# facebookresearch/goliath

Measured on NVIDIA H100. Metric: rendered megapixels/sec (fwd+bwd) RGCA head 300k Gaussians, higher is better.
Workload: dtype f32

## Files before the change

### goliath_b200/_lib.py

```python
import ctypes
import os

import torch

_HERE = os.path.dirname(os.path.abspath(__file__))
LIB_PATH = os.path.join(_HERE, "libgoliath_b200.so")
_lib = None

_vp, _i, _f, _i64, _sz = ctypes.c_void_p, ctypes.c_int, ctypes.c_float, ctypes.c_int64, ctypes.c_size_t

SIGNATURES = {
    "gb_version": (_i, []),
    "gb_launch_count": (ctypes.c_ulonglong, []),
    "gb_launch_count_reset": (None, []),
    "gb_sg_evaluate_fwd": (_i, [_vp] * 7 + [_i] * 4 + [_vp]),
    "gb_sg_evaluate_bwd": (_i, [_vp] * 10 + [_i] * 4 + [_vp]),
    "gb_project_gaussians_fwd": (_i, [_i, _vp, _vp, _f, _vp, _vp, _f, _f, _f, _f, _i, _i, _i, _f] + [_vp] * 7 + [_vp]),
    "gb_project_gaussians_bwd": (_i, [_i, _vp, _vp, _f, _vp, _vp, _f, _f] + [_vp] * 13 + [_vp]),
    "gb_cumsum_workspace_bytes": (_sz, [_i]),
    "gb_cumsum_i32": (_i, [_i, _vp, _vp, _vp, _vp]),
    "gb_map_gaussian_to_intersects": (_i, [_i, _vp, _vp, _vp, _vp, _i, _i, _i, _vp, _vp, _vp]),
    "gb_sort_workspace_bytes": (_sz, [_i64]),
    "gb_sort_intersects": (_i, [_i64, _vp, _vp, _vp, _vp, _i, _vp, _vp]),
    "gb_get_tile_bin_edges": (_i, [_i64, _vp, _vp, _vp]),
    "gb_rasterize_fwd": (_i, [_i, _i, _i, _i] + [_vp] * 10 + [_vp]),
    "gb_rasterize_bwd": (_i, [_i, _i, _i, _i] + [_vp] * 15 + [_vp]),
    "gb_pack_records": (_i, [_i64, _i] + [_vp] * 6 + [_vp]),
    "gb_tile_order": (_i, [_i, _vp, _vp, _vp]),
    "gb_pack_records_fused": (_i, [_i64] + [_vp] * 8 + [_vp]),
    "gb_pack_records_fused_dn": (_i, [_i64] + [_vp] * 9 + [_vp]),
    "gb_map_gaussian_to_intersects_dn": (_i, [_i, _vp, _vp, _vp, _vp, _i, _i, _i, _i64, _vp, _vp, _vp]),
    "gb_sort_intersects_dn": (_i, [_i64, _vp, _vp, _vp, _vp, _vp, _i, _vp, _vp]),
    "gb_get_tile_bin_edges_dn": (_i, [_i64, _vp, _vp, _vp, _vp, _vp]),
    "gb_get_tile_sort_mode": (_i, []),
    "gb_set_tile_sort_mode": (None, [_i]),
    "gb_get_rank_sort_mode": (_i, []),
    "gb_set_rank_sort_mode": (None, [_i]),
    "gb_bin_tiles_supported": (_i, [_i]),
    "gb_bin_tiles_workspace_bytes": (_sz, [_i, _i, _i64]),
    "gb_bin_tiles_pack": (_i, [_i] + [_vp] * 7 + [_i, _i, _i, _i64] + [_vp, _vp, _i] + [_vp] * 5 + [_vp]),
    "gb_bin_tiles_pack_ev": (_i, [_i] + [_vp] * 7 + [_i, _i, _i, _i64] + [_vp, _vp, _i] + [_vp] * 5 + [_vp, _vp]),
    "gb_tile_schedule_ints": (_i, [_i]),
    "gb_tile_schedule": (_i, [_i, _vp, _vp, _vp]),
    "gb_rasterize_sched_fwd": (_i, [_i, _i, _i] + [_vp] * 7 + [_vp]),
    "gb_rasterize_sched_bwd": (_i, [_i, _i, _i] + [_vp] * 13 + [_vp]),
    "gb_records_widen": (_i, [_i64, _vp, _vp, _vp, _vp]),
    "gb_records_set_colors4": (_i, [_i64, _vp, _vp, _vp, _i, _i64, _vp, _vp]),
    "gb_rasterize_multi_fwd": (_i, [_i, _i, _vp, _vp, _i, _vp, _vp, _vp, _vp]),
    "gb_rasterize_multi_bwd": (_i, [_i, _i, _vp, _vp, _vp, _i] + [_vp] * 9 + [_vp]),
    "gb_colors12_unpack": (_i, [_i64, _i, _vp, _vp, _vp]),
    "gb_records_set_colors": (_i, [_i64] + [_vp] * 5 + [_vp]),
    "gb_splat_grad_unpack": (_i, [_i] + [_vp] * 8 + [_vp]),
    "gb_get_blend_mode": (_i, []),
    "gb_set_blend_mode": (None, [_i]),
    "gb_rasterize_packed_fwd": (_i, [_i, _i, _i] + [_vp] * 7 + [_vp]),
    "gb_rasterize_packed_bwd": (_i, [_i, _i, _i] + [_vp] * 13 + [_vp]),
    "gb_rasterize_ranked_fwd": (_i, [_i, _i, _i] + [_vp] * 8 + [_vp]),
    "gb_rasterize_ranked_bwd": (_i, [_i, _i, _i] + [_vp] * 14 + [_vp]),
    "gb_rasterize_ranked_fwd_lists": (_i, [_i, _i, _i] + [_vp] * 10 + [_vp]),
    "gb_rasterize_ranked_bwd_lists": (_i, [_i, _i, _i] + [_vp] * 14 + [_vp]),
    "gb_bin_tiles_ranked": (_i, [_i] + [_vp] * 7 + [_i, _i, _i, _i64] + [_vp, _vp, _i] + [_vp] * 6 + [_vp, _vp]),
    "gb_compute_raydirs_fwd": (_i, [_i, _i, _i] + [_vp] * 5 + [_f] + [_vp] * 3 + [_vp]),
    "gb_compute_raydirs_bwd": (_i, []),
    "gb_mvp_aabb_workspace_bytes": (_sz, [_i, _i]),
    "gb_mvp_compute_aabb": (_i, [_i, _i] + [_vp] * 8 + [_vp]),
    "gb_get_raymarch_mode": (_i, []),
    "gb_set_raymarch_mode": (None, [_i]),
    "gb_mvp_raymarch_fwd": (_i, [_i] * 4 + [_vp, _vp, _f] + [_vp] * 5 + [_i] * 3 + [_vp] + [_i] * 3 + [_vp] * 4
                            + [_i, _f, _f, _i, _i, _vp]),
    "gb_deconv_tc_weight_bytes": (_sz, [_i, _i]),
    "gb_nchw_to_nhwc_split": (_i, [_i] * 5 + [_vp] * 3 + [_vp]),
    "gb_deconv4x4s2_tc_fwd": (_i, [_i] * 6 + [_vp] * 6 + [_f, _i, _vp, _vp, _i, _vp, _vp]),
    "gb_deconv4x4s2_wnub_fwd": (_i, [_i] * 5 + [_vp] * 4 + [_f, _i, _vp, _vp]),
    "gb_deconv4x4s2_wnub_bwd": (_i, [_i] * 5 + [_vp] * 5 + [_f, _i] + [_vp] * 4 + [_vp]),
    "gb_conv4x4s2_wnub_fwd": (_i, [_i] * 5 + [_vp] * 4 + [_f, _i, _vp, _vp]),
    "gb_conv4x4s2_wnub_bwd": (_i, [_i] * 5 + [_vp] * 5 + [_f, _i] + [_vp] * 4 + [_vp]),
    "gb_conv2d_wnub_fwd": (_i, [_i] * 6 + [_vp] * 4 + [_i, _f, _i, _vp, _vp]),
    "gb_conv2d_wnub_bwd": (_i, [_i] * 6 + [_vp] * 5 + [_f, _i, _i] + [_vp] * 4 + [_vp]),
    "gb_mvp_slab_to_prims_fwd": (_i, [_i] * 6 + [_vp] * 3 + [_f, _f, _i, _vp, _vp]),
    "gb_mvp_slab_to_prims_bwd": (_i, [_i] * 6 + [_vp] * 3 + [_f, _f, _i] + [_vp] * 3 + [_vp]),
    "gb_mvp_prim_transform_fwd": (_i, [_i, _i] + [_vp] * 3 + [_f, _i] + [_vp] * 3 + [_vp]),
    "gb_mvp_prim_transform_bwd": (_i, [_i, _i] + [_vp] * 3 + [_f, _i] + [_vp] * 4 + [_vp]),
    "gb_mvp_prim_frames_fwd": (_i, [_i] * 4 + [_vp] * 10 + [_vp]),
    "gb_lbs_max_joints": (_i, []),
    "gb_lbs_skeleton_fwd": (_i, [_i] * 4 + [_vp, _vp, _i] + [_vp] * 7 + [_i] + [_vp] * 3 + [_vp]),
    "gb_lbs_skin_fwd": (_i, [_i] * 4 + [_vp] * 7 + [_vp]),
    "gb_lbs_skin_bwd": (_i, [_i] * 4 + [_vp] * 6 + [_vp]),
    "gb_lbs_unskin_fwd": (_i, [_i] * 4 + [_vp] * 7 + [_vp]),
    "gb_sg_shade_compose_fwd":(_i, [_vp] * 10 + [_i] * 4 + [_vp]),
    "gb_sg_shade_compose_bwd": (_i, [_vp] * 16 + [_i] * 4 + [_vp]),
    "gb_render_finish_fwd": (_i, [_i, _i] + [_vp] * 5 + [_vp]),
    "gb_render_finish_bwd": (_i, [_i, _i] + [_vp] * 4 + [_vp]),
    "gb_rgca_heads_fwd": (_i, [_i, _i] + [_vp] * 7 + [_f, _f] + [_vp] * 15 + [_vp]),
    "gb_rgca_heads_bwd": (_i, [_i, _i] + [_vp] * 7 + [_f, _f] + [_vp] * 20 + [_vp]),
    "gb_vert_normals_fwd": (_i, [_i, _i, _i, _vp, _vp, _f, _vp, _vp, _vp]),
    "gb_vert_normals_bwd": (_i, [_i, _i, _i, _vp, _vp, _f, _vp, _vp, _vp, _vp, _vp]),
    "gb_values_to_uv_fwd": (_i, [_i, _i, _i, _i64, _vp, _vp, _vp, _vp, _vp]),
    "gb_values_to_uv_bwd": (_i, [_i, _i, _i, _i64, _vp, _vp, _vp, _vp, _vp]),
    "gb_optim_chunk_elems": (_i, []),
    "gb_optim_row_bytes": (_i, []),
    "gb_grad_sanitize_sqnorm": (_i, [_vp, _vp, _i, _vp, _vp]),
    "gb_adam_step": (_i, [_vp, _vp, _i, _vp, _f, _f, _f, _f, _i, _i, _i, _vp]),
    "gb_post_render_fwd": (_i, [_i, _i, _i] + [_vp] * 8 + [_vp]),
    "gb_post_render_bwd": (_i, [_i, _i, _i] + [_vp] * 12 + [_vp]),
    "gb_ssim_l1_fwd": (_i, [_i, _i, _i] + [_vp] * 7 + [_vp]),
    "gb_ssim_l1_bwd": (_i, [_i, _i, _i] + [_vp] * 8 + [_f, _f, _vp, _vp]),
    "gb_envmap_spec_fwd": (_i, [_i, _i, _i] + [_vp] * 6 + [_f, _vp, _vp]),
    "gb_envmap_spec_bwd": (_i, [_i, _i, _i] + [_vp] * 6 + [_f, _vp, _vp, _vp, _vp]),
    "gb_envmap_rotate": (_i, [_i, _i, _i, _vp, _vp, _vp, _vp]),
    "gb_envmap_compose_fwd": (_i, [_i] * 5 + [_vp] * 5 + [_i, _i, _vp, _vp, _vp]),
    "gb_envmap_compose_bwd": (_i, [_i, _i, _i, _vp, _vp, _vp]),
    "gb_envmap_prefilter_sg": (_i, [_i, _i] + [_vp] * 5 + [_i, ctypes.c_ulonglong, _vp, _vp]),
    "gb_envmap_spin_table": (_i, [_i, _i, _i, _vp, _vp, _f, _f] + [_vp] * 6 + [_vp]),
    "gb_mvp_shadow_march": (_i, [_i] * 5 + [_vp, _vp, _f] + [_vp] * 5 + [_i] * 4 + [_vp] * 3 + [_f, _f, _i, _i, _vp]),
    "gb_olat_features": (_i, [_i] * 7 + [_f] + [_vp] * 9 + [_i, _vp, _vp]),
    "gb_olat_compose_fwd": (_i, [_i] * 4 + [_vp] * 4 + [_i, _vp, _vp]),
    "gb_olat_compose_bwd": (_i, [_i] * 4 + [_vp] * 6 + [_vp]),
    "gb_mvp_raymarch_bwd":(_i, [_i] * 4 + [_vp, _vp, _f] + [_vp] * 5 + [_i] * 3 + [_vp] + [_i] * 3 + [_vp] * 8
                            + [_i, _f, _f, _i, _i, _vp]),
    "gb_upconv_block_fwd": (_i, [_i] * 6 + [_vp] * 10 + [_f] + [_vp] * 3 + [_vp]),
    "gb_upconv_block_bwd": (_i, [_i] * 6 + [_vp] * 10 + [_f] + [_vp] * 10 + [_vp]),
    "gb_sparse_rows_apply": (_i, [_i] * 3 + [_vp] * 4 + [_i64] * 3 + [_vp] + [_i64] * 3 + [_vp]),
    "gb_conv3x3_ub_slice_fwd": (_i, [_i] * 5 + [_vp, _i64] + [_vp] * 4 + [_vp]),
    "gb_conv3x3_ub_slice_bwd": (_i, [_i] * 5 + [_vp, _i64] + [_vp] * 6 + [_vp]),
    "gb_body_tex_compose_workspace_bytes": (_sz, [_i, _i]),
    "gb_body_tex_compose_fwd": (_i, [_i] * 3 + [_vp] * 5 + [_f] + [_vp] * 3 + [_vp]),
    "gb_body_tex_compose_bwd": (_i, [_i] * 3 + [_vp] * 5 + [_f] + [_vp] * 9 + [_vp]),
    "gb_mesh_raster_workspace_bytes": (_sz, [_i] * 4),
    "gb_mesh_raster": (_i, [_i] * 5 + [_vp] * 4 + [_vp]),
    "gb_mesh_render_fwd": (_i, [_i] * 8 + [_vp] * 11 + [_vp]),
    "gb_mesh_render_bwd_workspace_bytes": (_sz, [_i] * 6),
    "gb_mesh_render_bwd": (_i, [_i] * 8 + [_vp] * 9 + [_i] + [_vp] * 5 + [_vp]),
    "gb_downconv_block_fwd": (_i, [_i] * 6 + [_vp, _i64, _i64, _i, _i, _i, _vp, _f] + [_vp] * 9 + [_f] + [_vp] * 3 + [_vp]),
    "gb_downconv_block_bwd_workspace_bytes": (_sz, [_i] * 6),
    "gb_downconv_block_bwd": (_i, [_i] * 6 + [_vp, _i64, _i64, _i, _i, _i, _vp, _f] + [_vp] * 9 + [_f] + [_vp] * 10
                              + [_vp]),
    "gb_depth_disc_mask": (_i, [_i] * 3 + [_vp, _f, _vp, _vp]),
    "gb_pixel_bias_fwd": (_i, [_i] * 7 + [_vp] * 4 + [_vp]),
    "gb_pixel_bias_bwd": (_i, [_i] * 7 + [_vp] * 3 + [_vp]),
    "gb_face_tex_tail_fwd": (_i, [_i] * 5 + [_vp] * 7 + [_vp]),
    "gb_face_tex_cond_fwd": (_i, [_i] * 6 + [_vp] * 3 + [_vp]),
    "gb_pose_shadow_fwd": (_i, [_i] * 5 + [_vp, _f, _vp, _vp]),
    "gb_pose_shadow_bwd": (_i, [_i] * 5 + [_vp, _f, _vp, _vp, _vp]),
}


class GoliathB200Error(RuntimeError):
    pass


def lib():
    global _lib
    if _lib is None:
        if not os.path.exists(LIB_PATH):
            raise GoliathB200Error(
                "libgoliath_b200.so is not built (%s). Run `python -m goliath_b200.build`; there is no CPU "
                "fallback." % LIB_PATH
            )
        l = ctypes.CDLL(LIB_PATH)
        for name, (res, args) in SIGNATURES.items():
            fn = getattr(l, name)
            fn.restype = res
            fn.argtypes = args
        _lib = l
    return _lib


def check(err, what):
    if err != 0:
        raise GoliathB200Error("%s failed: CUDA error %d" % (what, err))


def ptr(t):
    return None if t is None else t.data_ptr()


def stream_ptr(device=None):
    return torch.cuda.current_stream(device).cuda_stream


def check_input(t, name, dtype=torch.float32):
    if not t.is_cuda:
        raise RuntimeError("%s must be a CUDA tensor" % name)
    if not t.is_contiguous():
        raise RuntimeError("%s must be contiguous" % name)
    if dtype is not None and t.dtype != dtype:
        raise RuntimeError("%s must have dtype %s (got %s)" % (name, dtype, t.dtype))
```

### goliath_b200/csrc/splat_bin_tiles.cu

```cuda

#include "common.cuh"
#include "splat_record.cuh"

#include <algorithm>

extern "C" int gb_tile_order(int num_tiles, const int32_t* tile_bins, int32_t* order, void* stream);
extern "C" int gb_tile_schedule(int num_tiles, const int32_t* tile_bins, int32_t* sched, void* stream);
GB_API int gb_bin_tiles_pack_ev(int G, const float* xys, const float* depths, const int32_t* radii, const float* conics,
                                const float* colors3, const float* opacity, const float* compensation, int img_h,
                                int img_w, int block_width, int64_t cap, int32_t* tile_bins, int32_t* tile_order,
                                int tile_sched, int32_t* gids_sorted, float* records, int32_t* n_out, int32_t* overflow,
                                void* workspace, void* colors_ready, void* stream);

namespace {

constexpr int kGaussBlock = 1024;
constexpr int kScatItems = 3;
constexpr int kMaxSmemTiles = 20 * 1024;
constexpr int kMaxGaussians = 3 << 19;

constexpr int kSortThreads = 512;
constexpr int kSortWarps = kSortThreads / 32;
constexpr int kSortItems = 10;
constexpr int kSortCap = kSortThreads * kSortItems;
constexpr int kDigitBits = 9;
constexpr int kDigits = 1 << kDigitBits;
static_assert(kDigits == kSortThreads, "one digit per thread");
constexpr int kTieRun = 16;

inline int count_items(int G) { return G <= 2048 * 192 ? 2 : 4; }

__device__ __forceinline__ int block_exclusive_scan(int v, int* s_warp, int& total) {
  const int lane = threadIdx.x & 31, warp = threadIdx.x >> 5;
  int inc = v;
#pragma unroll
  for (int o = 1; o < 32; o <<= 1) {
    int t = __shfl_up_sync(0xffffffffu, inc, o);
    if (lane >= o) inc += t;
  }
  if (lane == 31) s_warp[warp] = inc;
  __syncthreads();
  if (warp == 0) {
    int w = (lane < (int)(blockDim.x >> 5)) ? s_warp[lane] : 0;
    int winc = w;
#pragma unroll
    for (int o = 1; o < 32; o <<= 1) {
      int t = __shfl_up_sync(0xffffffffu, winc, o);
      if (lane >= o) winc += t;
    }
    s_warp[lane] = winc - w;
    if (lane == 31) s_warp[32] = winc;
  }
  __syncthreads();
  total = s_warp[32];
  const int r = s_warp[warp] + inc - v;
  __syncthreads();
  return r;
}

__device__ __forceinline__ void tile_bbox(float cx, float cy, float radius, int tbx, int tby, int bw, int& x0,
                                          int& y0, int& x1, int& y1) {
  const float fb = (float)bw;
  const float tcx = __fdiv_rn(cx, fb), tcy = __fdiv_rn(cy, fb), tr = __fdiv_rn(radius, fb);
  x0 = min(max(0, __float2int_rz(__fsub_rn(tcx, tr))), tbx);
  x1 = min(max(0, __float2int_rz(__fadd_rn(__fadd_rn(tcx, tr), 1.f))), tbx);
  y0 = min(max(0, __float2int_rz(__fsub_rn(tcy, tr))), tby);
  y1 = min(max(0, __float2int_rz(__fadd_rn(__fadd_rn(tcy, tr), 1.f))), tby);
}

template <int kItems>
__global__ void __launch_bounds__(kGaussBlock) tile_count_kernel(int G, const float2* __restrict__ xys,
                                                                 const int* __restrict__ radii, int tbx, int tby,
                                                                 int block_width, int smem_tiles,
                                                                 int* __restrict__ tile_counts, int4* __restrict__ rects,
                                                                 int* __restrict__ identity) {
  extern __shared__ int s_cnt[];
  for (int t = threadIdx.x; t < smem_tiles; t += kGaussBlock) s_cnt[t] = 0;
  const int base = blockIdx.x * (kGaussBlock * kItems);
  int r[kItems];
  float2 c[kItems];
#pragma unroll
  for (int j = 0; j < kItems; ++j) {
    const int i = base + j * kGaussBlock + threadIdx.x;
    const bool in = i < G;
    r[j] = in ? radii[i] : 0;
    c[j] = in ? xys[i] : make_float2(0.f, 0.f);
    if (in && identity) identity[i] = i;
  }
  __syncthreads();
#pragma unroll
  for (int j = 0; j < kItems; ++j) {
    const int i = base + j * kGaussBlock + threadIdx.x;
    if (i >= G) continue;
    if (r[j] <= 0) {
      rects[i] = make_int4(-1, 0, 0, 0);
      continue;
    }
    int x0, y0, x1, y1;
    tile_bbox(c[j].x, c[j].y, (float)r[j], tbx, tby, block_width, x0, y0, x1, y1);
    rects[i] = make_int4(x0, y0, x1, y1);
    for (int ty = y0; ty < y1; ++ty)
      for (int tx = x0; tx < x1; ++tx) {
        if (smem_tiles) atomicAdd(&s_cnt[ty * tbx + tx], 1);
        else atomicAdd(&tile_counts[ty * tbx + tx], 1);
      }
  }
  __syncthreads();
  for (int t = threadIdx.x; t < smem_tiles; t += kGaussBlock) {
    const int cnt = s_cnt[t];
    if (cnt) atomicAdd(&tile_counts[t], cnt);
  }
}

__global__ void __launch_bounds__(1024) tile_scan_kernel(int T, long long cap, const int* __restrict__ counts,
                                                         int2* __restrict__ tile_bins, int* __restrict__ cursor,
                                                         int* __restrict__ n_out, int* __restrict__ overflow) {
  __shared__ int s_warp[33];
  int carry = 0;
  for (int base = 0; base < T; base += blockDim.x) {
    const int i = base + threadIdx.x;
    const int v = (i < T) ? counts[i] : 0;
    int total;
    const int ex = block_exclusive_scan(v, s_warp, total);
    if (i < T) {
      const int s = carry + ex;
      cursor[i] = s;
      const int cs = (int)min((long long)s, cap), ce = (int)min((long long)s + v, cap);
      tile_bins[i] = (ce > cs) ? make_int2(cs, ce) : make_int2(0, 0);
    }
    carry += total;
  }
  if (threadIdx.x == 0) {
    if (n_out) *n_out = carry;
    if (overflow && (long long)carry > cap) *overflow = 1;
  }
}

constexpr int kStageCap = 12 * 1024;
constexpr int kStageMaxTiles = 10 * 1024;
constexpr size_t kStageEntryBytes = 4 + 4 + 2;
static_assert(kStageCap * 8 >= (kGaussBlock / 32) * 96 * 16, "the record spans fit in s_id | s_key");

inline int scatter_per_cta(int G, int num_sms) {
  const int per_sm = gb::cdiv(G, num_sms > 0 ? num_sms : 1);
  return std::min(kScatItems * kGaussBlock, std::max(kGaussBlock, (per_sm + 31) & ~31));
}

inline int scatter_stage_cap(int smem_tiles) { return (smem_tiles > 0 && smem_tiles <= kStageMaxTiles) ? kStageCap : 0; }
inline size_t scatter_smem_bytes(int smem_tiles) {
  return (size_t)((smem_tiles + 3) & ~3) * 8 + (size_t)scatter_stage_cap(smem_tiles) * kStageEntryBytes;
}

__global__ void __launch_bounds__(kGaussBlock, 1) tile_scatter_kernel(
    int G, const int4* __restrict__ rects, const float2* __restrict__ xys, const float* __restrict__ conics,
    const float* __restrict__ colors3, const float* __restrict__ depths, const float* __restrict__ opacity,
    const float* __restrict__ comp, int tbx, long long cap, int per_cta, int smem_tiles, int stage_cap,
    int* __restrict__ cursor, int* __restrict__ tile_ids, unsigned* __restrict__ keys, float4* __restrict__ rec_by_id) {
  extern __shared__ int s_cnt[];
  __shared__ int s_warp[33];
  const int tpad = (smem_tiles + 3) & ~3;
  int* s_off = s_cnt + tpad;
  int* s_id = s_off + tpad;
  unsigned* s_key = reinterpret_cast<unsigned*>(s_id + stage_cap);
  unsigned short* s_tile = reinterpret_cast<unsigned short*>(s_key + stage_cap);
  const int lane = threadIdx.x & 31, warp = threadIdx.x >> 5;
  for (int t = threadIdx.x; t < smem_tiles; t += kGaussBlock) s_cnt[t] = 0;
  const int base = blockIdx.x * per_cta, end = min(G, base + per_cta);
  int4 rc[kScatItems];
  unsigned dk[kScatItems];
#pragma unroll
  for (int j = 0; j < kScatItems; ++j) {
    const int i = base + j * kGaussBlock + threadIdx.x;
    rc[j] = (i < end) ? rects[i] : make_int4(-1, 0, 0, 0);
    dk[j] = (i < end) ? __float_as_uint(depths[i]) : 0u;
  }
  __syncthreads();
  unsigned bx[kScatItems], by[kScatItems];
#pragma unroll
  for (int j = 0; j < kScatItems; ++j) {
    const int i = base + j * kGaussBlock + threadIdx.x;
    const bool vis = rc[j].x >= 0;
    bx[j] = vis ? (unsigned)rc[j].x | ((unsigned)rc[j].z << 16) : 0u;
    by[j] = vis ? (unsigned)rc[j].y | ((unsigned)rc[j].w << 16) : 0u;
    if (stage_cap && j * kGaussBlock < per_cta) {
      float4* span = reinterpret_cast<float4*>(s_id) + warp * 96;
      if (vis) gb::pack_record_fused(i, xys, conics, colors3, depths, opacity, comp, span + 3 * lane);
      const unsigned vmask = __ballot_sync(0xffffffffu, vis);
      __syncwarp();
      float4* dst = rec_by_id + 3 * (size_t)(i - lane);
#pragma unroll
      for (int f = lane; f < 96; f += 32) {
        const int r = f / 3, part = f - 3 * r;
        if (((vmask >> r) & 1u) && (part < 2 || colors3)) dst[f] = span[f];
      }
      __syncwarp();
    } else if (vis) {
      gb::pack_record_fused(i, xys, conics, colors3, depths, opacity, comp, rec_by_id + 3 * (size_t)i);
    }
  }
  if (!smem_tiles) {
#pragma unroll
    for (int j = 0; j < kScatItems; ++j) {
      const int i = base + j * kGaussBlock + threadIdx.x;
      const int x0 = bx[j] & 0xffffu, x1 = bx[j] >> 16, y0 = by[j] & 0xffffu, y1 = by[j] >> 16;
      for (int ty = y0; ty < y1; ++ty)
        for (int tx = x0; tx < x1; ++tx) {
          const int pos = atomicAdd(&cursor[ty * tbx + tx], 1);
          if ((long long)pos < cap) {
            tile_ids[pos] = i;
            keys[pos] = dk[j];
          }
        }
    }
    return;
  }
#pragma unroll
  for (int j = 0; j < kScatItems; ++j) {
    const int x0 = bx[j] & 0xffffu, x1 = bx[j] >> 16, y0 = by[j] & 0xffffu, y1 = by[j] >> 16;
    for (int ty = y0; ty < y1; ++ty)
      for (int tx = x0; tx < x1; ++tx) atomicAdd(&s_cnt[ty * tbx + tx], 1);
  }
  __syncthreads();
#pragma unroll 4
  for (int t = threadIdx.x; t < smem_tiles; t += kGaussBlock) {
    const int cnt = s_cnt[t];
    s_off[t] = cnt ? atomicAdd(&cursor[t], cnt) : 0;
  }
  int n_local = 0;
  for (int t0 = 0; t0 < smem_tiles; t0 += kGaussBlock) {
    const int t = t0 + threadIdx.x;
    const int cnt = (t < smem_tiles) ? s_cnt[t] : 0;
    int total;
    const int loc = n_local + block_exclusive_scan(cnt, s_warp, total);
    if (t < smem_tiles) {
      s_off[t] -= loc;
      s_cnt[t] = loc;
    }
    n_local += total;
  }
  __syncthreads();
  const bool staged = n_local <= stage_cap;
#pragma unroll
  for (int j = 0; j < kScatItems; ++j) {
    const int i = base + j * kGaussBlock + threadIdx.x;
    const int x0 = bx[j] & 0xffffu, x1 = bx[j] >> 16, y0 = by[j] & 0xffffu, y1 = by[j] >> 16;
    for (int ty = y0; ty < y1; ++ty)
      for (int tx = x0; tx < x1; ++tx) {
        const int t = ty * tbx + tx;
        const int e = atomicAdd(&s_cnt[t], 1);
        if (staged) {
          s_id[e] = i;
          s_key[e] = dk[j];
          s_tile[e] = (unsigned short)t;
        } else {
          const int pos = s_off[t] + e;
          if ((long long)pos < cap) {
            tile_ids[pos] = i;
            keys[pos] = dk[j];
          }
        }
      }
  }
  if (!staged) return;
  __syncthreads();
  for (int e = threadIdx.x; e < n_local; e += kGaussBlock) {
    const int pos = s_off[s_tile[e]] + e;
    if ((long long)pos < cap) {
      tile_ids[pos] = s_id[e];
      keys[pos] = s_key[e];
    }
  }
}

struct SortSmem {
  unsigned short whist[kSortWarps][kDigits];
  int base[kDigits];
  int run[kDigits];
  int warp[33];
  unsigned red[4];
};

__device__ __forceinline__ int entry_of(int j, int ipt) {
  return (threadIdx.x >> 5) * (32 * ipt) + j * 32 + (threadIdx.x & 31);
}

__device__ __forceinline__ bool holds(int j, int ipt, int m) { return j < ipt && entry_of(j, ipt) < m; }

__device__ __forceinline__ void radix_positions(const unsigned long long (&k)[kSortItems], int m, int ipt, int shift,
                                                bool whole, SortSmem& s, int (&dst)[kSortItems]) {
  const int lane = threadIdx.x & 31, warp = threadIdx.x >> 5;
  const int wbase = warp * (32 * ipt);
  const int ours = min(ipt, max(0, (m - wbase + 31) >> 5)), mine = min(ipt, max(0, (m - wbase - lane + 31) >> 5));
  for (int d = lane; d < kDigits; d += 32) s.whist[warp][d] = 0;
  __syncwarp();
#pragma unroll
  for (int j = 0; j < kSortItems; ++j) {
    dst[j] = 0;
    if (j >= ours) continue;
    const bool valid = j < mine;
    const unsigned dgt = (unsigned)(k[j] >> shift) & (kDigits - 1);
    unsigned peers = __ballot_sync(0xffffffffu, valid);
#pragma unroll
    for (int b = 0; b < kDigitBits; ++b) {
      const unsigned bal = __ballot_sync(0xffffffffu, (dgt >> b) & 1u);
      peers &= ((dgt >> b) & 1u) ? bal : ~bal;
    }
    const unsigned lower = peers & ((1u << lane) - 1u);
    unsigned prev = 0;
    if (valid) prev = s.whist[warp][dgt];
    __syncwarp();
    dst[j] = (int)(prev + __popc(lower));
    if (valid && lower == 0u) s.whist[warp][dgt] = (unsigned short)(prev + __popc(peers));
    __syncwarp();
  }
  __syncthreads();
  {
    const int d = threadIdx.x;
    int run = 0;
#pragma unroll
    for (int w = 0; w < kSortWarps; ++w) {
      const int c = s.whist[w][d];
      s.whist[w][d] = (unsigned short)run;
      run += c;
    }
    int total;
    if (whole) {
      s.base[d] = block_exclusive_scan(run, s.warp, total);
    } else {
      const int b = s.run[d];
      s.base[d] = b;
      s.run[d] = b + run;
    }
  }
  __syncthreads();
#pragma unroll
  for (int j = 0; j < kSortItems; ++j) {
    const unsigned dgt = (unsigned)(k[j] >> shift) & (kDigits - 1);
    dst[j] = (j < mine) ? s.base[dgt] + s.whist[warp][dgt] + dst[j] : -1;
  }
}

__device__ __forceinline__ void smem_pass(unsigned long long (&k)[kSortItems], int n, int ipt, int shift, SortSmem& s,
                                          unsigned long long* s_key) {
  int dst[kSortItems];
  radix_positions(k, n, ipt, shift, true, s, dst);
#pragma unroll
  for (int j = 0; j < kSortItems; ++j)
    if (dst[j] >= 0) s_key[dst[j]] = k[j];
  __syncthreads();
#pragma unroll
  for (int j = 0; j < kSortItems; ++j)
    if (holds(j, ipt, n)) k[j] = s_key[entry_of(j, ipt)];
}

__device__ __forceinline__ void minmax_to_smem(unsigned kmin, unsigned kmax, unsigned imin, unsigned imax, SortSmem& s) {
  kmin = __reduce_min_sync(0xffffffffu, kmin);
  kmax = __reduce_max_sync(0xffffffffu, kmax);
  imin = __reduce_min_sync(0xffffffffu, imin);
  imax = __reduce_max_sync(0xffffffffu, imax);
  if ((threadIdx.x & 31) == 0) {
    atomicMin(&s.red[0], kmin);
    atomicMax(&s.red[1], kmax);
    atomicMin(&s.red[2], imin);
    atomicMax(&s.red[3], imax);
  }
}

__device__ __forceinline__ int bits_of(unsigned span) { return span ? 32 - __clz((int)span) : 0; }

__global__ void __launch_bounds__(kSortThreads, 2) tile_sort_kernel(const int* __restrict__ order,
                                                                    const int2* __restrict__ tile_bins,
                                                                    const unsigned* __restrict__ depth_keys,
                                                                    int* bucket, int* out) {
  extern __shared__ unsigned long long s_key[];
  __shared__ SortSmem s;
  const int tile = order ? order[blockIdx.x] : (int)blockIdx.x;
  const int2 range = tile_bins[tile];
  const int n = range.y - range.x;
  if (n <= 0) return;
  if (threadIdx.x == 0) {
    s.red[0] = s.red[2] = 0xffffffffu;
    s.red[1] = s.red[3] = 0u;
  }
  __syncthreads();

  if (n <= kSortCap) {
    const int ipt = (n + kSortThreads - 1) / kSortThreads;
    int id[kSortItems];
    unsigned dk[kSortItems];
#pragma unroll
    for (int j = 0; j < kSortItems; ++j) {
      const bool h = holds(j, ipt, n);
      id[j] = h ? bucket[range.x + entry_of(j, ipt)] : -1;
      dk[j] = h ? (unsigned)out[range.x + entry_of(j, ipt)] : 0u;
    }
    unsigned kmin = 0xffffffffu, kmax = 0u, imin = 0xffffffffu, imax = 0u;
#pragma unroll
    for (int j = 0; j < kSortItems; ++j) {
      if (id[j] < 0) continue;
      kmin = min(kmin, dk[j]); kmax = max(kmax, dk[j]);
      imin = min(imin, (unsigned)id[j]); imax = max(imax, (unsigned)id[j]);
    }
    minmax_to_smem(kmin, kmax, imin, imax, s);
    __syncthreads();
    kmin = s.red[0];
    imin = s.red[2];
    const int bi = bits_of(s.red[3] - imin), bits = bits_of(s.red[1] - kmin) + bi;
    unsigned long long k[kSortItems];
#pragma unroll
    for (int j = 0; j < kSortItems; ++j)
      k[j] = ((unsigned long long)(dk[j] - kmin) << bi) | (unsigned long long)((unsigned)id[j] - imin);
    for (int shift = bi; shift < bits; shift += kDigitBits) smem_pass(k, n, ipt, shift, s, s_key);
    if (bits == bi) {
#pragma unroll
      for (int j = 0; j < kSortItems; ++j)
        if (holds(j, ipt, n)) s_key[entry_of(j, ipt)] = k[j];
      __syncthreads();
    }
    static_assert(kTieRun < 32 && kSortItems * 5 <= 64, "run lengths are packed 5 bits per item");
    unsigned long long runs = 0ull;
    bool too_long = false;
#pragma unroll
    for (int j = 0; j < kSortItems; ++j) {
      const int e = j * kSortThreads + threadIdx.x;
      if (j >= ipt || e >= n) continue;
      const unsigned long long d = s_key[e] >> bi;
      if (e > 0 && (s_key[e - 1] >> bi) == d) continue;
      int len = 1;
      while (len <= kTieRun && e + len < n && (s_key[e + len] >> bi) == d) ++len;
      if (len > kTieRun) too_long = true;
      else runs |= (unsigned long long)len << (5 * j);
    }
    if (__syncthreads_or(too_long)) {
#pragma unroll
      for (int j = 0; j < kSortItems; ++j) k[j] = holds(j, ipt, n) ? s_key[entry_of(j, ipt)] : 0ull;
      for (int shift = 0; shift < bits; shift += kDigitBits) smem_pass(k, n, ipt, shift, s, s_key);
    } else {
#pragma unroll
      for (int j = 0; j < kSortItems; ++j) {
        const int e = j * kSortThreads + threadIdx.x, len = (int)(runs >> (5 * j)) & 31;
        for (int a = e + 1; a < e + len; ++a) {
          const unsigned long long v = s_key[a];
          int b = a;
          for (; b > e && s_key[b - 1] > v; --b) s_key[b] = s_key[b - 1];
          s_key[b] = v;
        }
      }
      __syncthreads();
    }
    const unsigned long long imask = (1ull << bi) - 1ull;
    for (int e = threadIdx.x; e < n; e += kSortThreads) out[range.x + e] = (int)(imin + (unsigned)(s_key[e] & imask));
    return;
  }

  {
    unsigned kmin = 0xffffffffu, kmax = 0u, imin = 0xffffffffu, imax = 0u;
    for (int i = threadIdx.x; i < n; i += kSortThreads) {
      const int g = bucket[range.x + i];
      const unsigned d = depth_keys[g];
      kmin = min(kmin, d); kmax = max(kmax, d);
      imin = min(imin, (unsigned)g); imax = max(imax, (unsigned)g);
    }
    minmax_to_smem(kmin, kmax, imin, imax, s);
  }
  __syncthreads();
  const unsigned kmin = s.red[0], imin = s.red[2];
  const int bi = bits_of(s.red[3] - imin), bits = bits_of(s.red[1] - kmin) + bi;
  const unsigned long long imask = (1ull << bi) - 1ull;
  auto key_of = [&](int g) {
    return ((unsigned long long)(depth_keys[g] - kmin) << bi) | (unsigned long long)((unsigned)g - imin);
  };
  int* src = bucket + range.x;
  int* dstp = out + range.x;
  for (int shift = 0; shift < bits; shift += kDigitBits) {
    unsigned* s_cnt = reinterpret_cast<unsigned*>(s_key);
    s_cnt[threadIdx.x] = 0u;
    __syncthreads();
    for (int i = threadIdx.x; i < n; i += kSortThreads)
      atomicAdd(&s_cnt[(unsigned)(key_of(src[i]) >> shift) & (kDigits - 1)], 1u);
    __syncthreads();
    int total;
    s.run[threadIdx.x] = block_exclusive_scan((int)s_cnt[threadIdx.x], s.warp, total);
    __syncthreads();
    for (int c0 = 0; c0 < n; c0 += kSortCap) {
      const int m = min(kSortCap, n - c0);
      unsigned long long k[kSortItems];
#pragma unroll
      for (int j = 0; j < kSortItems; ++j)
        k[j] = holds(j, kSortItems, m) ? key_of(src[c0 + entry_of(j, kSortItems)]) : 0ull;
      int dst[kSortItems];
      radix_positions(k, m, kSortItems, shift, false, s, dst);
#pragma unroll
      for (int j = 0; j < kSortItems; ++j)
        if (dst[j] >= 0) dstp[dst[j]] = (int)(imin + (unsigned)(k[j] & imask));
      __syncthreads();
    }
    int* t = src; src = dstp; dstp = t;
  }
  if (src != out + range.x) {
    for (int i = threadIdx.x; i < n; i += kSortThreads) out[range.x + i] = src[i];
  }
}

__global__ void __launch_bounds__(256) rec_colors_kernel(int G, const int* __restrict__ radii,
                                                         const float* __restrict__ colors3,
                                                         const float* __restrict__ depths, float4* __restrict__ rec_by_id) {
  const int g = blockIdx.x * blockDim.x + threadIdx.x;
  if (g >= G || radii[g] <= 0) return;
  rec_by_id[3 * (size_t)g + 2] = make_float4(colors3[3 * (size_t)g], colors3[3 * (size_t)g + 1],
                                             colors3[3 * (size_t)g + 2], depths[g]);
}

__global__ void __launch_bounds__(256) gather_records_kernel(long long cap, const int* __restrict__ n_dev,
                                                             const int* __restrict__ gids_sorted,
                                                             const float4* __restrict__ rec_by_id,
                                                             float4* __restrict__ rec) {
  const long long n = min((long long)*n_dev, cap);
  const long long j = (long long)blockIdx.x * blockDim.x + threadIdx.x;
  if (j >= 3 * n) return;
  const long long i = j / 3;
  const int part = (int)(j - 3 * i);
  rec[j] = gb::ld_nc_f4(rec_by_id + 3 * (size_t)gids_sorted[i] + part);
}

struct Layout {
  size_t counts, sync, zero_bytes, cursor, rects, rec_by_id, bucket, total;
};
inline size_t align256(size_t b) { return (b + 255) & ~(size_t)255; }
inline Layout make_layout(int G, int T, int64_t cap) {
  const int g1 = G > 0 ? G : 1;
  Layout l;
  size_t o = 0;
  l.counts = o; o += align256((size_t)T * 4);
  l.sync = o;   o += 256;
  l.zero_bytes = o;
  l.cursor = o; o += align256((size_t)T * 4);
  l.rects = o;  o += align256((size_t)g1 * 16);
  l.rec_by_id = o; o += align256((size_t)g1 * 48);
  l.bucket = o; o += align256((size_t)(cap > 0 ? cap : 1) * 4);
  l.total = o;
  return l;
}

int num_sms() {
  static int s_sms[64] = {};
  int dev = 0;
  if (cudaGetDevice(&dev) != cudaSuccess) return 0;
  if (dev < 0 || dev >= 64) return 0;
  if (!s_sms[dev] && cudaDeviceGetAttribute(&s_sms[dev], cudaDevAttrMultiProcessorCount, dev) != cudaSuccess) return 0;
  return s_sms[dev];
}

template <typename K>
int opt_in_smem(K kernel, size_t bytes, bool* done) {
  int dev = 0;
  GB_CUDA(cudaGetDevice(&dev));
  if (dev < 0 || dev >= 64 || !done[dev]) {
    GB_CUDA(cudaFuncSetAttribute(kernel, cudaFuncAttributeMaxDynamicSharedMemorySize, (int)bytes));
    if (dev >= 0 && dev < 64) done[dev] = true;
  }
  return 0;
}

}

GB_API int gb_get_tile_sort_mode(void) { return 0; }
GB_API void gb_set_tile_sort_mode(int mode) { (void)mode; }
GB_API int gb_get_rank_sort_mode(void) { return 0; }
GB_API void gb_set_rank_sort_mode(int mode) { (void)mode; }

GB_API int gb_bin_tiles_supported(int G) { return G >= 1 && G <= kMaxGaussians; }

GB_API size_t gb_bin_tiles_workspace_bytes(int G, int num_tiles, int64_t cap) {
  return make_layout(G, num_tiles, cap).total;
}

GB_API int gb_bin_tiles_pack(int G, const float* xys, const float* depths, const int32_t* radii, const float* conics,
                             const float* colors3, const float* opacity, const float* compensation, int img_h,
                             int img_w, int block_width, int64_t cap, int32_t* tile_bins, int32_t* tile_order,
                             int tile_sched, int32_t* gids_sorted, float* records, int32_t* n_out, int32_t* overflow,
                             void* workspace, void* stream) {
  return gb_bin_tiles_pack_ev(G, xys, depths, radii, conics, colors3, opacity, compensation, img_h, img_w, block_width, cap,
                              tile_bins, tile_order, tile_sched, gids_sorted, records, n_out, overflow, workspace, nullptr,
                              stream);
}

static int bin_tiles_impl(int G, const float* xys, const float* depths, const int32_t* radii, const float* conics,
                          const float* colors3, const float* opacity, const float* compensation, int img_h, int img_w,
                          int block_width, int64_t cap, int32_t* tile_bins, int32_t* tile_order, int tile_sched,
                          int32_t* gids_sorted, float* records, int32_t* n_out, int32_t* overflow, void* workspace,
                          void* colors_ready, void* stream, int32_t* ext_ids, float* ext_rec, int32_t* ext_identity);

GB_API int gb_bin_tiles_pack_ev(int G, const float* xys, const float* depths, const int32_t* radii, const float* conics,
                                const float* colors3, const float* opacity, const float* compensation, int img_h,
                                int img_w, int block_width, int64_t cap, int32_t* tile_bins, int32_t* tile_order,
                                int tile_sched, int32_t* gids_sorted, float* records, int32_t* n_out, int32_t* overflow,
                                void* workspace, void* colors_ready, void* stream) {
  return bin_tiles_impl(G, xys, depths, radii, conics, colors3, opacity, compensation, img_h, img_w, block_width, cap,
                        tile_bins, tile_order, tile_sched, gids_sorted, records, n_out, overflow, workspace, colors_ready,
                        stream, nullptr, nullptr, nullptr);
}

GB_API int gb_bin_tiles_ranked(int G, const float* xys, const float* depths, const int32_t* radii, const float* conics,
                               const float* colors3, const float* opacity, const float* compensation, int img_h,
                               int img_w, int block_width, int64_t cap, int32_t* tile_bins, int32_t* tile_order,
                               int tile_sched, int32_t* ranks_sorted, float* rec_by_rank, int32_t* rank_to_gid,
                               int32_t* n_out, int32_t* overflow, void* workspace, void* colors_ready, void* stream) {
  if (!ranks_sorted || !rec_by_rank || !rank_to_gid) return (int)cudaErrorInvalidValue;
  return bin_tiles_impl(G, xys, depths, radii, conics, colors3, opacity, compensation, img_h, img_w, block_width, cap,
                        tile_bins, tile_order, tile_sched, nullptr, nullptr, n_out, overflow, workspace, colors_ready, stream,
                        ranks_sorted, rec_by_rank, rank_to_gid);
}

static int bin_tiles_impl(int G, const float* xys, const float* depths, const int32_t* radii, const float* conics,
                          const float* colors3, const float* opacity, const float* compensation, int img_h, int img_w,
                          int block_width, int64_t cap, int32_t* tile_bins, int32_t* tile_order, int tile_sched,
                          int32_t* gids_sorted, float* records, int32_t* n_out, int32_t* overflow, void* workspace,
                          void* colors_ready, void* stream, int32_t* ext_ids, float* ext_rec, int32_t* ext_identity) {
  if (!gb_bin_tiles_supported(G) || block_width < 1 || cap < 0) return (int)cudaErrorInvalidValue;
  cudaStream_t s = (cudaStream_t)stream;
  const int tbx = gb::cdiv(img_w, block_width), tby = gb::cdiv(img_h, block_width);
  const int T = tbx * tby;
  if (T < 1 || tbx > 65535 || tby > 65535) return (int)cudaErrorInvalidValue;
  const Layout l = make_layout(G, T, cap);
  char* ws = (char*)workspace;
  int* counts = (int*)(ws + l.counts);
  int* cursor = (int*)(ws + l.cursor);
  int* bucket = (int*)(ws + l.bucket);
  int4* rects = (int4*)(ws + l.rects);
  const bool ranked = ext_ids != nullptr;
  float4* rec_by_id = ranked ? (float4*)ext_rec : (float4*)(ws + l.rec_by_id);
  int* ids_sorted = ranked ? ext_ids : gids_sorted;
  const int items = count_items(G);
  const int smem_tiles = (T <= kMaxSmemTiles) ? T : 0;
  const int stage_cap = scatter_stage_cap(smem_tiles);
  const size_t scat_smem = scatter_smem_bytes(smem_tiles);
  static bool s_opt_c2[64] = {}, s_opt_c4[64] = {}, s_opt_scat[64] = {}, s_opt_sort[64] = {};
  if ((size_t)smem_tiles * 4 > 40 * 1024) {
    constexpr size_t kCountSmem = (size_t)kMaxSmemTiles * 4;
    const int e = (items == 2) ? opt_in_smem(tile_count_kernel<2>, kCountSmem, s_opt_c2)
                               : opt_in_smem(tile_count_kernel<4>, kCountSmem, s_opt_c4);
    if (e) return e;
  }
  {
    const size_t a = scatter_smem_bytes(kMaxSmemTiles), b = scatter_smem_bytes(kStageMaxTiles);
    const int e = opt_in_smem(tile_scatter_kernel, a > b ? a : b, s_opt_scat);
    if (e) return e;
  }
  const size_t sort_smem = (size_t)kSortCap * 8;
  {
    const int e = opt_in_smem(tile_sort_kernel, sort_smem, s_opt_sort);
    if (e) return e;
  }

  GB_CUDA(cudaMemsetAsync(ws, 0, l.zero_bytes, s));
  const int ctas = gb::cdiv(G, kGaussBlock * items);
  if (items == 2)
    tile_count_kernel<2><<<ctas, kGaussBlock, (size_t)smem_tiles * 4, s>>>(G, (const float2*)xys, radii, tbx, tby,
                                                                          block_width, smem_tiles, counts, rects, ext_identity);
  else
    tile_count_kernel<4><<<ctas, kGaussBlock, (size_t)smem_tiles * 4, s>>>(G, (const float2*)xys, radii, tbx, tby,
                                                                          block_width, smem_tiles, counts, rects, ext_identity);
  int* n_total = n_out ? n_out : (int*)(ws + l.sync);
  tile_scan_kernel<<<1, 1024, 0, s>>>(T, (long long)cap, counts, (int2*)tile_bins, cursor, n_total, overflow);
  gb::count_launches(2);
  GB_CHECK_LAUNCH();
  const int e = tile_sched ? gb_tile_schedule(T, tile_bins, tile_order, stream)
                           : gb_tile_order(T, tile_bins, tile_order, stream);
  if (e) return e;
  const bool late = colors_ready != nullptr;
  const int per_cta = scatter_per_cta(G, num_sms());
  tile_scatter_kernel<<<gb::cdiv(G, per_cta), kGaussBlock, scat_smem, s>>>(
      G, rects, (const float2*)xys, conics, late ? nullptr : colors3, depths, opacity, compensation, tbx, (long long)cap,
      per_cta, smem_tiles, stage_cap, cursor, bucket, (unsigned*)ids_sorted, rec_by_id);
  tile_sort_kernel<<<T, kSortThreads, sort_smem, s>>>(tile_order, (const int2*)tile_bins, (const unsigned*)depths, bucket,
                                                      ids_sorted);
  gb::count_launches(2);
  if (late) {
    GB_CUDA(cudaStreamWaitEvent(s, (cudaEvent_t)colors_ready, 0));
    rec_colors_kernel<<<gb::cdiv(G, 256), 256, 0, s>>>(G, radii, colors3, depths, rec_by_id);
    gb::count_launches(1);
  }
  if (cap > 0 && !ranked) {
    gather_records_kernel<<<(unsigned)gb::cdiv64(3 * cap, 256), 256, 0, s>>>((long long)cap, n_total, gids_sorted,
                                                                           rec_by_id, (float4*)records);
    gb::count_launches(1);
  }
  GB_CHECK_LAUNCH();
  return 0;
}
```

### goliath_b200/csrc/splat_blend_mom.cu

```cuda
#include <cstdlib>
#include <cstring>

#include "common.cuh"
#include "splat_blend_common.cuh"

namespace {

using namespace gbblend;

constexpr int kPixelWarps = 8;
constexpr int kStageRecs = 128;
constexpr int kFwdStages = 4;
constexpr int kFwdThreads = (kPixelWarps + 1) * 32;
constexpr int kBwdStages = 3;
constexpr int kBwdThreads = kPixelWarps * 32;
constexpr int kChunk = 16;
constexpr int kEntryCap = 48;
constexpr int kMStride = 33;
constexpr float kCullMargin = 2e-3f;

__device__ __forceinline__ float rcp_approx(float x) {
  float r;
  asm("rcp.approx.ftz.f32 %0, %1;" : "=f"(r) : "f"(x));
  return r;
}

__device__ __forceinline__ float exp_neg(float s) {
  float r;
  asm("ex2.approx.ftz.f32 %0, %1;" : "=f"(r) : "f"(s * -1.4426950408889634f));
  return r;
}

__device__ __forceinline__ void cp_async16(void* dst, const void* src) {
  asm volatile("cp.async.cg.shared.global [%0], [%1], 16;" ::"r"(smem_u32(dst)), "l"(src) : "memory");
}
__device__ __forceinline__ void cp_async_arrive(unsigned long long* bar) {
  asm volatile("cp.async.mbarrier.arrive.noinc.shared::cta.b64 [%0];" ::"r"(smem_u32(bar)) : "memory");
}
__device__ __forceinline__ void cp_async_wait_all() { asm volatile("cp.async.wait_all;" ::: "memory"); }
__device__ __forceinline__ void cp_async4(void* dst, const void* src) {
  asm volatile("cp.async.ca.shared.global [%0], [%1], 4;" ::"r"(smem_u32(dst)), "l"(src) : "memory");
}
__device__ __forceinline__ bool footprint_hit(const float4 q0, const float4* __restrict__ q1p, float fx0, float fx1,
                                              float fy0, float fy1) {
  if (!((q0.x + q0.z >= fx0) && (q0.x - q0.z <= fx1) && (q0.y + q0.w >= fy0) && (q0.y - q0.w <= fy1))) return false;
  if (q0.z > 1e30f) return true;
  const float4 q1 = *q1p;
  const float dxlo = q0.x - fx1, dxhi = q0.x - fx0, dylo = q0.y - fy1, dyhi = q0.y - fy0;
  const float ex0 = fminf(fmaxf(0.f, dxlo), dxhi), ey0 = fminf(fmaxf(0.f, dylo), dyhi);
  const float dy1 = fminf(fmaxf(-q1.y * ex0 * rcp_approx(q1.z), dylo), dyhi);
  const float dx2 = fminf(fmaxf(-q1.y * ey0 * rcp_approx(q1.x), dxlo), dxhi);
  const float f1 = 0.5f * (q1.x * ex0 * ex0 + q1.z * dy1 * dy1) + q1.y * ex0 * dy1;
  const float f2 = 0.5f * (q1.x * dx2 * dx2 + q1.z * ey0 * ey0) + q1.y * dx2 * ey0;
  const float s = __logf(255.f * q1.w);
  return fminf(f1, f2) <= s + kCullMargin + 1e-4f * fabsf(s);
}

struct Tile {
  int tile_id, tx, ty;
};
__device__ __forceinline__ Tile make_tile(int tile_id, int tbx) {
  Tile t;
  t.tile_id = tile_id;
  t.ty = tile_id / tbx;
  t.tx = tile_id - t.ty * tbx;
  return t;
}

template <int C, bool LIST, bool RANKED, bool HITS = false>
__global__ void __launch_bounds__(kFwdThreads) blend_fwd_ilp_kernel(
    int img_w, int img_h, int tbx, const int* order, int sched, const int2* __restrict__ tile_bins,
    const float4* __restrict__ rec , const int* __restrict__ ranks ,
    const float* __restrict__ background, float* __restrict__ final_Ts, int* __restrict__ final_idx,
    float* __restrict__ out_img, int* __restrict__ hit_list = nullptr, int* __restrict__ hit_count = nullptr) {
  static_assert(!HITS || LIST, "hit lists are the LIST variant's per-stage lists");
  __shared__ __align__(128) float4 s_rec[kFwdStages][kStageRecs * 3];
  __shared__ __align__(8) unsigned long long s_full[kFwdStages];
  __shared__ __align__(8) unsigned long long s_empty[kFwdStages];
  __shared__ int s_ndone;
  __shared__ int s_tile;
  __shared__ __align__(16) int s_hits[LIST ? kPixelWarps : 1][LIST ? kStageRecs + 4 : 4];

  const int tr = threadIdx.x, lane = tr & 31, warp = tr >> 5;
  if (tr == 0) {
    s_tile = draw_tile(order, sched, tbx * ((img_h + 15) >> 4));
#pragma unroll
    for (int s = 0; s < kFwdStages; ++s) {
      mbar_init(&s_full[s], RANKED ? 32 : 1);
      mbar_init(&s_empty[s], kPixelWarps);
    }
    s_ndone = 0;
    fence_mbar_init();
  }
  __syncthreads();
  if (s_tile < 0) return;
  const Tile tl = make_tile(s_tile, tbx);
  const int2 range = tile_bins[tl.tile_id];
  const int num_batches = (range.y - range.x + kStageRecs - 1) / kStageRecs;

  if (RANKED && warp == kPixelWarps) {
    volatile int* ndone = &s_ndone;
    int r[4];
    auto load_ranks = [&](int b) {
      const int start = range.x + b * kStageRecs;
      const int count = min(kStageRecs, range.y - start);
#pragma unroll
      for (int k = 0; k < 4; ++k) r[k] = (b < num_batches && lane + 32 * k < count) ? ranks[start + lane + 32 * k] : -1;
    };
    load_ranks(0);
    for (int b = 0; b < num_batches; ++b) {
      const int s = b % kFwdStages;
      if (b >= kFwdStages) {
        int go = 1;
        if (lane == 0) {
          const unsigned par = (unsigned)(((b / kFwdStages) - 1) & 1);
          while (!mbar_try(&s_empty[s], par) && *ndone < kPixelWarps) {
        }
          go = *ndone < kPixelWarps;
        }
        go = __shfl_sync(0xffffffffu, go, 0);
        if (!go) break;
      }
#pragma unroll
      for (int k = 0; k < 4; ++k)
        if (r[k] >= 0) {
          const float4* src = rec + 3 * (size_t)r[k];
          float4* dst = &s_rec[s][3 * (lane + 32 * k)];
          cp_async16(dst, src);
          cp_async16(dst + 1, src + 1);
          cp_async16(dst + 2, src + 2);
        }
      cp_async_arrive(&s_full[s]);
      load_ranks(b + 1);
    }
    cp_async_wait_all();
    return;
  }
  if (warp == kPixelWarps) {
    if (lane != 0) return;
    volatile int* ndone = &s_ndone;
    int issued = 0;
    for (int b = 0; b < num_batches; ++b) {
      const int s = b % kFwdStages;
      if (b >= kFwdStages) {
        const unsigned par = (unsigned)(((b / kFwdStages) - 1) & 1);
        while (!mbar_try(&s_empty[s], par) && *ndone < kPixelWarps) {
        }
        if (*ndone >= kPixelWarps) break;
      }
      const int start = range.x + b * kStageRecs;
      const unsigned bytes = (unsigned)min(kStageRecs, range.y - start) * kRecBytes;
      mbar_expect_tx(&s_full[s], bytes);
      bulk_g2s(&s_rec[s][0], rec + (size_t)start * 3, bytes, &s_full[s]);
      issued = b + 1;
    }
    for (int b = max(0, issued - kFwdStages); b < issued; ++b)
      mbar_wait(&s_full[b % kFwdStages], (unsigned)((b / kFwdStages) & 1));
    return;
  }

  const int wx0 = tl.tx * 16 + ((warp & 1) << 3), wy0 = tl.ty * 16 + ((warp >> 1) << 2);
  const int pxi = wx0 + (lane & 7), pyi = wy0 + (lane >> 3);
  const bool inside = (pxi < img_w) && (pyi < img_h);
  const float px = (float)pxi + 0.5f, py = (float)pyi + 0.5f;
  const float fx0 = (float)wx0 + 0.5f, fx1 = (float)wx0 + 7.5f, fy0 = (float)wy0 + 0.5f, fy1 = (float)wy0 + 3.5f;

  bool done = !inside;
  float T = 1.f;
  int cur_idx = 0;
  float acc[4] = {0.f, 0.f, 0.f, 0.f};
  int* const seg = HITS ? hit_list + 8 * (size_t)range.x + (size_t)warp * (range.y - range.x) : nullptr;
  int written = 0, last_pos = -1;

  bool counted = false;
  for (int b = 0; b < num_batches; ++b) {
    const bool all_done = __all_sync(0xffffffffu, done);
    if (all_done && !counted) {
      counted = true;
      if (lane == 0) atomicAdd(&s_ndone, 1);
    }
    const int s = b % kFwdStages;
    const unsigned par = (unsigned)((b / kFwdStages) & 1);
    int st = 0;
    if (lane == 0) {
      volatile int* ndone = &s_ndone;
      for (;;) {
        if (mbar_try(&s_full[s], par)) { st = 1; break; }
        if (all_done && *ndone >= kPixelWarps) { st = 2; break; }
      }
    }
    st = __shfl_sync(0xffffffffu, st, 0);
    if (st == 2) break;
    if (all_done) {
      if (lane == 0) mbar_arrive(&s_empty[s]);
      continue;
    }
    mbar_wait(&s_full[s], par);
    const float4* sr = s_rec[s];
    const int batch_start = range.x + b * kStageRecs;
    const int batch_size = min(kStageRecs, range.y - batch_start);
    if (LIST) {
      int* hl = s_hits[LIST ? warp : 0];
      const unsigned lt = (1u << lane) - 1u;
      int cnt = 0;
#pragma unroll 4
      for (int c0 = 0; c0 < batch_size; c0 += 32) {
        const int ti = c0 + lane;
        bool hit = false;
        if (ti < batch_size) hit = footprint_hit(sr[ti * 3], &sr[ti * 3 + 1], fx0, fx1, fy0, fy1);
        const unsigned mask = __ballot_sync(0xffffffffu, hit);
        if (hit) hl[cnt + __popc(mask & lt)] = ti;
        cnt += __popc(mask);
      }
      __syncwarp();
      if (HITS) {
        for (int i = lane; i < cnt; i += 32) seg[written + i] = batch_start + hl[i];
        if (b == 0 && range.x == 0 && cnt > 0 && hl[0] == 0 && inside) last_pos = 0;
      }
      for (int i0 = 0; i0 < cnt; i0 += 16) {
        const int i1 = min(i0 + 16, cnt);
        for (int i = i0; i < i1; i += 4) {
          const int4 e = *reinterpret_cast<const int4*>(hl + i);
          bool live[4];
          int t[4];
          live[0] = true; live[1] = i + 1 < cnt; live[2] = i + 2 < cnt; live[3] = i + 3 < cnt;
          t[0] = e.x; t[1] = live[1] ? e.y : e.x; t[2] = live[2] ? e.z : e.x; t[3] = live[3] ? e.w : e.x;
          float alpha[4], sig[4];
          float4 col[4];
#pragma unroll
          for (int u = 0; u < 4; ++u) {
            const float4 q0 = sr[t[u] * 3], q1 = sr[t[u] * 3 + 1];
            col[u] = sr[t[u] * 3 + 2];
            const float dx = q0.x - px, dy = q0.y - py;
            sig[u] = 0.5f * (q1.x * dx * dx + q1.z * dy * dy) + q1.y * dx * dy;
            alpha[u] = fminf(kAlphaMaxFwd, q1.w * exp_neg(sig[u]));
          }
#pragma unroll
          for (int u = 0; u < 4; ++u) {
            const bool ok = live[u] && !done && !(sig[u] < 0.f) && !(alpha[u] < kAlphaMin);
            const float next_T = T * (1.f - alpha[u]);
            const bool stop = ok && (next_T <= kTEps);
            const bool take = ok && !stop;
            done = done || stop;
            if (take) {
              const float vis = alpha[u] * T;
              acc[0] += col[u].x * vis;
              acc[1] += col[u].y * vis;
              acc[2] += col[u].z * vis;
              if (C == 4) acc[3] += col[u].w * vis;
              T = next_T;
              cur_idx = batch_start + t[u];
              if (HITS) last_pos = written + i + u;
            }
          }
        }
        if (__all_sync(0xffffffffu, done)) break;
      }
      written += cnt;
    } else {
    for (int c0 = 0; c0 < batch_size; c0 += 32) {
        const int ti = c0 + lane;
        bool hit = false;
        if (ti < batch_size) hit = footprint_hit(sr[ti * 3], &sr[ti * 3 + 1], fx0, fx1, fy0, fy1);
        unsigned mask = __ballot_sync(0xffffffffu, hit);
        while (mask) {
          int t[4];
          bool live[4];
  #pragma unroll
          for (int u = 0; u < 4; ++u) {
            live[u] = mask != 0;
            t[u] = live[u] ? c0 + __ffs(mask) - 1 : t[0];
            mask &= mask - 1;
          }
          float alpha[4], sig[4];
          float4 col[4];
  #pragma unroll
          for (int u = 0; u < 4; ++u) {
            const float4 q0 = sr[t[u] * 3], q1 = sr[t[u] * 3 + 1];
            col[u] = sr[t[u] * 3 + 2];
            const float dx = q0.x - px, dy = q0.y - py;
            sig[u] = 0.5f * (q1.x * dx * dx + q1.z * dy * dy) + q1.y * dx * dy;
            alpha[u] = fminf(kAlphaMaxFwd, q1.w * __expf(-sig[u]));
          }
  #pragma unroll
          for (int u = 0; u < 4; ++u) {
            const bool ok = live[u] && !done && !(sig[u] < 0.f) && !(alpha[u] < kAlphaMin);
            const float next_T = T * (1.f - alpha[u]);
            const bool stop = ok && (next_T <= kTEps);
            const bool take = ok && !stop;
            done = done || stop;
            if (take) {
              const float vis = alpha[u] * T;
              acc[0] += col[u].x * vis;
              acc[1] += col[u].y * vis;
              acc[2] += col[u].z * vis;
              if (C == 4) acc[3] += col[u].w * vis;
              T = next_T;
              cur_idx = batch_start + t[u];
            }
          }
        }
        if (__all_sync(0xffffffffu, done)) break;
      }
  }
    __syncwarp();
    if (lane == 0) mbar_arrive(&s_empty[s]);
  }
  if (HITS) {
#pragma unroll
    for (int o = 16; o > 0; o >>= 1) last_pos = max(last_pos, __shfl_xor_sync(0xffffffffu, last_pos, o));
    if (lane == 0) hit_count[8 * tl.tile_id + warp] = last_pos + 1;
    if (blockIdx.x == 0 && tr == 0) hit_count[8 * tbx * ((img_h + 15) >> 4)] = 0;
  }
  if (inside) {
    const size_t pix = (size_t)pyi * img_w + pxi;
    final_Ts[pix] = T;
    final_idx[pix] = cur_idx;
    if (C == 4) {
      reinterpret_cast<float4*>(out_img)[pix] =
          make_float4(acc[0] + T * background[0], acc[1] + T * background[1], acc[2] + T * background[2],
                      acc[3] + T * background[3]);
    } else {
      out_img[pix * 3 + 0] = acc[0] + T * background[0];
      out_img[pix * 3 + 1] = acc[1] + T * background[1];
      out_img[pix * 3 + 2] = acc[2] + T * background[2];
    }
  }
}

constexpr int kSmRec = kBwdStages * kStageRecs * kRecBytes;
constexpr int kSmEntries = kPixelWarps * kEntryCap * 48;
constexpr int kSmM = kPixelWarps * kChunk * kMStride * 8;
constexpr int kSmVo = kPixelWarps * 32 * 16;
constexpr int kBwdSmem = kSmRec + kSmEntries + kSmM + kSmVo;

template <int C, bool RANKED>
__global__ void __launch_bounds__(kBwdThreads, 3) blend_bwd_mom_kernel(
    int img_w, int img_h, int tbx, const int* order, int sched,
    const int* __restrict__ gids_sorted , const int* __restrict__ ranks ,
    const int2* __restrict__ tile_bins, const float4* __restrict__ rec, const float* __restrict__ background,
    const float* __restrict__ final_Ts, const int* __restrict__ final_idx, const float* __restrict__ v_output,
    const float* __restrict__ v_output_alpha, float* __restrict__ v_xy, float* __restrict__ v_conic,
    float* __restrict__ v_colors, float* __restrict__ v_opacity) {
  extern __shared__ __align__(128) unsigned char smem[];
  float4* s_rec = reinterpret_cast<float4*>(smem);
  __shared__ __align__(8) unsigned long long s_full[kBwdStages];
  __shared__ int s_ticket[kBwdStages];
  __shared__ int s_cta_final;
  __shared__ int s_tile;
  __shared__ int s_rk[RANKED ? kBwdStages : 1][RANKED ? kStageRecs : 1];

  const int tr = threadIdx.x, lane = tr & 31, warp = tr >> 5;
  if (tr == 0) s_tile = draw_tile(order, sched, tbx * ((img_h + 15) >> 4));
  __syncthreads();
  if (s_tile < 0) return;
  float4* E = reinterpret_cast<float4*>(smem + kSmRec) + warp * kEntryCap * 3;
  float2* M = reinterpret_cast<float2*>(smem + kSmRec + kSmEntries) + warp * kChunk * kMStride;
  float4* VO = reinterpret_cast<float4*>(smem + kSmRec + kSmEntries + kSmM) + warp * 32;

  const Tile tl = make_tile(s_tile, tbx);
  const int2 range = tile_bins[tl.tile_id];
  if (range.y <= range.x) return;
  const int wx0 = tl.tx * 16 + ((warp & 1) << 3), wy0 = tl.ty * 16 + ((warp >> 1) << 2);
  const int pxi = wx0 + (lane & 7), pyi = wy0 + (lane >> 3);
  const bool inside = (pxi < img_w) && (pyi < img_h);
  const float px = (float)pxi + 0.5f, py = (float)pyi + 0.5f;
  const float fx0 = (float)wx0 + 0.5f, fx1 = (float)wx0 + 7.5f, fy0 = (float)wy0 + 0.5f, fy1 = (float)wy0 + 3.5f;
  const size_t pix = inside ? ((size_t)pyi * img_w + pxi) : 0;

  const float T_final = inside ? final_Ts[pix] : 1.f;
  float T = T_final;
  float bufv = 0.f;
  const int bin_final = inside ? final_idx[pix] : -1;
  float vo[4] = {0.f, 0.f, 0.f, 0.f};
  float voa = 0.f;
  if (inside) {
#pragma unroll
    for (int c = 0; c < C; ++c) vo[c] = v_output[pix * C + c];
    voa = v_output_alpha ? v_output_alpha[pix] : 0.f;
  }
  VO[lane] = make_float4(vo[0], vo[1], vo[2], vo[3]);
  float bgdot = 0.f;
#pragma unroll
  for (int c = 0; c < C; ++c) bgdot += background[c] * vo[c];
  const float tfc = T_final * (voa - bgdot);

  int warp_bin_final = bin_final;
#pragma unroll
  for (int o = 16; o > 0; o >>= 1) warp_bin_final = max(warp_bin_final, __shfl_xor_sync(0xffffffffu, warp_bin_final, o));
  if (tr == 0) {
    s_cta_final = -1;
#pragma unroll
    for (int s = 0; s < kBwdStages; ++s) {
      mbar_init(&s_full[s], RANKED ? 32 : 1);
      s_ticket[s] = 0;
    }
    fence_mbar_init();
  }
  __syncthreads();
  if (lane == 0) atomicMax(&s_cta_final, warp_bin_final);
  __syncthreads();
  const int last = min(s_cta_final, range.y - 1);
  if (last < range.x) return;
  const int num_batches = (last - range.x + kStageRecs) / kStageRecs;
  auto issue = [&](int k) {
    const int s = k % kBwdStages;
    const int hi = last - k * kStageRecs;
    const int lo = max(range.x, hi - kStageRecs + 1);
    const unsigned bytes = (unsigned)(hi - lo + 1) * kRecBytes;
    mbar_expect_tx(&s_full[s], bytes);
    bulk_g2s(s_rec + s * kStageRecs * 3, rec + (size_t)lo * 3, bytes, &s_full[s]);
  };
  auto issue_ranked = [&](int k) {
    const int s = k % kBwdStages;
    const int hi = last - k * kStageRecs;
    const int lo = max(range.x, hi - kStageRecs + 1);
    const int count = hi - lo + 1;
    int r[4];
#pragma unroll
    for (int i = 0; i < 4; ++i) {
      const int j = lane + 32 * i;
      r[i] = (j < count) ? (k >= kBwdStages ? s_rk[s][j] : ranks[lo + j]) : -1;
    }
    float4* stage = s_rec + s * kStageRecs * 3;
#pragma unroll
    for (int i = 0; i < 4; ++i)
      if (r[i] >= 0) {
        const float4* src = rec + 3 * (size_t)r[i];
        float4* dst = stage + 3 * (lane + 32 * i);
        cp_async16(dst, src);
        cp_async16(dst + 1, src + 1);
        cp_async16(dst + 2, src + 2);
      }
    const int k2 = k + kBwdStages;
    if (k2 < num_batches) {
      const int hi2 = last - k2 * kStageRecs;
      const int lo2 = max(range.x, hi2 - kStageRecs + 1);
#pragma unroll
      for (int i = 0; i < 4; ++i) {
        const int j = lane + 32 * i;
        if (j < hi2 - lo2 + 1) cp_async4(&s_rk[s][j], ranks + lo2 + j);
      }
    }
    cp_async_arrive(&s_full[s]);
  };
  if (RANKED) {
    if (warp == 0)
      for (int k = 0; k < min(kBwdStages, num_batches); ++k) issue_ranked(k);
  } else if (tr == 0) {
    for (int k = 0; k < min(kBwdStages, num_batches); ++k) issue(k);
  }

  auto chunk = [&](int base, int n) {
#pragma unroll 1
    for (int h0 = 0; h0 < n; h0 += 4) {
      float al[4], ov[4], ra[4];
      float4 col[4];
#pragma unroll
      for (int u = 0; u < 4; ++u) {
        const int h = h0 + u;
        const float4 a0 = E[(base + h) * 3], a1 = E[(base + h) * 3 + 1];
        col[u] = E[(base + h) * 3 + 2];
        const float dx = a0.x - px, dy = a0.y - py;
        const float sigma = 0.5f * (a0.z * dx * dx + a1.x * dy * dy) + a0.w * dx * dy;
        const float vis = exp_neg(sigma);
        const float alpha = fminf(kAlphaMaxBwd, a1.y * vis);
        const bool valid = (__float_as_int(a1.z) <= bin_final) && !(sigma < 0.f) && !(alpha < kAlphaMin);
        al[u] = valid ? alpha : 0.f;
        ov[u] = valid ? a1.y * vis : 0.f;
        ra[u] = rcp_approx(1.f - al[u]);
      }
#pragma unroll
      for (int u = 0; u < 4; ++u) {
        const float cc[4] = {col[u].x, col[u].y, col[u].z, col[u].w};
        float cv = 0.f;
#pragma unroll
        for (int c = 0; c < C; ++c) cv += cc[c] * vo[c];
        const float v_alpha = ((cv * T - bufv) + tfc) * ra[u];
        T *= ra[u];
        const float fac = al[u] * T;
        bufv += cv * fac;
        M[(h0 + u) * kMStride + lane] = make_float2(fac, -ov[u] * v_alpha);
      }
    }
    if (RANKED) cp_async_wait_all();
    __syncwarp();
    {
      const int hh = lane & 15, half = lane >> 4;
      const int he = min(hh, n - 1);
      const float4 a0 = E[(base + he) * 3], a1 = E[(base + he) * 3 + 1];
      const int e_idx = __float_as_int(a1.z);
      const int e_safe = e_idx == 0x7fffffff ? range.x : e_idx;
      const int g_id = RANKED ? __float_as_int(a1.w) : gids_sorted[e_safe];
      const float2* Mrow = M + hh * kMStride + half * 16;
      const float4* V = VO + half * 16;
      float g[4] = {0.f, 0.f, 0.f, 0.f};
      float r00 = 0.f, r01 = 0.f, r10 = 0.f, r11 = 0.f, sii = 0.f;
      float facmax = 0.f;
#pragma unroll
      for (int q = 0; q < 16; ++q) {
        const float2 m = Mrow[q];
        const float4 v = V[q];
        const float fi = (float)(q & 7);
        facmax = fmaxf(facmax, m.x);
        g[0] += m.x * v.x;
        g[1] += m.x * v.y;
        g[2] += m.x * v.z;
        if (C == 4) g[3] += m.x * v.w;
        if (q < 8) {
          r00 += m.y;
          r10 += m.y * fi;
        } else {
          r01 += m.y;
          r11 += m.y * fi;
        }
        sii += m.y * (fi * fi);
      }
      const float u_ = a0.x - fx0, v_ = a0.y - (fy0 + (float)(2 * half));
      const float S0 = r00 + r01, Sj = r01, Si = r10 + r11, Sij = r11;
      const float sx = u_ * S0 - Si, sy = v_ * S0 - Sj;
      const float sxx = u_ * (u_ * S0 - 2.f * Si) + sii;
      const float sxy = u_ * (v_ * S0 - Sj) - v_ * Si + Sij;
      const float syy = v_ * (v_ * S0 - 2.f * Sj) + Sj;
      float o[10];
      o[0] = g[0]; o[1] = g[1]; o[2] = g[2]; o[3] = g[3];
      o[4] = 0.5f * sxx; o[5] = sxy; o[6] = 0.5f * syy;
      o[7] = a0.z * sx + a0.w * sy;
      o[8] = a0.w * sx + a1.x * sy;
      o[9] = S0;
#pragma unroll
      for (int i = 0; i < 10; ++i) o[i] += __shfl_xor_sync(0xffffffffu, o[i], 16);
      facmax = fmaxf(facmax, __shfl_xor_sync(0xffffffffu, facmax, 16));
      if (half == 0 && hh < n && facmax > 0.f) {
        if (C == 4) {
          gb::red_add_v4(v_colors + 4 * (size_t)g_id, o[0], o[1], o[2], o[3]);
        } else {
          gb::red_add(v_colors + 3 * (size_t)g_id + 0, o[0]);
          gb::red_add(v_colors + 3 * (size_t)g_id + 1, o[1]);
          gb::red_add(v_colors + 3 * (size_t)g_id + 2, o[2]);
        }
        gb::red_add(v_conic + 3 * (size_t)g_id + 0, o[4]);
        gb::red_add(v_conic + 3 * (size_t)g_id + 1, o[5]);
        gb::red_add(v_conic + 3 * (size_t)g_id + 2, o[6]);
        gb::red_add_v2(v_xy + 2 * (size_t)g_id, o[7], o[8]);
        gb::red_add(v_opacity + g_id, -o[9] * rcp_approx(a1.y));
      }
    }
    __syncwarp();
  };

  auto pad4 = [&](int cnt_) {
    const int padded = (cnt_ + 3) & ~3;
    if (lane < padded - cnt_) {
      E[(cnt_ + lane) * 3 + 0] = make_float4(0.f, 0.f, 1.f, 0.f);
      E[(cnt_ + lane) * 3 + 1] = make_float4(1.f, 0.f, __int_as_float(0x7fffffff), 0.f);
      E[(cnt_ + lane) * 3 + 2] = make_float4(0.f, 0.f, 0.f, 0.f);
    }
    __syncwarp();
    return padded;
  };
  int cnt = 0;
  for (int k = 0; k < num_batches; ++k) {
    const int s = k % kBwdStages;
    const int hi = last - k * kStageRecs;
    const int lo = max(range.x, hi - kStageRecs + 1);
    const int batch_size = hi - lo + 1;
    while (!mbar_try(&s_full[s], (unsigned)((k / kBwdStages) & 1))) __nanosleep(64);
    const float4* sr = s_rec + s * kStageRecs * 3;
    const int j_top = min(batch_size - 1, warp_bin_final - lo);
    for (int c1 = (j_top & ~31); c1 >= 0 && j_top >= 0; c1 -= 32) {
      const int tj = c1 + lane;
      bool hit = false;
      if (tj <= j_top) hit = footprint_hit(sr[tj * 3], &sr[tj * 3 + 1], fx0, fx1, fy0, fy1);
      const unsigned mask = __ballot_sync(0xffffffffu, hit);
      if (mask == 0) continue;
      if (hit) {
        const int pos = cnt + __popc(mask & ~((2u << lane) - 1u));
        const float4 q0 = sr[tj * 3], q1 = sr[tj * 3 + 1], q2 = sr[tj * 3 + 2];
        E[pos * 3 + 0] = make_float4(q0.x, q0.y, q1.x, q1.y);
        if constexpr (RANKED) {
          float* e1 = reinterpret_cast<float*>(&E[pos * 3 + 1]);
          *reinterpret_cast<float2*>(e1) = make_float2(q1.z, q1.w);
          e1[2] = __int_as_float(lo + tj);
          cp_async4(e1 + 3, ranks + lo + tj);
        } else {
          E[pos * 3 + 1] = make_float4(q1.z, q1.w, __int_as_float(lo + tj), 0.f);
        }
        E[pos * 3 + 2] = q2;
      }
      cnt += __popc(mask);
      __syncwarp();
      if (cnt >= kChunk) {
        int base = 0;
        while (cnt - base >= kChunk) {
          chunk(base, kChunk);
          base += kChunk;
        }
        const int left = cnt - base;
        if (lane < left) {
          const float4 e0 = E[(base + lane) * 3], e1 = E[(base + lane) * 3 + 1], e2 = E[(base + lane) * 3 + 2];
          E[lane * 3 + 0] = e0;
          E[lane * 3 + 1] = e1;
          E[lane * 3 + 2] = e2;
        }
        cnt = left;
        __syncwarp();
      }
    }
    __syncwarp();
    int refill = 0;
    if (lane == 0) {
      __threadfence_block();
      const int ticket = atomicAdd(&s_ticket[s], 1);
      if (ticket == kPixelWarps - 1) {
        __threadfence_block();
        s_ticket[s] = 0;
        if (k + kBwdStages < num_batches) {
          if (RANKED) refill = 1;
          else issue(k + kBwdStages);
        }
      }
    }
    if (RANKED) {
      refill = __shfl_sync(0xffffffffu, refill, 0);
      if (refill) issue_ranked(k + kBwdStages);
    }
  }
  if (cnt > 0) chunk(0, pad4(cnt));
  if (RANKED) cp_async_wait_all();
}

constexpr int kListWarps = 4;
constexpr int kListThreads = kListWarps * 32;
constexpr int kOrderBuckets = 64;

__device__ __forceinline__ void cp_async_commit() { asm volatile("cp.async.commit_group;" ::: "memory"); }

__global__ void __launch_bounds__(1024) order_items_kernel(int n_items, int* __restrict__ hit_count) {
  __shared__ int s_off[kOrderBuckets];
  const int tr = threadIdx.x, lane = tr & 31;
  auto bucket = [](int n) { return kOrderBuckets - 1 - min((n + kChunk - 1) / kChunk, kOrderBuckets - 1); };
  if (tr < kOrderBuckets) s_off[tr] = 0;
  __syncthreads();
  for (int i = tr; i < n_items; i += blockDim.x) {
    const int n = hit_count[i];
    if (n > 0) atomicAdd(&s_off[bucket(n)], 1);
  }
  __syncthreads();
  if (tr < 32) {
    const int a = s_off[2 * lane], b = s_off[2 * lane + 1];
    int incl = a + b;
#pragma unroll
    for (int o = 1; o < 32; o <<= 1) {
      const int t = __shfl_up_sync(0xffffffffu, incl, o);
      if (lane >= o) incl += t;
    }
    const int excl = incl - a - b;
    s_off[2 * lane] = excl;
    s_off[2 * lane + 1] = excl + a;
    if (lane == 31) hit_count[n_items + 1] = incl;
  }
  __syncthreads();
  int* items = hit_count + n_items + 2;
  for (int i = tr; i < n_items; i += blockDim.x) {
    const int n = hit_count[i];
    if (n > 0) items[atomicAdd(&s_off[bucket(n)], 1)] = i;
  }
}

template <int C>
__global__ void __launch_bounds__(kListThreads, 6) blend_bwd_lists_kernel(
    int img_w, int img_h, int tbx, int n_items, const int2* __restrict__ tile_bins, const int* __restrict__ hit_list,
    const int* __restrict__ hit_count, int* draw ,
    const int* __restrict__ ranks, const float4* __restrict__ rec, const float* __restrict__ background,
    const float* __restrict__ final_Ts, const int* __restrict__ final_idx, const float* __restrict__ v_output,
    const float* __restrict__ v_output_alpha, float* __restrict__ v_xy, float* __restrict__ v_conic,
    float* __restrict__ v_colors, float* __restrict__ v_opacity) {
  __shared__ __align__(16) float4 s_e[kListWarps][2][kChunk * 3];
  __shared__ __align__(8) int2 s_ig[kListWarps][2][kChunk];
  __shared__ float2 s_m[kListWarps][kChunk * kMStride];
  __shared__ float4 s_vo[kListWarps][32];

  const int lane = threadIdx.x & 31, wib = threadIdx.x >> 5;
  float2* M = s_m[wib];
  float4* VO = s_vo[wib];
  const int n_work = hit_count[n_items + 1];
  const int* items = hit_count + n_items + 2;
  const int n_draws = n_work + (int)gridDim.x * kListWarps;
  for (;;) {
    int k = 0;
    if (lane == 0) {
      k = atomicAdd(draw, 1);
      if (k == n_draws - 1) *draw = 0;
    }
    k = __shfl_sync(0xffffffffu, k, 0);
    if (k >= n_work) break;
    const int item = items[k], tile = item >> 3, warp = item & 7;
    const int n = hit_count[item];
    const int2 range = tile_bins[tile];
    const int* list = hit_list + 8 * (size_t)range.x + (size_t)warp * (range.y - range.x);
    const Tile tl = make_tile(tile, tbx);
    const int wx0 = tl.tx * 16 + ((warp & 1) << 3), wy0 = tl.ty * 16 + ((warp >> 1) << 2);
    const int pxi = wx0 + (lane & 7), pyi = wy0 + (lane >> 3);
    const bool inside = (pxi < img_w) && (pyi < img_h);
    const float px = (float)pxi + 0.5f, py = (float)pyi + 0.5f;
    const float fx0 = (float)wx0 + 0.5f, fy0 = (float)wy0 + 0.5f;
    const size_t pix = inside ? ((size_t)pyi * img_w + pxi) : 0;

    const int nchunks = (n + kChunk - 1) / kChunk;
    int g_idx = 0, g_id = 0;
    auto load_next = [&](int j) {
      const int top = n - kChunk * j;
      if (lane < min(kChunk, top)) {
        g_idx = list[top - 1 - lane];
        g_id = ranks[g_idx];
      }
    };
    auto gather = [&](int j) {
      const int cnt = min(kChunk, n - kChunk * j);
      float4* E = s_e[wib][j & 1];
      if (lane < cnt) {
        const float4* src = rec + 3 * (size_t)g_id;
        cp_async16(&E[lane * 3 + 0], src);
        cp_async16(&E[lane * 3 + 1], src + 1);
        cp_async16(&E[lane * 3 + 2], src + 2);
        s_ig[wib][j & 1][lane] = make_int2(g_idx, g_id);
      } else if (lane < ((cnt + 3) & ~3)) {
        E[lane * 3 + 0] = make_float4(0.f, 0.f, 0.f, 0.f);
        E[lane * 3 + 1] = make_float4(1.f, 0.f, 1.f, 0.f);
        E[lane * 3 + 2] = make_float4(0.f, 0.f, 0.f, 0.f);
        s_ig[wib][j & 1][lane] = make_int2(0x7fffffff, 0);
      }
      cp_async_commit();
    };
    load_next(0);
    gather(0);

    const float T_final = inside ? final_Ts[pix] : 1.f;
    float T = T_final;
    float bufv = 0.f;
    const int bin_final = inside ? final_idx[pix] : -1;
    float vo[4] = {0.f, 0.f, 0.f, 0.f};
    float voa = 0.f;
    if (inside) {
#pragma unroll
      for (int c = 0; c < C; ++c) vo[c] = v_output[pix * C + c];
      voa = v_output_alpha ? v_output_alpha[pix] : 0.f;
    }
    VO[lane] = make_float4(vo[0], vo[1], vo[2], vo[3]);
    float bgdot = 0.f;
#pragma unroll
    for (int c = 0; c < C; ++c) bgdot += background[c] * vo[c];
    const float tfc = T_final * (voa - bgdot);
    if (nchunks > 1) load_next(1);

    for (int j = 0; j < nchunks; ++j) {
      const int cnt = min(kChunk, n - kChunk * j);
      const int nn = j + 1 < nchunks ? kChunk : ((cnt + 3) & ~3);
      const float4* E = s_e[wib][j & 1];
      const int2* IG = s_ig[wib][j & 1];
      cp_async_wait_all();
      __syncwarp();
#pragma unroll 1
      for (int h0 = 0; h0 < nn; h0 += 4) {
        float al[4], ov[4], ra[4];
        float4 col[4];
#pragma unroll
        for (int u = 0; u < 4; ++u) {
          const int h = h0 + u;
          const float4 q0 = E[h * 3], q1 = E[h * 3 + 1];
          col[u] = E[h * 3 + 2];
          const float dx = q0.x - px, dy = q0.y - py;
          const float sigma = 0.5f * (q1.x * dx * dx + q1.z * dy * dy) + q1.y * dx * dy;
          const float vis = exp_neg(sigma);
          const float alpha = fminf(kAlphaMaxBwd, q1.w * vis);
          const bool valid = (IG[h].x <= bin_final) && !(sigma < 0.f) && !(alpha < kAlphaMin);
          al[u] = valid ? alpha : 0.f;
          ov[u] = valid ? q1.w * vis : 0.f;
          ra[u] = rcp_approx(1.f - al[u]);
        }
#pragma unroll
        for (int u = 0; u < 4; ++u) {
          const float cc[4] = {col[u].x, col[u].y, col[u].z, col[u].w};
          float cv = 0.f;
#pragma unroll
          for (int c = 0; c < C; ++c) cv += cc[c] * vo[c];
          const float v_alpha = ((cv * T - bufv) + tfc) * ra[u];
          T *= ra[u];
          const float fac = al[u] * T;
          bufv += cv * fac;
          M[(h0 + u) * kMStride + lane] = make_float2(fac, -ov[u] * v_alpha);
        }
      }
      if (j + 1 < nchunks) {
        gather(j + 1);
        if (j + 2 < nchunks) load_next(j + 2);
      }
      __syncwarp();
      {
        const int hh = lane & 15, half = lane >> 4;
        const int he = min(hh, nn - 1);
        const float4 q0 = E[he * 3], q1 = E[he * 3 + 1];
        const int e_id = IG[he].y;
        const float2* Mrow = M + hh * kMStride + half * 16;
        const float4* V = VO + half * 16;
        float g[4] = {0.f, 0.f, 0.f, 0.f};
        float r00 = 0.f, r01 = 0.f, r10 = 0.f, r11 = 0.f, sii = 0.f;
        float facmax = 0.f;
#pragma unroll
        for (int q = 0; q < 16; ++q) {
          const float2 m = Mrow[q];
          const float4 v = V[q];
          const float fi = (float)(q & 7);
          facmax = fmaxf(facmax, m.x);
          g[0] += m.x * v.x;
          g[1] += m.x * v.y;
          g[2] += m.x * v.z;
          if (C == 4) g[3] += m.x * v.w;
          if (q < 8) {
            r00 += m.y;
            r10 += m.y * fi;
          } else {
            r01 += m.y;
            r11 += m.y * fi;
          }
          sii += m.y * (fi * fi);
        }
        const float u_ = q0.x - fx0, v_ = q0.y - (fy0 + (float)(2 * half));
        const float S0 = r00 + r01, Sj = r01, Si = r10 + r11, Sij = r11;
        const float sx = u_ * S0 - Si, sy = v_ * S0 - Sj;
        const float sxx = u_ * (u_ * S0 - 2.f * Si) + sii;
        const float sxy = u_ * (v_ * S0 - Sj) - v_ * Si + Sij;
        const float syy = v_ * (v_ * S0 - 2.f * Sj) + Sj;
        float o[10];
        o[0] = g[0]; o[1] = g[1]; o[2] = g[2]; o[3] = g[3];
        o[4] = 0.5f * sxx; o[5] = sxy; o[6] = 0.5f * syy;
        o[7] = q1.x * sx + q1.y * sy;
        o[8] = q1.y * sx + q1.z * sy;
        o[9] = S0;
#pragma unroll
        for (int i = 0; i < 10; ++i) o[i] += __shfl_xor_sync(0xffffffffu, o[i], 16);
        facmax = fmaxf(facmax, __shfl_xor_sync(0xffffffffu, facmax, 16));
        if (half == 0 && hh < nn && facmax > 0.f) {
          if (C == 4) {
            gb::red_add_v4(v_colors + 4 * (size_t)e_id, o[0], o[1], o[2], o[3]);
          } else {
            gb::red_add(v_colors + 3 * (size_t)e_id + 0, o[0]);
            gb::red_add(v_colors + 3 * (size_t)e_id + 1, o[1]);
            gb::red_add(v_colors + 3 * (size_t)e_id + 2, o[2]);
          }
          gb::red_add(v_conic + 3 * (size_t)e_id + 0, o[4]);
          gb::red_add(v_conic + 3 * (size_t)e_id + 1, o[5]);
          gb::red_add(v_conic + 3 * (size_t)e_id + 2, o[6]);
          gb::red_add_v2(v_xy + 2 * (size_t)e_id, o[7], o[8]);
          gb::red_add(v_opacity + e_id, -o[9] * rcp_approx(q1.w));
        }
      }
      __syncwarp();
    }
  }
}

constexpr int kMK = 4;
constexpr int kMC = 3 * kMK;
constexpr int kMRQ = 5;
constexpr int kMRecBytes = kMRQ * 16;

__global__ void __launch_bounds__(kFwdThreads) blend_fwd_multi_kernel(
    int img_w, int img_h, int tbx, const int* order, int sched, const int2* __restrict__ tile_bins,
    const float4* __restrict__ rec, const float* __restrict__ background, float* __restrict__ out_planes ) {
  __shared__ __align__(128) float4 s_rec[kFwdStages][kStageRecs * kMRQ];
  __shared__ __align__(8) unsigned long long s_full[kFwdStages];
  __shared__ __align__(8) unsigned long long s_empty[kFwdStages];
  __shared__ int s_ndone;
  __shared__ __align__(16) int s_hits[kPixelWarps][kStageRecs + 4];
  __shared__ int s_tile;

  const int tr = threadIdx.x, lane = tr & 31, warp = tr >> 5;
  if (tr == 0) {
    s_tile = draw_tile(order, sched, tbx * ((img_h + 15) >> 4));
#pragma unroll
    for (int s = 0; s < kFwdStages; ++s) {
      mbar_init(&s_full[s], 1);
      mbar_init(&s_empty[s], kPixelWarps);
    }
    s_ndone = 0;
    fence_mbar_init();
  }
  __syncthreads();
  if (s_tile < 0) return;
  const Tile tl = make_tile(s_tile, tbx);
  const int2 range = tile_bins[tl.tile_id];
  const int num_batches = (range.y - range.x + kStageRecs - 1) / kStageRecs;

  if (warp == kPixelWarps) {
    if (lane != 0) return;
    volatile int* ndone = &s_ndone;
    int issued = 0;
    for (int b = 0; b < num_batches; ++b) {
      const int s = b % kFwdStages;
      if (b >= kFwdStages) {
        const unsigned par = (unsigned)(((b / kFwdStages) - 1) & 1);
        while (!mbar_try(&s_empty[s], par) && *ndone < kPixelWarps) {
        }
        if (*ndone >= kPixelWarps) break;
      }
      const int start = range.x + b * kStageRecs;
      const unsigned bytes = (unsigned)min(kStageRecs, range.y - start) * kMRecBytes;
      mbar_expect_tx(&s_full[s], bytes);
      bulk_g2s(&s_rec[s][0], rec + (size_t)start * kMRQ, bytes, &s_full[s]);
      issued = b + 1;
    }
    for (int b = max(0, issued - kFwdStages); b < issued; ++b)
      mbar_wait(&s_full[b % kFwdStages], (unsigned)((b / kFwdStages) & 1));
    return;
  }

  const int wx0 = tl.tx * 16 + ((warp & 1) << 3), wy0 = tl.ty * 16 + ((warp >> 1) << 2);
  const int pxi = wx0 + (lane & 7), pyi = wy0 + (lane >> 3);
  const bool inside = (pxi < img_w) && (pyi < img_h);
  const float px = (float)pxi + 0.5f, py = (float)pyi + 0.5f;
  const float fx0 = (float)wx0 + 0.5f, fx1 = (float)wx0 + 7.5f, fy0 = (float)wy0 + 0.5f, fy1 = (float)wy0 + 3.5f;

  bool done = !inside;
  float T = 1.f;
  float acc[kMC];
#pragma unroll
  for (int c = 0; c < kMC; ++c) acc[c] = 0.f;

  bool counted = false;
  for (int b = 0; b < num_batches; ++b) {
    const bool all_done = __all_sync(0xffffffffu, done);
    if (all_done && !counted) {
      counted = true;
      if (lane == 0) atomicAdd(&s_ndone, 1);
    }
    const int s = b % kFwdStages;
    const unsigned par = (unsigned)((b / kFwdStages) & 1);
    int st = 0;
    if (lane == 0) {
      volatile int* ndone = &s_ndone;
      for (;;) {
        if (mbar_try(&s_full[s], par)) { st = 1; break; }
        if (all_done && *ndone >= kPixelWarps) { st = 2; break; }
      }
    }
    st = __shfl_sync(0xffffffffu, st, 0);
    if (st == 2) break;
    if (all_done) {
      if (lane == 0) mbar_arrive(&s_empty[s]);
      continue;
    }
    mbar_wait(&s_full[s], par);
    const float4* sr = s_rec[s];
    const int batch_start = range.x + b * kStageRecs;
    const int batch_size = min(kStageRecs, range.y - batch_start);
    {
      int* hl = s_hits[warp];
      const unsigned lt = (1u << lane) - 1u;
      int cnt = 0;
#pragma unroll 4
      for (int c0 = 0; c0 < batch_size; c0 += 32) {
        const int ti = c0 + lane;
        bool hit = false;
        if (ti < batch_size) hit = footprint_hit(sr[ti * kMRQ], &sr[ti * kMRQ + 1], fx0, fx1, fy0, fy1);
        const unsigned mask = __ballot_sync(0xffffffffu, hit);
        if (hit) hl[cnt + __popc(mask & lt)] = ti;
        cnt += __popc(mask);
      }
      __syncwarp();
      for (int i0 = 0; i0 < cnt; i0 += 16) {
        const int i1 = min(i0 + 16, cnt);
        for (int i = i0; i < i1; i += 2) {
          const int2 e = *reinterpret_cast<const int2*>(hl + i);
          bool live[2];
          int t[2];
          live[0] = true; live[1] = i + 1 < cnt;
          t[0] = e.x; t[1] = live[1] ? e.y : e.x;
          float alpha[2], sig[2];
          float4 col[2][3];
#pragma unroll
          for (int u = 0; u < 2; ++u) {
            const float4 q0 = sr[t[u] * kMRQ], q1 = sr[t[u] * kMRQ + 1];
            col[u][0] = sr[t[u] * kMRQ + 2]; col[u][1] = sr[t[u] * kMRQ + 3]; col[u][2] = sr[t[u] * kMRQ + 4];
            const float dx = q0.x - px, dy = q0.y - py;
            sig[u] = 0.5f * (q1.x * dx * dx + q1.z * dy * dy) + q1.y * dx * dy;
            alpha[u] = fminf(kAlphaMaxFwd, q1.w * exp_neg(sig[u]));
          }
#pragma unroll
          for (int u = 0; u < 2; ++u) {
            const bool ok = live[u] && !done && !(sig[u] < 0.f) && !(alpha[u] < kAlphaMin);
            const float next_T = T * (1.f - alpha[u]);
            const bool stop = ok && (next_T <= kTEps);
            const bool take = ok && !stop;
            done = done || stop;
            if (take) {
              const float vis = alpha[u] * T;
              const float cc[kMC] = {col[u][0].x, col[u][0].y, col[u][0].z, col[u][0].w, col[u][1].x, col[u][1].y,
                                     col[u][1].z, col[u][1].w, col[u][2].x, col[u][2].y, col[u][2].z, col[u][2].w};
#pragma unroll
              for (int c = 0; c < kMC; ++c) acc[c] += cc[c] * vis;
              T = next_T;
            }
          }
        }
        if (__all_sync(0xffffffffu, done)) break;
      }
    }
    __syncwarp();
    if (lane == 0) mbar_arrive(&s_empty[s]);
  }
  if (inside) {
    const size_t pix = (size_t)pyi * img_w + pxi, plane = (size_t)img_h * img_w * 3;
#pragma unroll
    for (int k = 0; k < kMK; ++k) {
      float* o = out_planes + k * plane + pix * 3;
      o[0] = acc[3 * k + 0] + T * background[0];
      o[1] = acc[3 * k + 1] + T * background[1];
      o[2] = acc[3 * k + 2] + T * background[2];
    }
  }
}

constexpr int kMSmRec = kBwdStages * kStageRecs * kMRecBytes;
constexpr int kMSmEntries = kPixelWarps * kEntryCap * kMRecBytes;
constexpr int kMSmM = kPixelWarps * kChunk * kMStride * 8;
constexpr int kMSmVo = kPixelWarps * 32 * 48;
constexpr int kMBwdSmem = kMSmRec + kMSmEntries + kMSmM + kMSmVo;

__global__ void __launch_bounds__(kBwdThreads, 2) blend_bwd_multi_kernel(
    int img_w, int img_h, int tbx, const int* order, int sched, const int* __restrict__ gids_sorted,
    const int2* __restrict__ tile_bins, const float4* __restrict__ rec, const float* __restrict__ background,
    const float* __restrict__ final_Ts, const int* __restrict__ final_idx,
    const float* __restrict__ v_planes , float* __restrict__ v_xy, float* __restrict__ v_conic,
    float* __restrict__ v_colors12 , float* __restrict__ v_opacity) {
  extern __shared__ __align__(128) unsigned char smem[];
  float4* s_rec = reinterpret_cast<float4*>(smem);
  __shared__ __align__(8) unsigned long long s_full[kBwdStages];
  __shared__ int s_ticket[kBwdStages];
  __shared__ int s_cta_final;
  __shared__ int s_tile;

  const int tr = threadIdx.x, lane = tr & 31, warp = tr >> 5;
  if (tr == 0) s_tile = draw_tile(order, sched, tbx * ((img_h + 15) >> 4));
  __syncthreads();
  if (s_tile < 0) return;
  float4* E = reinterpret_cast<float4*>(smem + kMSmRec) + warp * kEntryCap * kMRQ;
  float2* M = reinterpret_cast<float2*>(smem + kMSmRec + kMSmEntries) + warp * kChunk * kMStride;
  float4* VO = reinterpret_cast<float4*>(smem + kMSmRec + kMSmEntries + kMSmM) + warp * 32 * 3;

  const Tile tl = make_tile(s_tile, tbx);
  const int2 range = tile_bins[tl.tile_id];
  if (range.y <= range.x) return;
  const int wx0 = tl.tx * 16 + ((warp & 1) << 3), wy0 = tl.ty * 16 + ((warp >> 1) << 2);
  const int pxi = wx0 + (lane & 7), pyi = wy0 + (lane >> 3);
  const bool inside = (pxi < img_w) && (pyi < img_h);
  const float px = (float)pxi + 0.5f, py = (float)pyi + 0.5f;
  const float fx0 = (float)wx0 + 0.5f, fx1 = (float)wx0 + 7.5f, fy0 = (float)wy0 + 0.5f, fy1 = (float)wy0 + 3.5f;
  const size_t pix = inside ? ((size_t)pyi * img_w + pxi) : 0, plane = (size_t)img_h * img_w * 3;

  const float T_final = inside ? final_Ts[pix] : 1.f;
  float T = T_final;
  const int bin_final = inside ? final_idx[pix] : -1;
  float vo[kMC];
  float bufv = 0.f;
  float bgdot = 0.f;
#pragma unroll
  for (int k = 0; k < kMK; ++k) {
#pragma unroll
    for (int c = 0; c < 3; ++c) {
      vo[3 * k + c] = inside ? v_planes[k * plane + pix * 3 + c] : 0.f;
      bgdot += background[c] * vo[3 * k + c];
    }
  }
  VO[lane * 3 + 0] = make_float4(vo[0], vo[1], vo[2], vo[3]);
  VO[lane * 3 + 1] = make_float4(vo[4], vo[5], vo[6], vo[7]);
  VO[lane * 3 + 2] = make_float4(vo[8], vo[9], vo[10], vo[11]);
  const float tfc = -T_final * bgdot;

  int warp_bin_final = bin_final;
#pragma unroll
  for (int o = 16; o > 0; o >>= 1) warp_bin_final = max(warp_bin_final, __shfl_xor_sync(0xffffffffu, warp_bin_final, o));
  if (tr == 0) {
    s_cta_final = -1;
#pragma unroll
    for (int s = 0; s < kBwdStages; ++s) {
      mbar_init(&s_full[s], 1);
      s_ticket[s] = 0;
    }
    fence_mbar_init();
  }
  __syncthreads();
  if (lane == 0) atomicMax(&s_cta_final, warp_bin_final);
  __syncthreads();
  const int last = min(s_cta_final, range.y - 1);
  if (last < range.x) return;
  const int num_batches = (last - range.x + kStageRecs) / kStageRecs;
  auto issue = [&](int k) {
    const int s = k % kBwdStages;
    const int hi = last - k * kStageRecs;
    const int lo = max(range.x, hi - kStageRecs + 1);
    const unsigned bytes = (unsigned)(hi - lo + 1) * kMRecBytes;
    mbar_expect_tx(&s_full[s], bytes);
    bulk_g2s(s_rec + s * kStageRecs * kMRQ, rec + (size_t)lo * kMRQ, bytes, &s_full[s]);
  };
  if (tr == 0)
    for (int k = 0; k < min(kBwdStages, num_batches); ++k) issue(k);

  auto chunk = [&](int base, int n) {
#pragma unroll 1
    for (int h0 = 0; h0 < n; h0 += 2) {
      float al[2], ov[2], ra[2];
#pragma unroll
      for (int u = 0; u < 2; ++u) {
        const int h = h0 + u;
        const float4 a0 = E[(base + h) * kMRQ], a1 = E[(base + h) * kMRQ + 1];
        const float dx = a0.x - px, dy = a0.y - py;
        const float sigma = 0.5f * (a0.z * dx * dx + a1.x * dy * dy) + a0.w * dx * dy;
        const float vis = exp_neg(sigma);
        const float alpha = fminf(kAlphaMaxBwd, a1.y * vis);
        const bool valid = (__float_as_int(a1.z) <= bin_final) && !(sigma < 0.f) && !(alpha < kAlphaMin);
        al[u] = valid ? alpha : 0.f;
        ov[u] = valid ? a1.y * vis : 0.f;
        ra[u] = rcp_approx(1.f - al[u]);
      }
#pragma unroll
      for (int u = 0; u < 2; ++u) {
        const float4 c0 = E[(base + h0 + u) * kMRQ + 2], c1 = E[(base + h0 + u) * kMRQ + 3], c2 = E[(base + h0 + u) * kMRQ + 4];
        const float cc[kMC] = {c0.x, c0.y, c0.z, c0.w, c1.x, c1.y, c1.z, c1.w, c2.x, c2.y, c2.z, c2.w};
        float cv = 0.f;
#pragma unroll
        for (int c = 0; c < kMC; ++c) cv += cc[c] * vo[c];
        const float v_alpha = ((cv * T - bufv) + tfc) * ra[u];
        T *= ra[u];
        const float fac = al[u] * T;
        bufv += cv * fac;
        M[(h0 + u) * kMStride + lane] = make_float2(fac, -ov[u] * v_alpha);
      }
    }
    __syncwarp();
    {
      const int hh = lane & 15, half = lane >> 4;
      const int he = min(hh, n - 1);
      const float4 a0 = E[(base + he) * kMRQ], a1 = E[(base + he) * kMRQ + 1];
      const int e_idx = __float_as_int(a1.z);
      const int g_id = gids_sorted[e_idx == 0x7fffffff ? 0 : e_idx];
      const float2* Mrow = M + hh * kMStride + half * 16;
      const float4* V = VO + half * 16 * 3;
      float g[kMC];
#pragma unroll
      for (int c = 0; c < kMC; ++c) g[c] = 0.f;
      float r00 = 0.f, r01 = 0.f, r10 = 0.f, r11 = 0.f, sii = 0.f, facmax = 0.f;
#pragma unroll
      for (int q = 0; q < 16; ++q) {
        const float2 m = Mrow[q];
        const float4 v0 = V[q * 3], v1 = V[q * 3 + 1], v2 = V[q * 3 + 2];
        const float fi = (float)(q & 7);
        facmax = fmaxf(facmax, m.x);
        g[0] += m.x * v0.x; g[1] += m.x * v0.y; g[2] += m.x * v0.z; g[3] += m.x * v0.w;
        g[4] += m.x * v1.x; g[5] += m.x * v1.y; g[6] += m.x * v1.z; g[7] += m.x * v1.w;
        g[8] += m.x * v2.x; g[9] += m.x * v2.y; g[10] += m.x * v2.z; g[11] += m.x * v2.w;
        if (q < 8) {
          r00 += m.y;
          r10 += m.y * fi;
        } else {
          r01 += m.y;
          r11 += m.y * fi;
        }
        sii += m.y * (fi * fi);
      }
      const float u_ = a0.x - fx0, v_ = a0.y - (fy0 + (float)(2 * half));
      const float S0 = r00 + r01, Sj = r01, Si = r10 + r11, Sij = r11;
      const float sx = u_ * S0 - Si, sy = v_ * S0 - Sj;
      const float sxx = u_ * (u_ * S0 - 2.f * Si) + sii;
      const float sxy = u_ * (v_ * S0 - Sj) - v_ * Si + Sij;
      const float syy = v_ * (v_ * S0 - 2.f * Sj) + Sj;
      float o[kMC + 6];
#pragma unroll
      for (int c = 0; c < kMC; ++c) o[c] = g[c];
      o[kMC + 0] = 0.5f * sxx; o[kMC + 1] = sxy; o[kMC + 2] = 0.5f * syy;
      o[kMC + 3] = a0.z * sx + a0.w * sy;
      o[kMC + 4] = a0.w * sx + a1.x * sy;
      o[kMC + 5] = S0;
#pragma unroll
      for (int i = 0; i < kMC + 6; ++i) o[i] += __shfl_xor_sync(0xffffffffu, o[i], 16);
      facmax = fmaxf(facmax, __shfl_xor_sync(0xffffffffu, facmax, 16));
      if (half == 0 && hh < n && facmax > 0.f) {
        float* vc = v_colors12 + (size_t)kMC * g_id;
        gb::red_add_v4(vc, o[0], o[1], o[2], o[3]);
        gb::red_add_v4(vc + 4, o[4], o[5], o[6], o[7]);
        gb::red_add_v4(vc + 8, o[8], o[9], o[10], o[11]);
        gb::red_add(v_conic + 3 * (size_t)g_id + 0, o[kMC + 0]);
        gb::red_add(v_conic + 3 * (size_t)g_id + 1, o[kMC + 1]);
        gb::red_add(v_conic + 3 * (size_t)g_id + 2, o[kMC + 2]);
        gb::red_add_v2(v_xy + 2 * (size_t)g_id, o[kMC + 3], o[kMC + 4]);
        gb::red_add(v_opacity + g_id, -o[kMC + 5] * rcp_approx(a1.y));
      }
    }
    __syncwarp();
  };

  auto pad2 = [&](int cnt_) {
    const int padded = (cnt_ + 1) & ~1;
    if (lane < padded - cnt_) {
      E[(cnt_ + lane) * kMRQ + 0] = make_float4(0.f, 0.f, 1.f, 0.f);
      E[(cnt_ + lane) * kMRQ + 1] = make_float4(1.f, 0.f, __int_as_float(0x7fffffff), 0.f);
      E[(cnt_ + lane) * kMRQ + 2] = make_float4(0.f, 0.f, 0.f, 0.f);
      E[(cnt_ + lane) * kMRQ + 3] = make_float4(0.f, 0.f, 0.f, 0.f);
      E[(cnt_ + lane) * kMRQ + 4] = make_float4(0.f, 0.f, 0.f, 0.f);
    }
    __syncwarp();
    return padded;
  };
  int cnt = 0;
  for (int k = 0; k < num_batches; ++k) {
    const int s = k % kBwdStages;
    const int hi = last - k * kStageRecs;
    const int lo = max(range.x, hi - kStageRecs + 1);
    const int batch_size = hi - lo + 1;
    while (!mbar_try(&s_full[s], (unsigned)((k / kBwdStages) & 1))) __nanosleep(64);
    const float4* sr = s_rec + s * kStageRecs * kMRQ;
    const int j_top = min(batch_size - 1, warp_bin_final - lo);
    for (int c1 = (j_top & ~31); c1 >= 0 && j_top >= 0; c1 -= 32) {
      const int tj = c1 + lane;
      bool hit = false;
      if (tj <= j_top) hit = footprint_hit(sr[tj * kMRQ], &sr[tj * kMRQ + 1], fx0, fx1, fy0, fy1);
      const unsigned mask = __ballot_sync(0xffffffffu, hit);
      if (mask == 0) continue;
      if (hit) {
        const int pos = cnt + __popc(mask & ~((2u << lane) - 1u));
        const float4 q0 = sr[tj * kMRQ], q1 = sr[tj * kMRQ + 1];
        E[pos * kMRQ + 0] = make_float4(q0.x, q0.y, q1.x, q1.y);
        E[pos * kMRQ + 1] = make_float4(q1.z, q1.w, __int_as_float(lo + tj), 0.f);
        E[pos * kMRQ + 2] = sr[tj * kMRQ + 2];
        E[pos * kMRQ + 3] = sr[tj * kMRQ + 3];
        E[pos * kMRQ + 4] = sr[tj * kMRQ + 4];
      }
      cnt += __popc(mask);
      __syncwarp();
      if (cnt >= kChunk) {
        int base = 0;
        while (cnt - base >= kChunk) {
          chunk(base, kChunk);
          base += kChunk;
        }
        const int left = cnt - base;
        if (lane < left) {
          float4 e[kMRQ];
#pragma unroll
          for (int q = 0; q < kMRQ; ++q) e[q] = E[(base + lane) * kMRQ + q];
#pragma unroll
          for (int q = 0; q < kMRQ; ++q) E[lane * kMRQ + q] = e[q];
        }
        cnt = left;
        __syncwarp();
      }
    }
    __syncwarp();
    if (lane == 0) {
      __threadfence_block();
      const int ticket = atomicAdd(&s_ticket[s], 1);
      if (ticket == kPixelWarps - 1) {
        __threadfence_block();
        s_ticket[s] = 0;
        if (k + kBwdStages < num_batches) issue(k + kBwdStages);
      }
    }
  }
  if (cnt > 0) chunk(0, pad2(cnt));
}

__global__ void __launch_bounds__(256) records_widen_kernel(long long cap, const int* __restrict__ n_dev,
                                                            const float4* __restrict__ rec12, float4* __restrict__ rec20) {
  const long long n = n_dev ? min((long long)*n_dev, cap) : cap;
  const long long i = (long long)blockIdx.x * blockDim.x + threadIdx.x;
  if (i >= n) return;
  rec20[kMRQ * i + 0] = rec12[3 * i + 0];
  rec20[kMRQ * i + 1] = rec12[3 * i + 1];
}

__global__ void __launch_bounds__(256) records_set_colors4_kernel(long long cap, const int* __restrict__ n_dev,
                                                                  const int* __restrict__ gids_sorted,
                                                                  const float* __restrict__ colors , int nk,
                                                                  long long G, float4* __restrict__ rec20) {
  const long long n = n_dev ? min((long long)*n_dev, cap) : cap;
  const long long i = (long long)blockIdx.x * blockDim.x + threadIdx.x;
  if (i >= n) return;
  const int g = gids_sorted[i];
  float c[kMC];
#pragma unroll
  for (int k = 0; k < kMK; ++k) {
    const float* src = colors + ((size_t)k * G + g) * 3;
    const bool on = k < nk;
    c[3 * k + 0] = on ? src[0] : 0.f; c[3 * k + 1] = on ? src[1] : 0.f; c[3 * k + 2] = on ? src[2] : 0.f;
  }
  rec20[kMRQ * i + 2] = make_float4(c[0], c[1], c[2], c[3]);
  rec20[kMRQ * i + 3] = make_float4(c[4], c[5], c[6], c[7]);
  rec20[kMRQ * i + 4] = make_float4(c[8], c[9], c[10], c[11]);
}

__global__ void __launch_bounds__(256) colors12_unpack_kernel(long long G, int nk, float4* __restrict__ v12,
                                                              float* __restrict__ v_colors ) {
  const long long g = (long long)blockIdx.x * blockDim.x + threadIdx.x;
  if (g >= G) return;
  const float4 a = v12[3 * g], b = v12[3 * g + 1], c = v12[3 * g + 2];
  const float v[kMC] = {a.x, a.y, a.z, a.w, b.x, b.y, b.z, b.w, c.x, c.y, c.z, c.w};
#pragma unroll
  for (int k = 0; k < kMK; ++k)
    if (k < nk) {
      float* dst = v_colors + ((size_t)k * G + g) * 3;
      dst[0] = v[3 * k]; dst[1] = v[3 * k + 1]; dst[2] = v[3 * k + 2];
    }
  const float4 z = make_float4(0.f, 0.f, 0.f, 0.f);
  v12[3 * g] = z; v12[3 * g + 1] = z; v12[3 * g + 2] = z;
}

bool g_multi_attr_set[64] = {};

bool g_attr_set[64] = {};

}

namespace gbblend {

static bool fwd_list_variant() {
  const char* e = getenv("GOLIATH_B200_BLEND_FWD");
  return !(e && !strcmp(e, "rounds"));
}

static int launch_fwd_any(int img_h, int img_w, int channels, const int32_t* tile_bins, const int32_t* tile_order, int sched,
                          const float* records, const int32_t* ranks, const float* background, float* out_img,
                          float* final_Ts, int32_t* final_idx, cudaStream_t s, int32_t* hit_list = nullptr,
                          int32_t* hit_count = nullptr) {
  const int tbx = gb::cdiv(img_w, 16), tby = gb::cdiv(img_h, 16);
  if (sched && !tile_order) return (int)cudaErrorInvalidValue;
  static const bool list = fwd_list_variant();
#define GB_FWD_MOM(CC, LL, RR, ...)                                                                                     \
  blend_fwd_ilp_kernel<CC, LL, RR, ##__VA_ARGS__><<<tbx * tby, kFwdThreads, 0, s>>>(                                   \
      img_w, img_h, tbx, tile_order, sched, (const int2*)tile_bins, (const float4*)records, ranks, background, final_Ts, \
      final_idx, out_img, hit_list, hit_count)
  if (ranks && hit_list) {
    if (channels == 3) GB_FWD_MOM(3, true, true, true); else GB_FWD_MOM(4, true, true, true);
  } else if (ranks) {
    if (channels == 3) GB_FWD_MOM(3, true, true); else GB_FWD_MOM(4, true, true);
  } else if (channels == 3) {
    if (list) GB_FWD_MOM(3, true, false); else GB_FWD_MOM(3, false, false);
  } else {
    if (list) GB_FWD_MOM(4, true, false); else GB_FWD_MOM(4, false, false);
  }
#undef GB_FWD_MOM
  gb::count_launches(1);
  GB_CHECK_LAUNCH();
  return 0;
}

static int launch_bwd_any(int img_h, int img_w, int channels, const int32_t* gids_sorted, const int32_t* ranks,
                          const int32_t* tile_bins, const int32_t* tile_order, int sched, const float* records,
                          const float* background, const float* final_Ts, const int32_t* final_idx, const float* v_output,
                          const float* v_output_alpha, float* v_xy, float* v_conic, float* v_colors, float* v_opacity,
                          cudaStream_t s) {
  const int tbx = gb::cdiv(img_w, 16), tby = gb::cdiv(img_h, 16);
  if (sched && !tile_order) return (int)cudaErrorInvalidValue;
  int dev = 0;
  GB_CUDA(cudaGetDevice(&dev));
  if (dev < 0 || dev >= 64 || !g_attr_set[dev]) {
    GB_CUDA(cudaFuncSetAttribute(blend_bwd_mom_kernel<3, false>, cudaFuncAttributeMaxDynamicSharedMemorySize, kBwdSmem));
    GB_CUDA(cudaFuncSetAttribute(blend_bwd_mom_kernel<4, false>, cudaFuncAttributeMaxDynamicSharedMemorySize, kBwdSmem));
    GB_CUDA(cudaFuncSetAttribute(blend_bwd_mom_kernel<3, true>, cudaFuncAttributeMaxDynamicSharedMemorySize, kBwdSmem));
    GB_CUDA(cudaFuncSetAttribute(blend_bwd_mom_kernel<4, true>, cudaFuncAttributeMaxDynamicSharedMemorySize, kBwdSmem));
    if (dev >= 0 && dev < 64) g_attr_set[dev] = true;
  }
#define GB_BWD_MOM(CC, RR)                                                                                              \
  blend_bwd_mom_kernel<CC, RR><<<tbx * tby, kBwdThreads, kBwdSmem, s>>>(                                                \
      img_w, img_h, tbx, tile_order, sched, gids_sorted, ranks, (const int2*)tile_bins, (const float4*)records, background, \
      final_Ts, final_idx, v_output, v_output_alpha, v_xy, v_conic, v_colors, v_opacity)
  if (ranks) {
    if (channels == 3) GB_BWD_MOM(3, true); else GB_BWD_MOM(4, true);
  } else {
    if (channels == 3) GB_BWD_MOM(3, false); else GB_BWD_MOM(4, false);
  }
#undef GB_BWD_MOM
  gb::count_launches(1);
  GB_CHECK_LAUNCH();
  return 0;
}

static int launch_bwd_lists(int img_h, int img_w, int channels, const int32_t* ranks, const int32_t* tile_bins,
                            const int32_t* hit_list, int32_t* hit_count, const float* records,
                            const float* background, const float* final_Ts, const int32_t* final_idx,
                            const float* v_output, const float* v_output_alpha, float* v_xy, float* v_conic,
                            float* v_colors, float* v_opacity, cudaStream_t s) {
  const int tbx = gb::cdiv(img_w, 16), tby = gb::cdiv(img_h, 16);
  const int n_items = 8 * tbx * tby;
  int dev = 0;
  GB_CUDA(cudaGetDevice(&dev));
  static int resident[64][2] = {};
  int uncached = 0;
  int& per_sm = (dev >= 0 && dev < 64) ? resident[dev][channels == 4] : uncached;
  if (per_sm == 0) {
    int n = 0, sms = 0;
    if (channels == 4)
      GB_CUDA(cudaOccupancyMaxActiveBlocksPerMultiprocessor(&n, blend_bwd_lists_kernel<4>, kListThreads, 0));
    else
      GB_CUDA(cudaOccupancyMaxActiveBlocksPerMultiprocessor(&n, blend_bwd_lists_kernel<3>, kListThreads, 0));
    GB_CUDA(cudaDeviceGetAttribute(&sms, cudaDevAttrMultiProcessorCount, dev));
    per_sm = max(1, n) * sms;
  }
  const int grid = min(per_sm, gb::cdiv(n_items, kListWarps));
  order_items_kernel<<<1, 1024, 0, s>>>(n_items, hit_count);
#define GB_BWD_LISTS(CC)                                                                                                \
  blend_bwd_lists_kernel<CC><<<grid, kListThreads, 0, s>>>(                                                             \
      img_w, img_h, tbx, n_items, (const int2*)tile_bins, hit_list, hit_count, hit_count + n_items, ranks,              \
      (const float4*)records, background, final_Ts, final_idx, v_output, v_output_alpha, v_xy, v_conic, v_colors,       \
      v_opacity)
  if (channels == 3) GB_BWD_LISTS(3); else GB_BWD_LISTS(4);
#undef GB_BWD_LISTS
  gb::count_launches(2);
  GB_CHECK_LAUNCH();
  return 0;
}

int launch_fwd_mom(int img_h, int img_w, int channels, const int32_t* tile_bins, const int32_t* tile_order, int sched,
                   const float* records, const float* background, float* out_img, float* final_Ts, int32_t* final_idx,
                   cudaStream_t s) {
  return launch_fwd_any(img_h, img_w, channels, tile_bins, tile_order, sched, records, nullptr, background, out_img, final_Ts,
                        final_idx, s);
}

int launch_bwd_mom(int img_h, int img_w, int channels, const int32_t* gids_sorted, const int32_t* tile_bins,
                   const int32_t* tile_order, int sched, const float* records, const float* background, const float* final_Ts,
                   const int32_t* final_idx, const float* v_output, const float* v_output_alpha, float* v_xy,
                   float* v_conic, float* v_colors, float* v_opacity, cudaStream_t s) {
  return launch_bwd_any(img_h, img_w, channels, gids_sorted, nullptr, tile_bins, tile_order, sched, records, background,
                        final_Ts, final_idx, v_output, v_output_alpha, v_xy, v_conic, v_colors, v_opacity, s);
}

}

GB_API int gb_rasterize_ranked_fwd(int img_h, int img_w, int channels, const int32_t* tile_bins, const int32_t* tile_order,
                                   const int32_t* ranks_sorted, const float* rec_by_rank, const float* background,
                                   float* out_img, float* final_Ts, int32_t* final_idx, void* stream) {
  if (img_h <= 0 || img_w <= 0) return 0;
  if ((channels != 3 && channels != 4) || !ranks_sorted) return (int)cudaErrorInvalidValue;
  return gbblend::launch_fwd_any(img_h, img_w, channels, tile_bins, tile_order, 0, rec_by_rank, ranks_sorted, background,
                                 out_img, final_Ts, final_idx, (cudaStream_t)stream);
}
GB_API int gb_rasterize_ranked_bwd(int img_h, int img_w, int channels, const int32_t* rank_to_gid,
                                   const int32_t* ranks_sorted, const int32_t* tile_bins, const int32_t* tile_order,
                                   const float* rec_by_rank, const float* background, const float* final_Ts,
                                   const int32_t* final_idx, const float* v_output, const float* v_output_alpha,
                                   float* v_xy, float* v_conic, float* v_colors, float* v_opacity, void* stream) {
  if (img_h <= 0 || img_w <= 0) return 0;
  if ((channels != 3 && channels != 4) || !ranks_sorted) return (int)cudaErrorInvalidValue;
  return gbblend::launch_bwd_any(img_h, img_w, channels, rank_to_gid, ranks_sorted, tile_bins, tile_order, 0, rec_by_rank,
                                 background, final_Ts, final_idx, v_output, v_output_alpha, v_xy, v_conic, v_colors,
                                 v_opacity, (cudaStream_t)stream);
}
GB_API int gb_rasterize_ranked_fwd_lists(int img_h, int img_w, int channels, const int32_t* tile_bins,
                                         const int32_t* tile_order, const int32_t* ranks_sorted, const float* rec_by_rank,
                                         const float* background, float* out_img, float* final_Ts, int32_t* final_idx,
                                         int32_t* hit_list, int32_t* hit_count, void* stream) {
  if (img_h <= 0 || img_w <= 0) return 0;
  if ((channels != 3 && channels != 4) || !ranks_sorted || !hit_list || !hit_count) return (int)cudaErrorInvalidValue;
  return gbblend::launch_fwd_any(img_h, img_w, channels, tile_bins, tile_order, 0, rec_by_rank, ranks_sorted, background,
                                 out_img, final_Ts, final_idx, (cudaStream_t)stream, hit_list, hit_count);
}
GB_API int gb_rasterize_ranked_bwd_lists(int img_h, int img_w, int channels, const int32_t* ranks_sorted,
                                         const int32_t* tile_bins, const int32_t* hit_list, int32_t* hit_count,
                                         const float* rec_by_rank, const float* background, const float* final_Ts,
                                         const int32_t* final_idx, const float* v_output, const float* v_output_alpha,
                                         float* v_xy, float* v_conic, float* v_colors, float* v_opacity, void* stream) {
  if (img_h <= 0 || img_w <= 0) return 0;
  if ((channels != 3 && channels != 4) || !ranks_sorted || !hit_list || !hit_count) return (int)cudaErrorInvalidValue;
  return gbblend::launch_bwd_lists(img_h, img_w, channels, ranks_sorted, tile_bins, hit_list, hit_count,
                                   rec_by_rank, background, final_Ts, final_idx, v_output, v_output_alpha, v_xy, v_conic,
                                   v_colors, v_opacity, (cudaStream_t)stream);
}

GB_API int gb_records_widen(int64_t cap, const int32_t* n_dev, const float* records, float* records_wide, void* stream) {
  if (cap <= 0) return 0;
  records_widen_kernel<<<(unsigned)gb::cdiv64(cap, 256), 256, 0, (cudaStream_t)stream>>>(cap, n_dev, (const float4*)records,
                                                                                         (float4*)records_wide);
  gb::count_launches(1);
  GB_CHECK_LAUNCH();
  return 0;
}
GB_API int gb_records_set_colors4(int64_t cap, const int32_t* n_dev, const int32_t* gids_sorted, const float* colors, int nk,
                                  int64_t G, float* records_wide, void* stream) {
  if (cap <= 0) return 0;
  if (nk < 1 || nk > 4) return (int)cudaErrorInvalidValue;
  records_set_colors4_kernel<<<(unsigned)gb::cdiv64(cap, 256), 256, 0, (cudaStream_t)stream>>>(cap, n_dev, gids_sorted, colors, nk,
                                                                                               G, (float4*)records_wide);
  gb::count_launches(1);
  GB_CHECK_LAUNCH();
  return 0;
}
GB_API int gb_rasterize_multi_fwd(int img_h, int img_w, const int32_t* tile_bins, const int32_t* tile_order, int sched,
                                  const float* records_wide, const float* background, float* out_planes, void* stream) {
  if (img_h <= 0 || img_w <= 0) return 0;
  if (sched && !tile_order) return (int)cudaErrorInvalidValue;
  const int tbx = gb::cdiv(img_w, 16), tby = gb::cdiv(img_h, 16);
  blend_fwd_multi_kernel<<<tbx * tby, kFwdThreads, 0, (cudaStream_t)stream>>>(
      img_w, img_h, tbx, tile_order, sched, (const int2*)tile_bins, (const float4*)records_wide, background, out_planes);
  gb::count_launches(1);
  GB_CHECK_LAUNCH();
  return 0;
}
GB_API int gb_rasterize_multi_bwd(int img_h, int img_w, const int32_t* gids_sorted, const int32_t* tile_bins,
                                  const int32_t* tile_order, int sched, const float* records_wide, const float* background,
                                  const float* final_Ts, const int32_t* final_idx, const float* v_planes, float* v_xy,
                                  float* v_conic, float* v_colors12, float* v_opacity, void* stream) {
  if (img_h <= 0 || img_w <= 0) return 0;
  if (sched && !tile_order) return (int)cudaErrorInvalidValue;
  int dev = 0;
  GB_CUDA(cudaGetDevice(&dev));
  if (dev < 0 || dev >= 64 || !g_multi_attr_set[dev]) {
    GB_CUDA(cudaFuncSetAttribute(blend_bwd_multi_kernel, cudaFuncAttributeMaxDynamicSharedMemorySize, kMBwdSmem));
    if (dev >= 0 && dev < 64) g_multi_attr_set[dev] = true;
  }
  const int tbx = gb::cdiv(img_w, 16), tby = gb::cdiv(img_h, 16);
  blend_bwd_multi_kernel<<<tbx * tby, kBwdThreads, kMBwdSmem, (cudaStream_t)stream>>>(
      img_w, img_h, tbx, tile_order, sched, gids_sorted, (const int2*)tile_bins, (const float4*)records_wide, background, final_Ts,
      final_idx, v_planes, v_xy, v_conic, v_colors12, v_opacity);
  gb::count_launches(1);
  GB_CHECK_LAUNCH();
  return 0;
}
GB_API int gb_colors12_unpack(int64_t G, int nk, float* v_colors12, float* v_colors, void* stream) {
  if (G <= 0) return 0;
  if (nk < 1 || nk > 4) return (int)cudaErrorInvalidValue;
  colors12_unpack_kernel<<<(unsigned)gb::cdiv64(G, 256), 256, 0, (cudaStream_t)stream>>>(G, nk, (float4*)v_colors12, v_colors);
  gb::count_launches(1);
  GB_CHECK_LAUNCH();
  return 0;
}
```

### goliath_b200/gsplat/fused.py

```python
import os
from typing import NamedTuple

import torch
from torch.autograd import Function

from .. import _lib
from .project import _project_bwd, _project_fwd
from .utils import _tile_bounds, _workspace, bin_and_sort_gaussians, compute_cumulative_intersects, key_bits

_OVERFLOW = {}

BINNING = os.environ.get("GOLIATH_B200_BINNING", "buckets")
SPLIT = os.environ.get("GOLIATH_B200_RENDER_SPLIT", "1") != "0"
RANKED = os.environ.get("GOLIATH_B200_RECORDS", "ranked") == "ranked"


def _overflow_flag(dev):
    f = _OVERFLOW.get(dev.index)
    if f is None:
        f = torch.zeros(1, dtype=torch.int32, device=dev)
        _OVERFLOW[dev.index] = f
    return f


def check_overflow(device=None) -> bool:
    dev = torch.device("cuda", torch.cuda.current_device()) if device is None else torch.device(device)
    f = _OVERFLOW.get(dev.index)
    if f is None:
        return False
    hit = bool(f.item())
    if hit:
        f.zero_()
    return hit


class _BlendPlan(NamedTuple):
    sched: int
    order_len: int
    fwd: object
    bwd: object
    ranked: bool


def _blend_plan(T, schedule=True):
    L = _lib.lib()
    mode = L.gb_get_blend_mode()
    sched = 1 if schedule and mode in (2, 4) else 0
    return _BlendPlan(sched, L.gb_tile_schedule_ints(T) if sched else T,
                      L.gb_rasterize_sched_fwd if sched else L.gb_rasterize_packed_fwd,
                      L.gb_rasterize_sched_bwd if sched else L.gb_rasterize_packed_bwd,
                      RANKED and not sched and mode == 3)


def _bin_tiles(xys, depths, radii, conics, colors, opacity, comp, H, W, cap, plan, outs, ranked=False, n_out=None,
               colors_ready=None):
    G = xys.size(0)
    dev = xys.device
    L = _lib.lib()
    tb = _tile_bounds(H, W, 16)
    T = tb[0] * tb[1]
    bins = torch.empty(T, 2, device=dev, dtype=torch.int32)
    order = torch.empty(plan.order_len, device=dev, dtype=torch.int32)
    ws = _workspace(dev, L.gb_bin_tiles_workspace_bytes(G, T, cap))
    with torch.cuda.device(dev):
        _lib.check((L.gb_bin_tiles_ranked if ranked else L.gb_bin_tiles_pack_ev)(
            G, _lib.ptr(xys), _lib.ptr(depths), _lib.ptr(radii), _lib.ptr(conics), _lib.ptr(colors), _lib.ptr(opacity),
            _lib.ptr(comp), H, W, 16, cap, _lib.ptr(bins), _lib.ptr(order), plan.sched, *map(_lib.ptr, outs),
            _lib.ptr(n_out), _lib.ptr(_overflow_flag(dev)), _lib.ptr(ws), colors_ready, _lib.stream_ptr(dev)),
            "bin_tiles_ranked" if ranked else "bin_tiles_pack")
    return bins, order


def _blend_grads(H, W, v_out4, v_alpha, opacity, comp, blend, v_colors=None):
    G = comp.size(0)
    dev = comp.device
    f32 = dict(device=dev, dtype=torch.float32)
    v_out4 = torch.zeros(H, W, 4, **f32) if v_out4 is None else v_out4.contiguous()
    v_alpha = None if v_alpha is None else v_alpha.contiguous()
    acc = torch.zeros(G * 10, **f32)
    v_xy, v_conic = acc[:2 * G].view(G, 2), acc[2 * G:5 * G].view(G, 3)
    v_col4, v_opeff = acc[5 * G:9 * G].view(G, 4), acc[9 * G:]
    v_colors = torch.empty(G, 3, **f32) if v_colors is None else v_colors
    v_opacity, v_comp, v_depth = torch.empty(G, 1, **f32), torch.empty(G, **f32), torch.empty(G, **f32)
    with torch.cuda.device(dev):
        st = _lib.stream_ptr(dev)
        blend(st, v_out4, v_alpha, v_xy, v_conic, v_col4, v_opeff)
        _lib.check(_lib.lib().gb_splat_grad_unpack(G, _lib.ptr(v_col4), _lib.ptr(v_opeff), _lib.ptr(opacity),
                                                   _lib.ptr(comp), _lib.ptr(v_colors), _lib.ptr(v_opacity),
                                                   _lib.ptr(v_comp), _lib.ptr(v_depth), st), "splat_grad_unpack")
    return v_xy, v_conic, v_colors, v_opacity, v_comp, v_depth


class _RenderFused(Function):
    @staticmethod
    def forward(ctx, means3d, scales, quats, opacity, colors, viewmat, background, glob_scale, fx, fy, cx, cy, img_height,
                img_width, clip_thresh, capacity):
        ins = [t.contiguous() for t in (means3d, scales, quats, opacity, colors, viewmat, background)]
        for t, n in zip(ins, ("means3d", "scales", "quats", "opacity", "colors", "viewmat", "background")):
            _lib.check_input(t, n)
        means3d, scales, quats, opacity, colors, viewmat, background = ins
        G = means3d.size(0)
        if G == 0:
            capacity = None
        dev = means3d.device
        L = _lib.lib()
        f32 = dict(device=dev, dtype=torch.float32)
        i32 = dict(device=dev, dtype=torch.int32)
        H, W, BW = int(img_height), int(img_width), 16
        out4 = torch.empty(H, W, 4, **f32)
        final_Ts = torch.empty(H, W, **f32)
        final_idx = torch.empty(H, W, **i32)
        bg4 = torch.cat([background, background[:1]])
        xys, depths, radii, conics, comp, num_tiles_hit, cov3d = _project_fwd(
            means3d, scales, quats, viewmat, glob_scale, fx, fy, cx, cy, H, W, BW, clip_thresh)
        tb = _tile_bounds(H, W, BW)
        T = tb[0] * tb[1]
        plan = _blend_plan(T, schedule=capacity is not None)
        with torch.cuda.device(dev):
            st = _lib.stream_ptr(dev)
            if capacity is not None:
                cap = num_intersects = int(capacity)
                gids = torch.empty(cap, **i32)
                records = torch.empty(cap, 12, **f32)
                if BINNING == "buckets" and L.gb_bin_tiles_supported(G):
                    bins, order = _bin_tiles(xys, depths, radii, conics, colors, opacity, comp, H, W, cap, plan,
                                             (gids, records))
                else:
                    order = torch.empty(plan.order_len, **i32)
                    cum = torch.empty_like(num_tiles_hit)
                    ws = _workspace(dev, max(L.gb_cumsum_workspace_bytes(G), L.gb_sort_workspace_bytes(cap)))
                    _lib.check(L.gb_cumsum_i32(G, _lib.ptr(num_tiles_hit), _lib.ptr(cum), _lib.ptr(ws), st), "cumsum")
                    n_dev = cum.data_ptr() + 4 * (G - 1)
                    isect = torch.empty(cap, device=dev, dtype=torch.int64)
                    gids_u = torch.empty(cap, **i32)
                    isect_s = torch.empty(cap, device=dev, dtype=torch.int64)
                    bins = torch.zeros(T, 2, **i32)
                    _lib.check(L.gb_map_gaussian_to_intersects_dn(G, _lib.ptr(xys), _lib.ptr(depths), _lib.ptr(radii),
                                                                  _lib.ptr(cum), H, W, BW, cap, _lib.ptr(isect),
                                                                  _lib.ptr(gids_u), st), "map_dn")
                    _lib.check(L.gb_sort_intersects_dn(cap, n_dev, _lib.ptr(isect), _lib.ptr(gids_u),
                                                       _lib.ptr(isect_s), _lib.ptr(gids), key_bits(T), _lib.ptr(ws),
                                                       st), "sort_dn")
                    _lib.check(L.gb_get_tile_bin_edges_dn(cap, n_dev, _lib.ptr(isect_s), _lib.ptr(bins),
                                                          _lib.ptr(_overflow_flag(dev)), st), "edges_dn")
                    _lib.check((L.gb_tile_schedule if plan.sched else L.gb_tile_order)(
                        T, _lib.ptr(bins), _lib.ptr(order), st), "tile_order")
                    _lib.check(L.gb_pack_records_fused_dn(cap, n_dev, _lib.ptr(gids), _lib.ptr(xys), _lib.ptr(conics),
                                                          _lib.ptr(colors), _lib.ptr(depths), _lib.ptr(opacity),
                                                          _lib.ptr(comp), _lib.ptr(records), st),
                               "pack_records_fused_dn")
            else:
                num_intersects, cum = compute_cumulative_intersects(num_tiles_hit)
                if num_intersects < 1:
                    out4.copy_(bg4.expand(H, W, 4))
                    final_Ts.zero_()
                    final_idx.zero_()
                    gids = bins = order = records = torch.empty(0, **i32)
                else:
                    _, _, _, gids, bins = bin_and_sort_gaussians(G, num_intersects, xys, depths, radii, cum, tb, BW)
                    order = torch.empty(T, **i32)
                    records = torch.empty(num_intersects, 12, **f32)
                    _lib.check(L.gb_tile_order(T, _lib.ptr(bins), _lib.ptr(order), st), "tile_order")
                    _lib.check(L.gb_pack_records_fused(num_intersects, _lib.ptr(gids), _lib.ptr(xys), _lib.ptr(conics),
                                                       _lib.ptr(colors), _lib.ptr(depths), _lib.ptr(opacity),
                                                       _lib.ptr(comp), _lib.ptr(records), st), "pack_records_fused")
            if capacity is not None or num_intersects >= 1:
                _lib.check(plan.fwd(H, W, 4, _lib.ptr(bins), _lib.ptr(order), _lib.ptr(records), _lib.ptr(bg4),
                                    _lib.ptr(out4), _lib.ptr(final_Ts), _lib.ptr(final_idx), st),
                           "rasterize_packed_forward")
        ctx.save_for_backward(means3d, scales, quats, opacity, viewmat, bg4, cov3d, radii, conics, comp, gids, bins, order,
                              records, final_Ts, final_idx)
        ctx.meta = (H, W, num_intersects, float(glob_scale), float(fx), float(fy), plan)
        ctx.mark_non_differentiable(radii)
        ctx.set_materialize_grads(False)
        return out4, 1 - final_Ts, radii

    @staticmethod
    def backward(ctx, v_out4, v_alpha, _v_radii):
        (means3d, scales, quats, opacity, viewmat, bg4, cov3d, radii, conics, comp, gids, bins, order, records, final_Ts,
         final_idx) = ctx.saved_tensors
        H, W, num_intersects, glob_scale, fx, fy, plan = ctx.meta

        def blend(st, *grads):
            if num_intersects >= 1:
                _lib.check(plan.bwd(H, W, 4, _lib.ptr(gids), _lib.ptr(bins), _lib.ptr(order), _lib.ptr(records),
                                    _lib.ptr(bg4), _lib.ptr(final_Ts), _lib.ptr(final_idx), *map(_lib.ptr, grads), st),
                           "rasterize_packed_backward")

        v_xy, v_conic, v_colors, v_opacity, v_comp, v_depth = _blend_grads(H, W, v_out4, v_alpha, opacity, comp, blend)
        g_mean, g_scale, g_quat = _project_bwd(means3d, scales, quats, viewmat, cov3d, radii, conics, comp, glob_scale,
                                               fx, fy, v_xy, v_depth, v_conic, v_comp)
        return (g_mean, g_scale, g_quat, v_opacity, v_colors) + (None,) * 11


class _ProjectGeom(Function):

    @staticmethod
    def forward(ctx, means3d, scales, quats, viewmat, glob_scale, fx, fy, cx, cy, img_height, img_width, clip_thresh):
        ins = [t.contiguous() for t in (means3d, scales, quats, viewmat)]
        for t, n in zip(ins, ("means3d", "scales", "quats", "viewmat")):
            _lib.check_input(t, n)
        means3d, scales, quats, viewmat = ins
        xys, depths, radii, conics, comp, _, cov3d = _project_fwd(means3d, scales, quats, viewmat, glob_scale, fx, fy,
                                                                  cx, cy, img_height, img_width, 16, clip_thresh)
        ctx.save_for_backward(means3d, scales, quats, viewmat, cov3d, radii, conics, comp)
        ctx.meta = (float(glob_scale), float(fx), float(fy))
        ctx.mark_non_differentiable(radii)
        ctx.set_materialize_grads(False)
        return xys, depths, conics, comp, radii

    @staticmethod
    def backward(ctx, v_xy, v_depth, v_conic, v_comp, _v_radii):
        return _project_bwd(*ctx.saved_tensors, *ctx.meta, v_xy, v_depth, v_conic, v_comp) + (None,) * 9


class _BinBlend(Function):

    @staticmethod
    def forward(ctx, xys, depths, conics, comp, radii, opacity, colors, background, img_height, img_width, capacity,
                colors_event):
        opacity, colors, background = opacity.contiguous(), colors.contiguous(), background.contiguous()
        for t, n in zip((opacity, colors, background), ("opacity", "colors", "background")):
            _lib.check_input(t, n)
        G = xys.size(0)
        dev = xys.device
        L = _lib.lib()
        f32 = dict(device=dev, dtype=torch.float32)
        i32 = dict(device=dev, dtype=torch.int32)
        H, W = int(img_height), int(img_width)
        out4 = torch.empty(H, W, 4, **f32)
        final_Ts = torch.empty(H, W, **f32)
        final_idx = torch.empty(H, W, **i32)
        bg4 = torch.cat([background, background[:1]])
        tb = _tile_bounds(H, W, 16)
        cap = int(capacity)
        plan = _blend_plan(tb[0] * tb[1])
        ev = None
        if colors_event is not None:
            ev = colors_event.cuda_event
            colors.record_stream(torch.cuda.current_stream(dev))
        if plan.ranked:
            gids = torch.empty(G, **i32)
            ranks = torch.empty(cap, **i32)
            records = torch.empty(G, 12, **f32)
            outs = (ranks, records, gids)
        else:
            gids = torch.empty(cap, **i32)
            ranks = gids
            records = torch.empty(cap, 12, **f32)
            outs = (gids, records)
        bins, order = _bin_tiles(xys, depths, radii, conics, colors, opacity, comp, H, W, cap, plan, outs,
                                 ranked=plan.ranked, colors_ready=ev)
        hit_list = hit_count = None
        with torch.cuda.device(dev):
            st = _lib.stream_ptr(dev)
            if plan.ranked:
                hit_list = torch.empty(8 * cap, **i32)
                hit_count = torch.empty(16 * tb[0] * tb[1] + 2, **i32)
                _lib.check(L.gb_rasterize_ranked_fwd_lists(H, W, 4, _lib.ptr(bins), _lib.ptr(order), _lib.ptr(ranks),
                                                           _lib.ptr(records), _lib.ptr(bg4), _lib.ptr(out4),
                                                           _lib.ptr(final_Ts), _lib.ptr(final_idx), _lib.ptr(hit_list),
                                                           _lib.ptr(hit_count), st), "rasterize_ranked_forward")
            else:
                _lib.check(plan.fwd(H, W, 4, _lib.ptr(bins), _lib.ptr(order), _lib.ptr(records), _lib.ptr(bg4),
                                    _lib.ptr(out4), _lib.ptr(final_Ts), _lib.ptr(final_idx), st),
                           "rasterize_packed_forward")
        ctx.save_for_backward(opacity, comp, bg4, gids, bins, order, records, final_Ts, final_idx, ranks, hit_list,
                              hit_count)
        ctx.meta = (H, W, plan)
        ctx.set_materialize_grads(False)
        return out4, 1 - final_Ts

    @staticmethod
    def backward(ctx, v_out4, v_alpha):
        (opacity, comp, bg4, gids, bins, order, records, final_Ts, final_idx, ranks, hit_list,
         hit_count) = ctx.saved_tensors
        H, W, plan = ctx.meta

        def blend(st, *grads):
            if plan.ranked:
                _lib.check(_lib.lib().gb_rasterize_ranked_bwd_lists(
                    H, W, 4, _lib.ptr(ranks), _lib.ptr(bins), _lib.ptr(hit_list),
                    _lib.ptr(hit_count), _lib.ptr(records), _lib.ptr(bg4), _lib.ptr(final_Ts), _lib.ptr(final_idx),
                    *map(_lib.ptr, grads), st), "rasterize_ranked_backward")
            else:
                _lib.check(plan.bwd(H, W, 4, _lib.ptr(gids), _lib.ptr(bins), _lib.ptr(order), _lib.ptr(records),
                                    _lib.ptr(bg4), _lib.ptr(final_Ts), _lib.ptr(final_idx), *map(_lib.ptr, grads), st),
                           "rasterize_packed_backward")

        v_xy, v_conic, v_colors, v_opacity, v_comp, v_depth = _blend_grads(H, W, v_out4, v_alpha, opacity, comp, blend)
        return (v_xy, v_depth, v_conic, v_comp, None, v_opacity, v_colors) + (None,) * 5


def render_fused_split(means3d, scales, glob_scale, quats, viewmat, fx, fy, cx, cy, img_height, img_width, opacity, colors,
                       background, clip_thresh, capacity, colors_event=None):
    xys, depths, conics, comp, radii = _ProjectGeom.apply(means3d, scales, quats, viewmat, glob_scale, fx, fy, cx, cy,
                                                          img_height, img_width, clip_thresh)
    out4, alpha = _BinBlend.apply(xys, depths, conics, comp, radii, opacity, colors, background, img_height, img_width,
                                  capacity, colors_event)
    return out4, alpha, radii


def render_fused(means3d, scales, glob_scale, quats, viewmat, fx, fy, cx, cy, img_height, img_width, opacity, colors,
                 background, clip_thresh=0.01, capacity=None, colors_event=None):
    if (capacity is not None and SPLIT and BINNING == "buckets" and means3d.size(0) > 0
            and _lib.lib().gb_bin_tiles_supported(means3d.size(0))):
        return render_fused_split(means3d, scales, glob_scale, quats, viewmat, fx, fy, cx, cy, img_height, img_width,
                                  opacity, colors, background, clip_thresh, capacity, colors_event)
    if colors_event is not None:
        torch.cuda.current_stream(means3d.device).wait_event(colors_event)
    return _RenderFused.apply(means3d, scales, quats, opacity, colors, viewmat, background, glob_scale, fx, fy, cx, cy,
                              img_height, img_width, clip_thresh, capacity)
```

### include/goliath_b200.h

```cpp
#ifndef GOLIATH_B200_H_
#define GOLIATH_B200_H_

#include <stddef.h>
#include <stdint.h>

#ifdef __cplusplus
extern "C" {
#endif

int gb_version(void);
unsigned long long gb_launch_count(void);
void gb_launch_count_reset(void);


int gb_sg_evaluate_fwd(const float* lobe_dirs, const float* lobe_sigmas, const float* light_values,
                       const float* light_pts, const float* prim_pts, const int32_t* n_lights, float* integral,
                       int N, int D, int L, int w_type, void* stream);

int gb_sg_evaluate_bwd(const float* lobe_dirs, const float* lobe_sigmas, const float* light_values,
                       const float* light_pts, const float* prim_pts, const int32_t* n_lights,
                       const float* grad_integral, float* grad_dirs, float* grad_sigmas, float* grad_light_values,
                       int N, int D, int L, int w_type, void* stream);


int gb_project_gaussians_fwd(int G, const float* means3d, const float* scales, float glob_scale,
                             const float* quats, const float* viewmat, float fx, float fy, float cx, float cy,
                             int img_h, int img_w, int block_width, float clip_thresh, float* cov3d, float* xys,
                             float* depths, int32_t* radii, float* conics, float* compensation,
                             int32_t* num_tiles_hit, void* stream);

int gb_project_gaussians_bwd(int G, const float* means3d, const float* scales, float glob_scale,
                             const float* quats, const float* viewmat, float fx, float fy, const float* cov3d,
                             const int32_t* radii, const float* conics, const float* compensation,
                             const float* v_xy, const float* v_depth, const float* v_conic,
                             const float* v_compensation, float* v_cov2d, float* v_cov3d, float* v_mean3d,
                             float* v_scale, float* v_quat, void* stream);

size_t gb_cumsum_workspace_bytes(int n);
int gb_cumsum_i32(int n, const int32_t* in, int32_t* out, void* workspace, void* stream);

int gb_map_gaussian_to_intersects(int G, const float* xys, const float* depths, const int32_t* radii,
                                  const int32_t* cum_tiles_hit, int img_h, int img_w, int block_width,
                                  int64_t* isect_ids, int32_t* gaussian_ids, void* stream);

size_t gb_sort_workspace_bytes(int64_t n);
int gb_sort_intersects(int64_t n, const int64_t* isect_ids, const int32_t* gaussian_ids, int64_t* isect_sorted,
                       int32_t* gids_sorted, int key_bits, void* workspace, void* stream);

int gb_get_tile_bin_edges(int64_t n, const int64_t* isect_sorted, int32_t* tile_bins, void* stream);

int gb_rasterize_fwd(int img_h, int img_w, int block_width, int channels, const int32_t* gids_sorted,
                     const int32_t* tile_bins, const float* xys, const float* conics, const float* colors,
                     const float* opacities, const float* background, float* out_img, float* final_Ts,
                     int32_t* final_idx, void* stream);

int gb_rasterize_bwd(int img_h, int img_w, int block_width, int channels, const int32_t* gids_sorted,
                     const int32_t* tile_bins, const float* xys, const float* conics, const float* colors,
                     const float* opacities, const float* background, const float* final_Ts,
                     const int32_t* final_idx, const float* v_output, const float* v_output_alpha, float* v_xy,
                     float* v_conic, float* v_colors, float* v_opacity, void* stream);


int gb_pack_records(int64_t n, int channels, const int32_t* gids_sorted, const float* xys, const float* conics,
                    const float* colors, const float* opacities, float* records, void* stream);

int gb_pack_records_fused(int64_t n, const int32_t* gids_sorted, const float* xys, const float* conics,
                          const float* colors3, const float* depths, const float* opacity, const float* compensation,
                          float* records, void* stream);

int gb_records_set_colors(int64_t cap, const int32_t* n_dev, const int32_t* gids_sorted, const float* colors3,
                          const float* depths, float* records, void* stream);

int gb_records_widen(int64_t cap, const int32_t* n_dev, const float* records, float* records_wide, void* stream);
int gb_records_set_colors4(int64_t cap, const int32_t* n_dev, const int32_t* gids_sorted, const float* colors, int nk,
                           int64_t G, float* records_wide, void* stream);
int gb_rasterize_multi_fwd(int img_h, int img_w, const int32_t* tile_bins, const int32_t* tile_order, int sched,
                           const float* records_wide, const float* background, float* out_planes, void* stream);
int gb_rasterize_multi_bwd(int img_h, int img_w, const int32_t* gids_sorted, const int32_t* tile_bins,
                           const int32_t* tile_order, int sched, const float* records_wide, const float* background,
                           const float* final_Ts, const int32_t* final_idx, const float* v_planes, float* v_xy, float* v_conic,
                           float* v_colors12, float* v_opacity, void* stream);
int gb_colors12_unpack(int64_t G, int nk, float* v_colors12, float* v_colors, void* stream);

int gb_splat_grad_unpack(int G, const float* v_colors4, const float* v_opac_eff, const float* opacity,
                         const float* compensation, float* v_colors3, float* v_opacity, float* v_comp, float* v_depth,
                         void* stream);

int gb_map_gaussian_to_intersects_dn(int G, const float* xys, const float* depths, const int32_t* radii,
                                     const int32_t* cum_tiles_hit, int img_h, int img_w, int block_width, int64_t cap,
                                     int64_t* isect_ids, int32_t* gaussian_ids, void* stream);
int gb_sort_intersects_dn(int64_t cap, const int32_t* n_dev, const int64_t* isect_ids, const int32_t* gaussian_ids,
                          int64_t* isect_sorted, int32_t* gids_sorted, int key_bits, void* workspace, void* stream);
int gb_get_tile_bin_edges_dn(int64_t cap, const int32_t* n_dev, const int64_t* isect_sorted, int32_t* tile_bins,
                             int32_t* overflow, void* stream);
int gb_pack_records_fused_dn(int64_t cap, const int32_t* n_dev, const int32_t* gids_sorted, const float* xys,
                             const float* conics, const float* colors3, const float* depths, const float* opacity,
                             const float* compensation, float* records, void* stream);

int gb_get_rank_sort_mode(void);
int gb_get_tile_sort_mode(void);
void gb_set_tile_sort_mode(int mode);
void gb_set_rank_sort_mode(int mode);

int gb_bin_tiles_supported(int G);
size_t gb_bin_tiles_workspace_bytes(int G, int num_tiles, int64_t cap);
int gb_bin_tiles_pack(int G, const float* xys, const float* depths, const int32_t* radii, const float* conics,
                      const float* colors3, const float* opacity, const float* compensation, int img_h, int img_w,
                      int block_width, int64_t cap, int32_t* tile_bins, int32_t* tile_order, int tile_sched,
                      int32_t* gids_sorted, float* records, int32_t* n_out, int32_t* overflow, void* workspace,
                      void* stream);
int gb_bin_tiles_pack_ev(int G, const float* xys, const float* depths, const int32_t* radii, const float* conics,
                         const float* colors3, const float* opacity, const float* compensation, int img_h, int img_w,
                         int block_width, int64_t cap, int32_t* tile_bins, int32_t* tile_order, int tile_sched,
                         int32_t* gids_sorted, float* records, int32_t* n_out, int32_t* overflow, void* workspace,
                         void* colors_ready, void* stream);

int gb_bin_tiles_ranked(int G, const float* xys, const float* depths, const int32_t* radii, const float* conics,
                        const float* colors3, const float* opacity, const float* compensation, int img_h, int img_w,
                        int block_width, int64_t cap, int32_t* tile_bins, int32_t* tile_order, int tile_sched,
                        int32_t* ranks_sorted, float* rec_by_rank, int32_t* rank_to_gid, int32_t* n_out, int32_t* overflow,
                        void* workspace, void* colors_ready, void* stream);
int gb_rasterize_ranked_fwd(int img_h, int img_w, int channels, const int32_t* tile_bins, const int32_t* tile_order,
                            const int32_t* ranks_sorted, const float* rec_by_rank, const float* background,
                            float* out_img, float* final_Ts, int32_t* final_idx, void* stream);
int gb_rasterize_ranked_bwd(int img_h, int img_w, int channels, const int32_t* rank_to_gid, const int32_t* ranks_sorted,
                            const int32_t* tile_bins, const int32_t* tile_order, const float* rec_by_rank,
                            const float* background, const float* final_Ts, const int32_t* final_idx,
                            const float* v_output, const float* v_output_alpha, float* v_xy, float* v_conic,
                            float* v_colors, float* v_opacity, void* stream);
int gb_rasterize_ranked_fwd_lists(int img_h, int img_w, int channels, const int32_t* tile_bins, const int32_t* tile_order,
                                  const int32_t* ranks_sorted, const float* rec_by_rank, const float* background,
                                  float* out_img, float* final_Ts, int32_t* final_idx, int32_t* hit_list,
                                  int32_t* hit_count, void* stream);
int gb_rasterize_ranked_bwd_lists(int img_h, int img_w, int channels, const int32_t* ranks_sorted,
                                  const int32_t* tile_bins, const int32_t* hit_list,
                                  int32_t* hit_count, const float* rec_by_rank, const float* background,
                                  const float* final_Ts, const int32_t* final_idx, const float* v_output,
                                  const float* v_output_alpha, float* v_xy, float* v_conic, float* v_colors,
                                  float* v_opacity, void* stream);

int gb_tile_order(int num_tiles, const int32_t* tile_bins, int32_t* order, void* stream);

int gb_get_blend_mode(void);
void gb_set_blend_mode(int mode);

int gb_tile_schedule_ints(int num_tiles);
int gb_tile_schedule(int num_tiles, const int32_t* tile_bins, int32_t* sched, void* stream);
int gb_rasterize_sched_fwd(int img_h, int img_w, int channels, const int32_t* tile_bins, int32_t* sched,
                           const float* records, const float* background, float* out_img, float* final_Ts,
                           int32_t* final_idx, void* stream);
int gb_rasterize_sched_bwd(int img_h, int img_w, int channels, const int32_t* gids_sorted, const int32_t* tile_bins,
                           int32_t* sched, const float* records, const float* background, const float* final_Ts,
                           const int32_t* final_idx, const float* v_output, const float* v_output_alpha, float* v_xy,
                           float* v_conic, float* v_colors, float* v_opacity, void* stream);

int gb_rasterize_packed_fwd(int img_h, int img_w, int channels, const int32_t* tile_bins, const int32_t* tile_order,
                            const float* records, const float* background, float* out_img, float* final_Ts,
                            int32_t* final_idx, void* stream);

int gb_rasterize_packed_bwd(int img_h, int img_w, int channels, const int32_t* gids_sorted,
                            const int32_t* tile_bins, const int32_t* tile_order, const float* records,
                            const float* background, const float* final_Ts, const int32_t* final_idx,
                            const float* v_output, const float* v_output_alpha, float* v_xy, float* v_conic,
                            float* v_colors, float* v_opacity, void* stream);


int gb_compute_raydirs_fwd(int N, int H, int W, const float* viewpos, const float* viewrot, const float* focal,
                           const float* princpt, const float* pixelcoords, float volradius, float* raypos,
                           float* raydir, float* tminmax, void* stream);
int gb_compute_raydirs_bwd(void);


size_t gb_mvp_aabb_workspace_bytes(int N, int K);
int gb_mvp_compute_aabb(int N, int K, const float* primpos, const float* primrot, const float* primscale,
                        const int32_t* sortedobjid, const int32_t* nodechildren, const int32_t* nodeparent,
                        float* nodeaabb, void* workspace, void* stream);

int gb_get_raymarch_mode(void);
void gb_set_raymarch_mode(int mode);

int gb_mvp_raymarch_fwd(int N, int H, int W, int K, const float* raypos, const float* raydir, float stepsize,
                        const float* tminmax, const float* nodeaabb, const float* primpos, const float* primrot,
                        const float* primscale, int TD, int TH, int TW, const float* tplate, int WD, int WH, int WW,
                        const float* warp, float* rayrgba, float* raysat, float* shadow, int algo, float fadescale,
                        float fadeexp, int blocksizex, int blocksizey, void* stream);

int gb_mvp_raymarch_bwd(int N, int H, int W, int K, const float* raypos, const float* raydir, float stepsize,
                        const float* tminmax, const float* nodeaabb, const float* primpos, const float* primrot,
                        const float* primscale, int TD, int TH, int TW, const float* tplate, int WD, int WH, int WW,
                        const float* warp, const float* raysat, const float* grad_rayrgba, float* grad_primpos,
                        float* grad_primrot, float* grad_primscale, float* grad_tplate, float* grad_warp, int algo,
                        float fadescale, float fadeexp, int blocksizex, int blocksizey, void* stream);


int gb_rgca_heads_fwd(int B, int G, const float* f_vnocond, const float* f_vcond, const float* postex, const float* tn,
                      const float* albedo, const float* light_sh, const float* campos, float scale_lo, float scale_hi,
                      float* primpos, float* primqvec, float* primscale, float* primscale_preclip, float* opacity,
                      float* sigma, float* spec_vis, float* spec_dnml, float* spec_nml, float* diff_color,
                      float* ref_dirs, float* primnmlbase, float* shsum, const float* light_sh2, float* shsum2,
                      void* stream);

int gb_rgca_heads_bwd(int B, int G, const float* f_vnocond, const float* f_vcond, const float* postex, const float* tn,
                      const float* albedo, const float* light_sh, const float* campos, float scale_lo, float scale_hi,
                      const float* shsum, const float* g_primpos, const float* g_primqvec, const float* g_primscale,
                      const float* g_primscale_preclip, const float* g_opacity, const float* g_sigma,
                      const float* g_spec_vis, const float* g_spec_dnml, const float* g_spec_nml,
                      const float* g_diff_color, const float* g_ref_dirs, const float* g_primnmlbase, float* g_f_vnocond,
                      float* g_f_vcond, float* g_postex, float* g_tn, float* g_albedo, const float* light_sh2,
                      const float* g_shsum2, void* stream);


int gb_vert_normals_fwd(int B, int V, int F, const float* v, const int32_t* vi, float eps, float* acc, float* vn, void* stream);
int gb_vert_normals_bwd(int B, int V, int F, const float* v, const int32_t* vi, float eps, const float* acc, const float* g_vn,
                        float* g_acc, float* g_v, void* stream);
int gb_values_to_uv_fwd(int B, int V, int C, int64_t T, const float* values, const int32_t* index, const float* bary, float* out,
                        void* stream);
int gb_values_to_uv_bwd(int B, int V, int C, int64_t T, const int32_t* index, const float* bary, const float* g_out,
                        float* g_values, void* stream);


int gb_optim_chunk_elems(void);
int gb_optim_row_bytes(void);
int gb_grad_sanitize_sqnorm(const void* rows, const int32_t* chunks, int n_chunks, double* sqnorm, void* stream);
int gb_adam_step(const void* rows, const int32_t* chunks, int n_chunks, const double* sqnorm, float max_norm, float beta1,
                 float beta2, float eps, int step, int adamw, int write_grads, void* stream);


int gb_post_render_fwd(int B, int H, int W, const float* rgb, const float* alpha, const float* bg, const float* cal_w,
                       const float* cal_b, const int32_t* grey, const float* blur_w, float* pred, void* stream);
int gb_post_render_bwd(int B, int H, int W, const float* rgb, const float* alpha, const float* bg, const float* cal_w,
                       const float* cal_b, const int32_t* grey, const float* blur_w, const float* g_pred, float* g_rgb,
                       float* g_cal_w, float* g_cal_b, float* g_blur_w, void* stream);
int gb_ssim_l1_fwd(int B, int H, int W, const float* pred, const float* target, const float* mask, float* d_mu, float* d_pp,
                   float* d_tp, double* sums, void* stream);
int gb_ssim_l1_bwd(int B, int H, int W, const float* pred, const float* target, const float* mask, const float* d_mu,
                   const float* d_pp, const float* d_tp, const double* sums, const float* g_loss, float l1_weight,
                   float ssim_weight, float* g_pred, void* stream);

int gb_envmap_spec_fwd(int B, int G, int q, const float* const* levels, const int32_t* level_hw, const float* ref_dirs,
                       const float* sigma, const float* spec_vis, const float* lightrot, float level_scale, float* spec,
                       void* stream);
int gb_envmap_spec_bwd(int B, int G, int q, const float* const* levels, const int32_t* level_hw, const float* ref_dirs,
                       const float* sigma, const float* spec_vis, const float* lightrot, float level_scale,
                       const float* g_spec, float* g_ref_dirs, float* g_spec_vis, void* stream);

int gb_envmap_rotate(int B, int He, int We, const float* image, const float* rot_mat, float* out, void* stream);
int gb_envmap_compose_fwd(int B, int H, int W, int He, int We, const float* render, const float* alpha,
                          const float* envbg, const float* K, const float* Rt, int rt_rows, int rt_cols, float* hblur,
                          float* out, void* stream);
int gb_envmap_compose_bwd(int B, int H, int W, const float* g_out, float* g_render, void* stream);
int gb_envmap_prefilter_sg(int B, int q, const int32_t* level_hw, const float* sigma, const float* const* v,
                           const float* const* env_tex, const float* const* xi, int num_samples, unsigned long long seed,
                           float* const* out, void* stream);
int gb_envmap_spin_table(int B, int He, int We, const float* angles, const float* image, float perc90, float env_scale,
                         float* lightrot, float* envbg, float* hpass, float* envmap, float* light_intensity,
                         float* norm_scale, void* stream);

int gb_render_finish_fwd(int img_h, int img_w, const float* out4, const float* alpha, float* rgb, float* alpha_img,
                         float* depth, void* stream);
int gb_render_finish_bwd(int img_h, int img_w, const float* alpha, const float* g_rgb, const float* g_depth,
                         float* g_out4, void* stream);

int gb_sg_shade_compose_fwd(const float* lobe_dirs, const float* lobe_sigmas, const float* light_values,
                            const float* light_pts, const float* prim_pts, const int32_t* n_lights,
                            const float* diff_color, const float* spec_vis, float* color, float* spec_color, int N,
                            int D, int L, int w_type, void* stream);
int gb_sg_shade_compose_bwd(const float* lobe_dirs, const float* lobe_sigmas, const float* light_values,
                            const float* light_pts, const float* prim_pts, const int32_t* n_lights,
                            const float* diff_color, const float* spec_vis, const float* color, const float* g_color,
                            const float* g_spec_color, float* g_dirs, float* g_sigmas, float* g_diff, float* g_vis,
                            float* g_light_values, int N, int D, int L, int w_type, void* stream);


int gb_deconv4x4s2_wnub_fwd(int B, int Cin, int Cout, int Hi, int Wi, const float* x, const float* v,
                            const float* scale, const float* bias, float slope, int apply_act, float* out,
                            void* stream);

int gb_deconv4x4s2_wnub_bwd(int B, int Cin, int Cout, int Hi, int Wi, const float* x, const float* v,
                            const float* scale, const float* out, const float* gout, float slope, int apply_act,
                            float* gz, float* g_bias, float* gx, float* gw, void* stream);

int gb_conv4x4s2_wnub_fwd(int B, int Cin, int Cout, int Ho, int Wo, const float* x, const float* v,
                          const float* scale, const float* bias, float slope, int apply_act, float* out, void* stream);

int gb_conv4x4s2_wnub_bwd(int B, int Cin, int Cout, int Ho, int Wo, const float* x, const float* v,
                          const float* scale, const float* out, const float* gout, float slope, int apply_act,
                          float* gz, float* g_bias, float* gx, float* gw, void* stream);

size_t gb_deconv_tc_weight_bytes(int Cin_pad, int Cout);
int gb_nchw_to_nhwc_split(int B, int C, int Cpad, int H, int W, const float* x, float* hi, float* lo, void* stream);
int gb_deconv4x4s2_tc_fwd(int B, int Cin, int Cin_pad, int Cout, int Hi, int Wi, const float* x_hi, const float* x_lo,
                          const float* v, float* w_scratch, const float* scale, const float* bias, float slope,
                          int apply_act, float* out_hi, float* out_lo, int ldc, float* out_nchw, void* stream);


int gb_conv2d_wnub_fwd(int B, int Cin, int Cout, int H, int W, int K, const float* x, const float* v, const float* scale,
                       const float* bias, int bias_mode, float slope, int apply_act, float* out, void* stream);

int gb_conv2d_wnub_bwd(int B, int Cin, int Cout, int H, int W, int K, const float* x, const float* v, const float* scale,
                       const float* out, const float* gout, float slope, int apply_act, int bias_mode, float* gz,
                       float* g_bias, float* gx, float* gw, void* stream);

int gb_mvp_slab_to_prims_fwd(int B, int PZ, int U, int PSX, int PSY, int Kout, const float* rgb, const float* alpha,
                             const int* prim_slot, float rgb_mul, float rgb_add, int apply_relu, float* tpl,
                             void* stream);
int gb_mvp_slab_to_prims_bwd(int B, int PZ, int U, int PSX, int PSY, int Kout, const float* rgb, const float* alpha,
                             const int* prim_slot, float rgb_mul, float rgb_add, int apply_relu, const float* g_tpl,
                             float* g_rgb, float* g_alpha, void* stream);

int gb_mvp_prim_transform_fwd(int B, int K, const float* dec, const float* posbase, const float* rotbase,
                              float prim_scale, int zero_delta, float* primpos, float* primrot, float* primscale,
                              void* stream);
int gb_mvp_prim_transform_bwd(int B, int K, const float* dec, const float* posbase, const float* rotbase,
                              float prim_scale, int zero_delta, const float* g_primpos, const float* g_primrot,
                              const float* g_primscale, float* g_dec, void* stream);

int gb_mvp_prim_frames_fwd(int B, int V, int NT, int T, const float* verts, const int32_t* vidx, const int32_t* vtidx,
                           const float* bary, const float* vt, const float* vn, const float* campos, float* posbase,
                           float* rotbase, float* view_cos, void* stream);


int gb_lbs_max_joints(void);

int gb_lbs_skeleton_fwd(int B, int J, int P, int S, const float* motion, const float* scale, int scale_stride,
                        const float* transform, const float* transform_offsets, const float* joint_offset,
                        const float* joint_rotation, const int32_t* parents, const int32_t* level_order,
                        const int32_t* level_start, int n_levels, const float* bind_state, float* mats, float* states,
                        void* stream);

int gb_lbs_skin_fwd(int B, int V, int J, int vb, const float* mats, const float* verts, const float* templ,
                    const int32_t* skin_indices, const float* skin_weights, const float* global_scaling, float* out,
                    void* stream);
int gb_lbs_skin_bwd(int B, int V, int J, int vb, const float* mats, const int32_t* skin_indices,
                    const float* skin_weights, const float* global_scaling, const float* g_out, float* g_verts,
                    void* stream);

int gb_lbs_unskin_fwd(int B, int V, int J, int vb, const float* mats, const float* verts, const float* templ,
                      const int32_t* skin_indices, const float* skin_weights, const float* global_scaling, float* out,
                      void* stream);


int gb_mvp_shadow_march(int N, int L, int H, int W, int K, const float* raypos, const float* raydir, float stepsize,
                        const float* tminmax, const float* nodeaabb, const float* primpos, const float* primrot,
                        const float* primscale, int TD, int TH, int TW, int U, const float* alpha_slab,
                        const float* valid, float* shadow, float fadescale, float fadeexp, int blocksizex,
                        int blocksizey, void* stream);

int gb_olat_features(int B, int L, int K, int TD, int TH, int TW, int U, float volradius, const float* primpos,
                     const float* primrot, const float* primscale, const float* valid, const float* light_pos,
                     const float* campos, const float* shadow, float* feat, float* primshadow, int accumulate,
                     float* shadow_feat, void* stream);

int gb_olat_compose_fwd(int B, int L, int Z, int U, const float* tex, const float* intensity, const float* shadow_feat,
                        float* rgb, int accumulate, float* texolat, void* stream);
int gb_olat_compose_bwd(int B, int L, int Z, int U, const float* tex, const float* intensity, const float* shadow_feat,
                        const float* g_rgb, const float* g_texolat, float* g_tex, void* stream);


int gb_upconv_block_fwd(int B, int Cin, int Cout, int groups, int Hi, int Wi, const float* x, const float* v1,
                        const float* s1, const float* b1, const float* v2, const float* s2, const float* b2,
                        const float* vr, const float* sr, const float* br, float slope, float* h1, float* out,
                        unsigned char* mask, void* stream);
int gb_upconv_block_bwd(int B, int Cin, int Cout, int groups, int Hi, int Wi, const float* x, const float* v1,
                        const float* s1, const float* v2, const float* s2, const float* vr, const float* sr,
                        const float* h1, const unsigned char* mask, const float* gout, float slope, float* gz2,
                        float* gz1, float* gu, float* gb1, float* gb2, float* gbr, float* gw1, float* gw2, float* gwr,
                        float* gx, void* stream);

int gb_sparse_rows_apply(int B, int C, int n_rows, const int* row_ptr, const int* col, const float* coef,
                         const float* in, long long in_bs, long long in_cs, long long in_rs, float* out,
                         long long out_bs, long long out_cs, long long out_rs, void* stream);

int gb_conv3x3_ub_slice_fwd(int B, int Cin, int Cout, int H, int W, const float* x, long long x_bs, const float* v,
                            const float* scale, const float* bias, float* out, void* stream);
int gb_conv3x3_ub_slice_bwd(int B, int Cin, int Cout, int H, int W, const float* x, long long x_bs, const float* v,
                            const float* scale, const float* gout, float* g_bias, float* gx, float* gw, void* stream);

int gb_body_tex_compose_fwd(int B, int H, int W, const float* t1, const float* h, const float* v, const float* scale,
                            const float* bias, float tex_std, const float* tex_mean, const float* s3, float* out,
                            void* stream);
size_t gb_body_tex_compose_workspace_bytes(int H, int W);
int gb_body_tex_compose_bwd(int B, int H, int W, const float* t1, const float* h, const float* v, const float* scale,
                            const float* bias, float tex_std, const float* tex_mean, const float* s3,
                            const float* g_out, float* g_t1, float* g_h, float* g_bias, float* g_w, float* g_s3,
                            float* workspace, void* stream);


size_t gb_mesh_raster_workspace_bytes(int B, int F, int H, int W);
int gb_mesh_raster(int B, int V, int F, int H, int W, const float* v_pix, const int32_t* vi, int32_t* index_img,
                   void* workspace, void* stream);
int gb_mesh_render_fwd(int B, int V, int F, int H, int W, int C, int Ht, int Wt, const float* v_pix, const int32_t* vi,
                       const int32_t* vti, const float* vt, const float* tex, const int32_t* index_img,
                       float* depth_img, float* bary_img, float* vt_img, float* mask, float* render, void* stream);
size_t gb_mesh_render_bwd_workspace_bytes(int B, int F, int H, int W, int Ht, int Wt);
int gb_mesh_render_bwd(int B, int V, int F, int H, int W, int C, int Ht, int Wt, const float* v_pix, const int32_t* vi,
                       const int32_t* vti, const float* vt, const float* tex, const int32_t* index_img,
                       const float* vt_img, const float* render, const float* g_render, int edge_grad,
                       const int32_t* inc_ptr, const int32_t* inc, float* g_v_pix, float* g_tex, void* workspace,
                       void* stream);


int gb_downconv_block_fwd(int B, int Cin, int Cout, int groups, int H, int W, const float* x, long long x_bs,
                          long long x_cs, int x_rs, int Hs, int Ws, const unsigned char* cond_mask, float cond_scale,
                          const float* v1, const float* s1, const float* b1, const float* v2, const float* s2,
                          const float* b2, const float* vr, const float* sr, const float* br, float slope, float* h1,
                          float* out, unsigned char* mask, void* stream);
size_t gb_downconv_block_bwd_workspace_bytes(int B, int Cin, int Cout, int groups, int H, int W);
int gb_downconv_block_bwd(int B, int Cin, int Cout, int groups, int H, int W, const float* x, long long x_bs,
                          long long x_cs, int x_rs, int Hs, int Ws, const unsigned char* cond_mask, float cond_scale,
                          const float* v1, const float* s1, const float* v2, const float* s2, const float* vr,
                          const float* sr, const float* h1, const unsigned char* mask, const float* gout, float slope,
                          float* gz2, float* gz1, float* gb1, float* gb2, float* gbr, float* gw1, float* gw2,
                          float* gwr, float* gx, void* workspace, void* stream);


int gb_depth_disc_mask(int B, int H, int W, const float* depth, float threshold, unsigned char* mask, void* stream);
int gb_pixel_bias_fwd(int B, int C, int H, int W, int n_cams, int Hb, int Wb, const float* rgb, const float* bias,
                      const long long* idx, float* out, void* stream);
int gb_pixel_bias_bwd(int B, int C, int H, int W, int n_cams, int Hb, int Wb, const long long* idx, const float* g_out,
                      float* g_bias, void* stream);


int gb_face_tex_tail_fwd(int B, int Cin, int Cout, int Hi, int Wi, const float* x, const float* weight_v,
                         const float* scale, const float* bias, const float* face_bias, float* tex_raw, float* tex,
                         void* stream);
int gb_face_tex_cond_fwd(int B, int C, int Hs, int Ws, int H, int W, const float* x, const float* mask, float* out,
                         void* stream);
int gb_pose_shadow_fwd(int N, int h, int w, int H, int W, const float* x, float beta, float* out, void* stream);
int gb_pose_shadow_bwd(int N, int h, int w, int H, int W, const float* x, float beta, const float* g_out, float* g_x,
                       void* stream);

#ifdef __cplusplus
}
#endif
#endif
```

Baseline: 1583.

## Fuse per-tile depth sort into ranked rasterize forward kernel

Moves the per-tile radix sort out of the binning pipeline into a shared TileSort template, and adds a ranked rasterize forward entry point that sorts each tile's bucket inside the rasterizer before blending. The ranked path now calls a new bin_tiles_buckets entry that skips the separate tile_sort launch and hands the unsorted bucket to the rasterizer. This removes one kernel launch and a global round-trip of sorted ids. In exchange the rasterize kernel does more work per tile and may need more shared memory, which can lower occupancy.

Result: faster. 1644 (median of 6 runs) (+3.9%).

```diff
diff --git a/goliath_b200/_lib.py b/goliath_b200/_lib.py
--- a/goliath_b200/_lib.py
+++ b/goliath_b200/_lib.py
@@ -59,7 +59,9 @@
     "gb_rasterize_ranked_bwd": (_i, [_i, _i, _i] + [_vp] * 14 + [_vp]),
     "gb_rasterize_ranked_fwd_lists": (_i, [_i, _i, _i] + [_vp] * 10 + [_vp]),
     "gb_rasterize_ranked_bwd_lists": (_i, [_i, _i, _i] + [_vp] * 14 + [_vp]),
+    "gb_rasterize_ranked_fwd_sort_lists": (_i, [_i, _i, _i] + [_vp] * 12 + [_vp]),
     "gb_bin_tiles_ranked": (_i, [_i] + [_vp] * 7 + [_i, _i, _i, _i64] + [_vp, _vp, _i] + [_vp] * 6 + [_vp, _vp]),
+    "gb_bin_tiles_buckets": (_i, [_i] + [_vp] * 7 + [_i, _i, _i, _i64] + [_vp] * 8 + [_vp, _vp, _vp]),
     "gb_compute_raydirs_fwd": (_i, [_i, _i, _i] + [_vp] * 5 + [_f] + [_vp] * 3 + [_vp]),
     "gb_compute_raydirs_bwd": (_i, []),
     "gb_mvp_aabb_workspace_bytes": (_sz, [_i, _i]),
diff --git a/goliath_b200/csrc/splat_bin_tiles.cu b/goliath_b200/csrc/splat_bin_tiles.cu
--- a/goliath_b200/csrc/splat_bin_tiles.cu
+++ b/goliath_b200/csrc/splat_bin_tiles.cu
@@ -1,6 +1,7 @@
 
 #include "common.cuh"
 #include "splat_record.cuh"
+#include "splat_tile_sort.cuh"
 
 #include <algorithm>
 
@@ -20,43 +21,11 @@
 constexpr int kMaxGaussians = 3 << 19;
 
 constexpr int kSortThreads = 512;
-constexpr int kSortWarps = kSortThreads / 32;
-constexpr int kSortItems = 10;
-constexpr int kSortCap = kSortThreads * kSortItems;
-constexpr int kDigitBits = 9;
-constexpr int kDigits = 1 << kDigitBits;
-static_assert(kDigits == kSortThreads, "one digit per thread");
-constexpr int kTieRun = 16;
+using Sort = gbsort::TileSort<kSortThreads, 10>;
+constexpr int kSortCap = Sort::kCap;
+using gbsort::block_exclusive_scan;
 
 inline int count_items(int G) { return G <= 2048 * 192 ? 2 : 4; }
-
-__device__ __forceinline__ int block_exclusive_scan(int v, int* s_warp, int& total) {
-  const int lane = threadIdx.x & 31, warp = threadIdx.x >> 5;
-  int inc = v;
-#pragma unroll
-  for (int o = 1; o < 32; o <<= 1) {
-    int t = __shfl_up_sync(0xffffffffu, inc, o);
-    if (lane >= o) inc += t;
-  }
-  if (lane == 31) s_warp[warp] = inc;
-  __syncthreads();
-  if (warp == 0) {
-    int w = (lane < (int)(blockDim.x >> 5)) ? s_warp[lane] : 0;
-    int winc = w;
-#pragma unroll
-    for (int o = 1; o < 32; o <<= 1) {
-      int t = __shfl_up_sync(0xffffffffu, winc, o);
-      if (lane >= o) winc += t;
-    }
-    s_warp[lane] = winc - w;
-    if (lane == 31) s_warp[32] = winc;
-  }
-  __syncthreads();
-  total = s_warp[32];
-  const int r = s_warp[warp] + inc - v;
-  __syncthreads();
-  return r;
-}
 
 __device__ __forceinline__ void tile_bbox(float cx, float cy, float radius, int tbx, int tby, int bw, int& x0,
                                           int& y0, int& x1, int& y1) {
@@ -272,234 +241,16 @@
   }
 }
 
-struct SortSmem {
-  unsigned short whist[kSortWarps][kDigits];
-  int base[kDigits];
-  int run[kDigits];
-  int warp[33];
-  unsigned red[4];
-};
-
-__device__ __forceinline__ int entry_of(int j, int ipt) {
-  return (threadIdx.x >> 5) * (32 * ipt) + j * 32 + (threadIdx.x & 31);
-}
-
-__device__ __forceinline__ bool holds(int j, int ipt, int m) { return j < ipt && entry_of(j, ipt) < m; }
-
-__device__ __forceinline__ void radix_positions(const unsigned long long (&k)[kSortItems], int m, int ipt, int shift,
-                                                bool whole, SortSmem& s, int (&dst)[kSortItems]) {
-  const int lane = threadIdx.x & 31, warp = threadIdx.x >> 5;
-  const int wbase = warp * (32 * ipt);
-  const int ours = min(ipt, max(0, (m - wbase + 31) >> 5)), mine = min(ipt, max(0, (m - wbase - lane + 31) >> 5));
-  for (int d = lane; d < kDigits; d += 32) s.whist[warp][d] = 0;
-  __syncwarp();
-#pragma unroll
-  for (int j = 0; j < kSortItems; ++j) {
-    dst[j] = 0;
-    if (j >= ours) continue;
-    const bool valid = j < mine;
-    const unsigned dgt = (unsigned)(k[j] >> shift) & (kDigits - 1);
-    unsigned peers = __ballot_sync(0xffffffffu, valid);
-#pragma unroll
-    for (int b = 0; b < kDigitBits; ++b) {
-      const unsigned bal = __ballot_sync(0xffffffffu, (dgt >> b) & 1u);
-      peers &= ((dgt >> b) & 1u) ? bal : ~bal;
-    }
-    const unsigned lower = peers & ((1u << lane) - 1u);
-    unsigned prev = 0;
-    if (valid) prev = s.whist[warp][dgt];
-    __syncwarp();
-    dst[j] = (int)(prev + __popc(lower));
-    if (valid && lower == 0u) s.whist[warp][dgt] = (unsigned short)(prev + __popc(peers));
-    __syncwarp();
-  }
-  __syncthreads();
-  {
-    const int d = threadIdx.x;
-    int run = 0;
-#pragma unroll
-    for (int w = 0; w < kSortWarps; ++w) {
-      const int c = s.whist[w][d];
-      s.whist[w][d] = (unsigned short)run;
-      run += c;
-    }
-    int total;
-    if (whole) {
-      s.base[d] = block_exclusive_scan(run, s.warp, total);
-    } else {
-      const int b = s.run[d];
-      s.base[d] = b;
-      s.run[d] = b + run;
-    }
-  }
-  __syncthreads();
-#pragma unroll
-  for (int j = 0; j < kSortItems; ++j) {
-    const unsigned dgt = (unsigned)(k[j] >> shift) & (kDigits - 1);
-    dst[j] = (j < mine) ? s.base[dgt] + s.whist[warp][dgt] + dst[j] : -1;
-  }
-}
-
-__device__ __forceinline__ void smem_pass(unsigned long long (&k)[kSortItems], int n, int ipt, int shift, SortSmem& s,
-                                          unsigned long long* s_key) {
-  int dst[kSortItems];
-  radix_positions(k, n, ipt, shift, true, s, dst);
-#pragma unroll
-  for (int j = 0; j < kSortItems; ++j)
-    if (dst[j] >= 0) s_key[dst[j]] = k[j];
-  __syncthreads();
-#pragma unroll
-  for (int j = 0; j < kSortItems; ++j)
-    if (holds(j, ipt, n)) k[j] = s_key[entry_of(j, ipt)];
-}
-
-__device__ __forceinline__ void minmax_to_smem(unsigned kmin, unsigned kmax, unsigned imin, unsigned imax, SortSmem& s) {
-  kmin = __reduce_min_sync(0xffffffffu, kmin);
-  kmax = __reduce_max_sync(0xffffffffu, kmax);
-  imin = __reduce_min_sync(0xffffffffu, imin);
-  imax = __reduce_max_sync(0xffffffffu, imax);
-  if ((threadIdx.x & 31) == 0) {
-    atomicMin(&s.red[0], kmin);
-    atomicMax(&s.red[1], kmax);
-    atomicMin(&s.red[2], imin);
-    atomicMax(&s.red[3], imax);
-  }
-}
-
-__device__ __forceinline__ int bits_of(unsigned span) { return span ? 32 - __clz((int)span) : 0; }
-
 __global__ void __launch_bounds__(kSortThreads, 2) tile_sort_kernel(const int* __restrict__ order,
                                                                     const int2* __restrict__ tile_bins,
                                                                     const unsigned* __restrict__ depth_keys,
                                                                     int* bucket, int* out) {
   extern __shared__ unsigned long long s_key[];
-  __shared__ SortSmem s;
+  __shared__ Sort::Smem s;
   const int tile = order ? order[blockIdx.x] : (int)blockIdx.x;
   const int2 range = tile_bins[tile];
-  const int n = range.y - range.x;
-  if (n <= 0) return;
-  if (threadIdx.x == 0) {
-    s.red[0] = s.red[2] = 0xffffffffu;
-    s.red[1] = s.red[3] = 0u;
-  }
-  __syncthreads();
-
-  if (n <= kSortCap) {
-    const int ipt = (n + kSortThreads - 1) / kSortThreads;
-    int id[kSortItems];
-    unsigned dk[kSortItems];
-#pragma unroll
-    for (int j = 0; j < kSortItems; ++j) {
-      const bool h = holds(j, ipt, n);
-      id[j] = h ? bucket[range.x + entry_of(j, ipt)] : -1;
-      dk[j] = h ? (unsigned)out[range.x + entry_of(j, ipt)] : 0u;
-    }
-    unsigned kmin = 0xffffffffu, kmax = 0u, imin = 0xffffffffu, imax = 0u;
-#pragma unroll
-    for (int j = 0; j < kSortItems; ++j) {
-      if (id[j] < 0) continue;
-      kmin = min(kmin, dk[j]); kmax = max(kmax, dk[j]);
-      imin = min(imin, (unsigned)id[j]); imax = max(imax, (unsigned)id[j]);
-    }
-    minmax_to_smem(kmin, kmax, imin, imax, s);
-    __syncthreads();
-    kmin = s.red[0];
-    imin = s.red[2];
-    const int bi = bits_of(s.red[3] - imin), bits = bits_of(s.red[1] - kmin) + bi;
-    unsigned long long k[kSortItems];
-#pragma unroll
-    for (int j = 0; j < kSortItems; ++j)
-      k[j] = ((unsigned long long)(dk[j] - kmin) << bi) | (unsigned long long)((unsigned)id[j] - imin);
-    for (int shift = bi; shift < bits; shift += kDigitBits) smem_pass(k, n, ipt, shift, s, s_key);
-    if (bits == bi) {
-#pragma unroll
-      for (int j = 0; j < kSortItems; ++j)
-        if (holds(j, ipt, n)) s_key[entry_of(j, ipt)] = k[j];
-      __syncthreads();
-    }
-    static_assert(kTieRun < 32 && kSortItems * 5 <= 64, "run lengths are packed 5 bits per item");
-    unsigned long long runs = 0ull;
-    bool too_long = false;
-#pragma unroll
-    for (int j = 0; j < kSortItems; ++j) {
-      const int e = j * kSortThreads + threadIdx.x;
-      if (j >= ipt || e >= n) continue;
-      const unsigned long long d = s_key[e] >> bi;
-      if (e > 0 && (s_key[e - 1] >> bi) == d) continue;
-      int len = 1;
-      while (len <= kTieRun && e + len < n && (s_key[e + len] >> bi) == d) ++len;
-      if (len > kTieRun) too_long = true;
-      else runs |= (unsigned long long)len << (5 * j);
-    }
-    if (__syncthreads_or(too_long)) {
-#pragma unroll
-      for (int j = 0; j < kSortItems; ++j) k[j] = holds(j, ipt, n) ? s_key[entry_of(j, ipt)] : 0ull;
-      for (int shift = 0; shift < bits; shift += kDigitBits) smem_pass(k, n, ipt, shift, s, s_key);
-    } else {
-#pragma unroll
-      for (int j = 0; j < kSortItems; ++j) {
-        const int e = j * kSortThreads + threadIdx.x, len = (int)(runs >> (5 * j)) & 31;
-        for (int a = e + 1; a < e + len; ++a) {
-          const unsigned long long v = s_key[a];
-          int b = a;
-          for (; b > e && s_key[b - 1] > v; --b) s_key[b] = s_key[b - 1];
-          s_key[b] = v;
-        }
-      }
-      __syncthreads();
-    }
-    const unsigned long long imask = (1ull << bi) - 1ull;
-    for (int e = threadIdx.x; e < n; e += kSortThreads) out[range.x + e] = (int)(imin + (unsigned)(s_key[e] & imask));
-    return;
-  }
-
-  {
-    unsigned kmin = 0xffffffffu, kmax = 0u, imin = 0xffffffffu, imax = 0u;
-    for (int i = threadIdx.x; i < n; i += kSortThreads) {
-      const int g = bucket[range.x + i];
-      const unsigned d = depth_keys[g];
-      kmin = min(kmin, d); kmax = max(kmax, d);
-      imin = min(imin, (unsigned)g); imax = max(imax, (unsigned)g);
-    }
-    minmax_to_smem(kmin, kmax, imin, imax, s);
-  }
-  __syncthreads();
-  const unsigned kmin = s.red[0], imin = s.red[2];
-  const int bi = bits_of(s.red[3] - imin), bits = bits_of(s.red[1] - kmin) + bi;
-  const unsigned long long imask = (1ull << bi) - 1ull;
-  auto key_of = [&](int g) {
-    return ((unsigned long long)(depth_keys[g] - kmin) << bi) | (unsigned long long)((unsigned)g - imin);
-  };
-  int* src = bucket + range.x;
-  int* dstp = out + range.x;
-  for (int shift = 0; shift < bits; shift += kDigitBits) {
-    unsigned* s_cnt = reinterpret_cast<unsigned*>(s_key);
-    s_cnt[threadIdx.x] = 0u;
-    __syncthreads();
-    for (int i = threadIdx.x; i < n; i += kSortThreads)
-      atomicAdd(&s_cnt[(unsigned)(key_of(src[i]) >> shift) & (kDigits - 1)], 1u);
-    __syncthreads();
-    int total;
-    s.run[threadIdx.x] = block_exclusive_scan((int)s_cnt[threadIdx.x], s.warp, total);
-    __syncthreads();
-    for (int c0 = 0; c0 < n; c0 += kSortCap) {
-      const int m = min(kSortCap, n - c0);
-      unsigned long long k[kSortItems];
-#pragma unroll
-      for (int j = 0; j < kSortItems; ++j)
-        k[j] = holds(j, kSortItems, m) ? key_of(src[c0 + entry_of(j, kSortItems)]) : 0ull;
-      int dst[kSortItems];
-      radix_positions(k, m, kSortItems, shift, false, s, dst);
-#pragma unroll
-      for (int j = 0; j < kSortItems; ++j)
-        if (dst[j] >= 0) dstp[dst[j]] = (int)(imin + (unsigned)(k[j] & imask));
-      __syncthreads();
-    }
-    int* t = src; src = dstp; dstp = t;
-  }
-  if (src != out + range.x) {
-    for (int i = threadIdx.x; i < n; i += kSortThreads) out[range.x + i] = src[i];
-  }
+  if (range.y <= range.x) return;
+  Sort::sort_tile(range, depth_keys, bucket, out, s_key, s);
 }
 
 __global__ void __launch_bounds__(256) rec_colors_kernel(int G, const int* __restrict__ radii,
@@ -589,7 +340,8 @@
                           const float* colors3, const float* opacity, const float* compensation, int img_h, int img_w,
                           int block_width, int64_t cap, int32_t* tile_bins, int32_t* tile_order, int tile_sched,
                           int32_t* gids_sorted, float* records, int32_t* n_out, int32_t* overflow, void* workspace,
-                          void* colors_ready, void* stream, int32_t* ext_ids, float* ext_rec, int32_t* ext_identity);
+                          void* colors_ready, void* stream, int32_t* ext_ids, float* ext_rec, int32_t* ext_identity,
+                          int32_t* ext_bucket);
 
 GB_API int gb_bin_tiles_pack_ev(int G, const float* xys, const float* depths, const int32_t* radii, const float* conics,
                                 const float* colors3, const float* opacity, const float* compensation, int img_h,
@@ -598,7 +350,7 @@
                                 void* workspace, void* colors_ready, void* stream) {
   return bin_tiles_impl(G, xys, depths, radii, conics, colors3, opacity, compensation, img_h, img_w, block_width, cap,
                         tile_bins, tile_order, tile_sched, gids_sorted, records, n_out, overflow, workspace, colors_ready,
-                        stream, nullptr, nullptr, nullptr);
+                        stream, nullptr, nullptr, nullptr, nullptr);
 }
 
 GB_API int gb_bin_tiles_ranked(int G, const float* xys, const float* depths, const int32_t* radii, const float* conics,
@@ -609,14 +361,26 @@
   if (!ranks_sorted || !rec_by_rank || !rank_to_gid) return (int)cudaErrorInvalidValue;
   return bin_tiles_impl(G, xys, depths, radii, conics, colors3, opacity, compensation, img_h, img_w, block_width, cap,
                         tile_bins, tile_order, tile_sched, nullptr, nullptr, n_out, overflow, workspace, colors_ready, stream,
-                        ranks_sorted, rec_by_rank, rank_to_gid);
+                        ranks_sorted, rec_by_rank, rank_to_gid, nullptr);
+}
+
+GB_API int gb_bin_tiles_buckets(int G, const float* xys, const float* depths, const int32_t* radii, const float* conics,
+                                const float* colors3, const float* opacity, const float* compensation, int img_h,
+                                int img_w, int block_width, int64_t cap, int32_t* tile_bins, int32_t* tile_order,
+                                int32_t* ranks_keys, int32_t* bucket, float* rec_by_rank, int32_t* rank_to_gid,
+                                int32_t* n_out, int32_t* overflow, void* workspace, void* colors_ready, void* stream) {
+  if (!ranks_keys || !bucket || !rec_by_rank || !rank_to_gid) return (int)cudaErrorInvalidValue;
+  return bin_tiles_impl(G, xys, depths, radii, conics, colors3, opacity, compensation, img_h, img_w, block_width, cap,
+                        tile_bins, tile_order, 0, nullptr, nullptr, n_out, overflow, workspace, colors_ready, stream,
+                        ranks_keys, rec_by_rank, rank_to_gid, bucket);
 }
 
 static int bin_tiles_impl(int G, const float* xys, const float* depths, const int32_t* radii, const float* conics,
                           const float* colors3, const float* opacity, const float* compensation, int img_h, int img_w,
                           int block_width, int64_t cap, int32_t* tile_bins, int32_t* tile_order, int tile_sched,
                           int32_t* gids_sorted, float* records, int32_t* n_out, int32_t* overflow, void* workspace,
-                          void* colors_ready, void* stream, int32_t* ext_ids, float* ext_rec, int32_t* ext_identity) {
+                          void* colors_ready, void* stream, int32_t* ext_ids, float* ext_rec, int32_t* ext_identity,
+                          int32_t* ext_bucket) {
   if (!gb_bin_tiles_supported(G) || block_width < 1 || cap < 0) return (int)cudaErrorInvalidValue;
   cudaStream_t s = (cudaStream_t)stream;
   const int tbx = gb::cdiv(img_w, block_width), tby = gb::cdiv(img_h, block_width);
@@ -626,7 +390,7 @@
   char* ws = (char*)workspace;
   int* counts = (int*)(ws + l.counts);
   int* cursor = (int*)(ws + l.cursor);
-  int* bucket = (int*)(ws + l.bucket);
+  int* bucket = ext_bucket ? ext_bucket : (int*)(ws + l.bucket);
   int4* rects = (int4*)(ws + l.rects);
   const bool ranked = ext_ids != nullptr;
   float4* rec_by_id = ranked ? (float4*)ext_rec : (float4*)(ws + l.rec_by_id);
@@ -673,9 +437,12 @@
   tile_scatter_kernel<<<gb::cdiv(G, per_cta), kGaussBlock, scat_smem, s>>>(
       G, rects, (const float2*)xys, conics, late ? nullptr : colors3, depths, opacity, compensation, tbx, (long long)cap,
       per_cta, smem_tiles, stage_cap, cursor, bucket, (unsigned*)ids_sorted, rec_by_id);
-  tile_sort_kernel<<<T, kSortThreads, sort_smem, s>>>(tile_order, (const int2*)tile_bins, (const unsigned*)depths, bucket,
-                                                      ids_sorted);
-  gb::count_launches(2);
+  gb::count_launches(1);
+  if (!ext_bucket) {
+    tile_sort_kernel<<<T, kSortThreads, sort_smem, s>>>(tile_order, (const int2*)tile_bins, (const unsigned*)depths, bucket,
+                                                        ids_sorted);
+    gb::count_launches(1);
+  }
   if (late) {
     GB_CUDA(cudaStreamWaitEvent(s, (cudaEvent_t)colors_ready, 0));
     rec_colors_kernel<<<gb::cdiv(G, 256), 256, 0, s>>>(G, radii, colors3, depths, rec_by_id);
diff --git a/goliath_b200/csrc/splat_blend_mom.cu b/goliath_b200/csrc/splat_blend_mom.cu
--- a/goliath_b200/csrc/splat_blend_mom.cu
+++ b/goliath_b200/csrc/splat_blend_mom.cu
@@ -3,6 +3,7 @@
 
 #include "common.cuh"
 #include "splat_blend_common.cuh"
+#include "splat_tile_sort.cuh"
 
 namespace {
 
@@ -67,19 +68,46 @@
   return t;
 }
 
-template <int C, bool LIST, bool RANKED, bool HITS = false>
-__global__ void __launch_bounds__(kFwdThreads) blend_fwd_ilp_kernel(
+using FwdSort = gbsort::TileSort<kFwdThreads, 15>;
+
+template <bool LIST>
+struct FwdRing {
+  float4 rec[kFwdStages][kStageRecs * 3];
+  int hits[LIST ? kPixelWarps : 1][LIST ? kStageRecs + 4 : 4];
+};
+template <bool LIST, bool SORT>
+struct FwdSmem {
+  FwdRing<LIST> f;
+};
+template <bool LIST>
+struct FwdSmem<LIST, true> {
+  union {
+    FwdRing<LIST> f;
+    struct {
+      unsigned long long key[FwdSort::kCap];
+      FwdSort::Smem s;
+    } sort;
+  };
+};
+
+template <int C, bool LIST, bool RANKED, bool HITS, bool SORT>
+__device__ __forceinline__ void blend_fwd_body(
     int img_w, int img_h, int tbx, const int* order, int sched, const int2* __restrict__ tile_bins,
     const float4* __restrict__ rec , const int* __restrict__ ranks ,
     const float* __restrict__ background, float* __restrict__ final_Ts, int* __restrict__ final_idx,
-    float* __restrict__ out_img, int* __restrict__ hit_list = nullptr, int* __restrict__ hit_count = nullptr) {
+    float* __restrict__ out_img, int* __restrict__ hit_list, int* __restrict__ hit_count,
+    const unsigned* __restrict__ depth_keys , int* bucket ,
+    int* sorted ) {
   static_assert(!HITS || LIST, "hit lists are the LIST variant's per-stage lists");
-  __shared__ __align__(128) float4 s_rec[kFwdStages][kStageRecs * 3];
+  static_assert(!SORT || (LIST && RANKED && HITS), "the sorting forward is the ranked hit-list forward");
+  __shared__ __align__(128) FwdSmem<LIST, SORT> sm;
+  float4 (&s_rec)[kFwdStages][kStageRecs * 3] = sm.f.rec;
+  auto& s_hits = sm.f.hits;
   __shared__ __align__(8) unsigned long long s_full[kFwdStages];
   __shared__ __align__(8) unsigned long long s_empty[kFwdStages];
   __shared__ int s_ndone;
   __shared__ int s_tile;
-  __shared__ __align__(16) int s_hits[LIST ? kPixelWarps : 1][LIST ? kStageRecs + 4 : 4];
+  const int* rk = SORT ? sorted : ranks;
 
   const int tr = threadIdx.x, lane = tr & 31, warp = tr >> 5;
   if (tr == 0) {
@@ -96,6 +124,9 @@
   if (s_tile < 0) return;
   const Tile tl = make_tile(s_tile, tbx);
   const int2 range = tile_bins[tl.tile_id];
+  if constexpr (SORT) {
+    if (range.y > range.x) FwdSort::sort_tile(range, depth_keys, bucket, sorted, sm.sort.key, sm.sort.s);
+  }
   const int num_batches = (range.y - range.x + kStageRecs - 1) / kStageRecs;
 
   if (RANKED && warp == kPixelWarps) {
@@ -105,7 +136,7 @@
       const int start = range.x + b * kStageRecs;
       const int count = min(kStageRecs, range.y - start);
 #pragma unroll
-      for (int k = 0; k < 4; ++k) r[k] = (b < num_batches && lane + 32 * k < count) ? ranks[start + lane + 32 * k] : -1;
+      for (int k = 0; k < 4; ++k) r[k] = (b < num_batches && lane + 32 * k < count) ? rk[start + lane + 32 * k] : -1;
     };
     load_ranks(0);
     for (int b = 0; b < num_batches; ++b) {
@@ -328,6 +359,27 @@
   }
 }
 
+template <int C, bool LIST, bool RANKED, bool HITS = false>
+__global__ void __launch_bounds__(kFwdThreads) blend_fwd_ilp_kernel(
+    int img_w, int img_h, int tbx, const int* order, int sched, const int2* __restrict__ tile_bins,
+    const float4* __restrict__ rec, const int* __restrict__ ranks, const float* __restrict__ background,
+    float* __restrict__ final_Ts, int* __restrict__ final_idx, float* __restrict__ out_img,
+    int* __restrict__ hit_list = nullptr, int* __restrict__ hit_count = nullptr) {
+  blend_fwd_body<C, LIST, RANKED, HITS, false>(img_w, img_h, tbx, order, sched, tile_bins, rec, ranks, background,
+                                               final_Ts, final_idx, out_img, hit_list, hit_count, nullptr, nullptr,
+                                               nullptr);
+}
+
+template <int C>
+__global__ void __launch_bounds__(kFwdThreads, 3) blend_fwd_sort_kernel(
+    int img_w, int img_h, int tbx, const int* order, const int2* __restrict__ tile_bins, const float4* __restrict__ rec,
+    const float* __restrict__ background, float* __restrict__ final_Ts, int* __restrict__ final_idx,
+    float* __restrict__ out_img, int* __restrict__ hit_list, int* __restrict__ hit_count,
+    const unsigned* __restrict__ depth_keys, int* bucket, int* sorted) {
+  blend_fwd_body<C, true, true, true, true>(img_w, img_h, tbx, order, 0, tile_bins, rec, nullptr, background, final_Ts,
+                                            final_idx, out_img, hit_list, hit_count, depth_keys, bucket, sorted);
+}
+
 constexpr int kSmRec = kBwdStages * kStageRecs * kRecBytes;
 constexpr int kSmEntries = kPixelWarps * kEntryCap * 48;
 constexpr int kSmM = kPixelWarps * kChunk * kMStride * 8;
@@ -1354,6 +1406,23 @@
   return 0;
 }
 
+static int launch_fwd_sort(int img_h, int img_w, int channels, const int32_t* tile_bins, const int32_t* tile_order,
+                           const float* depths, int32_t* bucket, int32_t* ranks, const float* records,
+                           const float* background, float* out_img, float* final_Ts, int32_t* final_idx,
+                           int32_t* hit_list, int32_t* hit_count, cudaStream_t s) {
+  const int tbx = gb::cdiv(img_w, 16), tby = gb::cdiv(img_h, 16);
+#define GB_FWD_SORT(CC)                                                                                                 \
+  blend_fwd_sort_kernel<CC><<<tbx * tby, kFwdThreads, 0, s>>>(img_w, img_h, tbx, tile_order, (const int2*)tile_bins,     \
+                                                            (const float4*)records, background, final_Ts, final_idx,    \
+                                                            out_img, hit_list, hit_count, (const unsigned*)depths,      \
+                                                            bucket, ranks)
+  if (channels == 3) GB_FWD_SORT(3); else GB_FWD_SORT(4);
+#undef GB_FWD_SORT
+  gb::count_launches(1);
+  GB_CHECK_LAUNCH();
+  return 0;
+}
+
 static int launch_bwd_any(int img_h, int img_w, int channels, const int32_t* gids_sorted, const int32_t* ranks,
                           const int32_t* tile_bins, const int32_t* tile_order, int sched, const float* records,
                           const float* background, const float* final_Ts, const int32_t* final_idx, const float* v_output,
@@ -1465,6 +1534,17 @@
   return gbblend::launch_fwd_any(img_h, img_w, channels, tile_bins, tile_order, 0, rec_by_rank, ranks_sorted, background,
                                  out_img, final_Ts, final_idx, (cudaStream_t)stream, hit_list, hit_count);
 }
+GB_API int gb_rasterize_ranked_fwd_sort_lists(int img_h, int img_w, int channels, const int32_t* tile_bins,
+                                              const int32_t* tile_order, const float* depths, int32_t* bucket,
+                                              int32_t* ranks_keys, const float* rec_by_rank, const float* background,
+                                              float* out_img, float* final_Ts, int32_t* final_idx, int32_t* hit_list,
+                                              int32_t* hit_count, void* stream) {
+  if (img_h <= 0 || img_w <= 0) return 0;
+  if ((channels != 3 && channels != 4) || !depths || !bucket || !ranks_keys || !hit_list || !hit_count)
+    return (int)cudaErrorInvalidValue;
+  return gbblend::launch_fwd_sort(img_h, img_w, channels, tile_bins, tile_order, depths, bucket, ranks_keys, rec_by_rank,
+                                  background, out_img, final_Ts, final_idx, hit_list, hit_count, (cudaStream_t)stream);
+}
 GB_API int gb_rasterize_ranked_bwd_lists(int img_h, int img_w, int channels, const int32_t* ranks_sorted,
                                          const int32_t* tile_bins, const int32_t* hit_list, int32_t* hit_count,
                                          const float* rec_by_rank, const float* background, const float* final_Ts,
diff --git a/goliath_b200/csrc/splat_tile_sort.cuh b/goliath_b200/csrc/splat_tile_sort.cuh
--- /dev/null
+++ b/goliath_b200/csrc/splat_tile_sort.cuh
@@ -0,0 +1,309 @@
+#pragma once
+
+#include "common.cuh"
+
+namespace gbsort {
+
+constexpr int kDigitBits = 9;
+constexpr int kDigits = 1 << kDigitBits;
+constexpr int kTieRun = 16;
+
+__device__ __forceinline__ int block_exclusive_scan(int v, int* s_warp, int& total) {
+  const int lane = threadIdx.x & 31, warp = threadIdx.x >> 5;
+  int inc = v;
+#pragma unroll
+  for (int o = 1; o < 32; o <<= 1) {
+    int t = __shfl_up_sync(0xffffffffu, inc, o);
+    if (lane >= o) inc += t;
+  }
+  if (lane == 31) s_warp[warp] = inc;
+  __syncthreads();
+  if (warp == 0) {
+    int w = (lane < (int)(blockDim.x >> 5)) ? s_warp[lane] : 0;
+    int winc = w;
+#pragma unroll
+    for (int o = 1; o < 32; o <<= 1) {
+      int t = __shfl_up_sync(0xffffffffu, winc, o);
+      if (lane >= o) winc += t;
+    }
+    s_warp[lane] = winc - w;
+    if (lane == 31) s_warp[32] = winc;
+  }
+  __syncthreads();
+  total = s_warp[32];
+  const int r = s_warp[warp] + inc - v;
+  __syncthreads();
+  return r;
+}
+
+__device__ __forceinline__ int bits_of(unsigned span) { return span ? 32 - __clz((int)span) : 0; }
+
+template <int kThreads, int kItems>
+struct TileSort {
+  static constexpr int kWarps = kThreads / 32;
+  static constexpr int kCap = kThreads * kItems;
+  static constexpr int kDpt = (kDigits + kThreads - 1) / kThreads;
+  static constexpr int kRunWords = (kItems + 11) / 12;
+  static_assert(kThreads % 32 == 0 && kThreads <= 1024, "whole warps");
+  static_assert(kTieRun < 32, "run lengths are packed 5 bits per item");
+
+  struct Smem {
+    unsigned short whist[kWarps][kDigits];
+    int base[kDigits];
+    int run[kDigits];
+    int warp[33];
+    unsigned red[4];
+  };
+  static constexpr size_t kKeyBytes = (size_t)kCap * 8;
+
+  static __device__ __forceinline__ int entry_of(int j, int ipt) {
+    return (threadIdx.x >> 5) * (32 * ipt) + j * 32 + (threadIdx.x & 31);
+  }
+
+  static __device__ __forceinline__ bool holds(int j, int ipt, int m) { return j < ipt && entry_of(j, ipt) < m; }
+
+  static __device__ __forceinline__ void radix_positions(const unsigned long long (&k)[kItems], int m, int ipt,
+                                                         int shift, bool whole, Smem& s, int (&dst)[kItems]) {
+    const int lane = threadIdx.x & 31, warp = threadIdx.x >> 5;
+    const int wbase = warp * (32 * ipt);
+    const int ours = min(ipt, max(0, (m - wbase + 31) >> 5)), mine = min(ipt, max(0, (m - wbase - lane + 31) >> 5));
+    for (int d = lane; d < kDigits; d += 32) s.whist[warp][d] = 0;
+    __syncwarp();
+#pragma unroll
+    for (int j = 0; j < kItems; ++j) {
+      dst[j] = 0;
+      if (j >= ours) continue;
+      const bool valid = j < mine;
+      const unsigned dgt = (unsigned)(k[j] >> shift) & (kDigits - 1);
+      unsigned peers = __ballot_sync(0xffffffffu, valid);
+#pragma unroll
+      for (int b = 0; b < kDigitBits; ++b) {
+        const unsigned bal = __ballot_sync(0xffffffffu, (dgt >> b) & 1u);
+        peers &= ((dgt >> b) & 1u) ? bal : ~bal;
+      }
+      const unsigned lower = peers & ((1u << lane) - 1u);
+      unsigned prev = 0;
+      if (valid) prev = s.whist[warp][dgt];
+      __syncwarp();
+      dst[j] = (int)(prev + __popc(lower));
+      if (valid && lower == 0u) s.whist[warp][dgt] = (unsigned short)(prev + __popc(peers));
+      __syncwarp();
+    }
+    __syncthreads();
+    {
+      int run[kDpt], sum = 0;
+#pragma unroll
+      for (int i = 0; i < kDpt; ++i) {
+        const int d = (int)threadIdx.x * kDpt + i;
+        run[i] = 0;
+        if (d >= kDigits) continue;
+#pragma unroll
+        for (int w = 0; w < kWarps; ++w) {
+          const int c = s.whist[w][d];
+          s.whist[w][d] = (unsigned short)run[i];
+          run[i] += c;
+        }
+        sum += run[i];
+      }
+      if (whole) {
+        int total;
+        int b = block_exclusive_scan(sum, s.warp, total);
+#pragma unroll
+        for (int i = 0; i < kDpt; ++i) {
+          const int d = (int)threadIdx.x * kDpt + i;
+          if (d < kDigits) s.base[d] = b;
+          b += run[i];
+        }
+      } else {
+#pragma unroll
+        for (int i = 0; i < kDpt; ++i) {
+          const int d = (int)threadIdx.x * kDpt + i;
+          if (d >= kDigits) continue;
+          const int b = s.run[d];
+          s.base[d] = b;
+          s.run[d] = b + run[i];
+        }
+      }
+    }
+    __syncthreads();
+#pragma unroll
+    for (int j = 0; j < kItems; ++j) {
+      const unsigned dgt = (unsigned)(k[j] >> shift) & (kDigits - 1);
+      dst[j] = (j < mine) ? s.base[dgt] + s.whist[warp][dgt] + dst[j] : -1;
+    }
+  }
+
+  static __device__ __forceinline__ void smem_pass(unsigned long long (&k)[kItems], int n, int ipt, int shift,
+                                                   Smem& s, unsigned long long* s_key) {
+    int dst[kItems];
+    radix_positions(k, n, ipt, shift, true, s, dst);
+#pragma unroll
+    for (int j = 0; j < kItems; ++j)
+      if (dst[j] >= 0) s_key[dst[j]] = k[j];
+    __syncthreads();
+#pragma unroll
+    for (int j = 0; j < kItems; ++j)
+      if (holds(j, ipt, n)) k[j] = s_key[entry_of(j, ipt)];
+  }
+
+  static __device__ __forceinline__ void minmax_to_smem(unsigned kmin, unsigned kmax, unsigned imin, unsigned imax,
+                                                        Smem& s) {
+    kmin = __reduce_min_sync(0xffffffffu, kmin);
+    kmax = __reduce_max_sync(0xffffffffu, kmax);
+    imin = __reduce_min_sync(0xffffffffu, imin);
+    imax = __reduce_max_sync(0xffffffffu, imax);
+    if ((threadIdx.x & 31) == 0) {
+      atomicMin(&s.red[0], kmin);
+      atomicMax(&s.red[1], kmax);
+      atomicMin(&s.red[2], imin);
+      atomicMax(&s.red[3], imax);
+    }
+  }
+
+  static __device__ __forceinline__ void sort_tile(int2 range, const unsigned* __restrict__ depth_keys, int* bucket,
+                                                   int* out, unsigned long long* s_key, Smem& s) {
+    const int n = range.y - range.x;
+    if (threadIdx.x == 0) {
+      s.red[0] = s.red[2] = 0xffffffffu;
+      s.red[1] = s.red[3] = 0u;
+    }
+    __syncthreads();
+
+    if (n <= kCap) {
+      const int ipt = (n + kThreads - 1) / kThreads;
+      int id[kItems];
+      unsigned dk[kItems];
+#pragma unroll
+      for (int j = 0; j < kItems; ++j) {
+        const bool h = holds(j, ipt, n);
+        id[j] = h ? bucket[range.x + entry_of(j, ipt)] : -1;
+        dk[j] = h ? (unsigned)out[range.x + entry_of(j, ipt)] : 0u;
+      }
+      unsigned kmin = 0xffffffffu, kmax = 0u, imin = 0xffffffffu, imax = 0u;
+#pragma unroll
+      for (int j = 0; j < kItems; ++j) {
+        if (id[j] < 0) continue;
+        kmin = min(kmin, dk[j]); kmax = max(kmax, dk[j]);
+        imin = min(imin, (unsigned)id[j]); imax = max(imax, (unsigned)id[j]);
+      }
+      minmax_to_smem(kmin, kmax, imin, imax, s);
+      __syncthreads();
+      kmin = s.red[0];
+      imin = s.red[2];
+      const int bi = bits_of(s.red[3] - imin), bits = bits_of(s.red[1] - kmin) + bi;
+      unsigned long long k[kItems];
+#pragma unroll
+      for (int j = 0; j < kItems; ++j)
+        k[j] = ((unsigned long long)(dk[j] - kmin) << bi) | (unsigned long long)((unsigned)id[j] - imin);
+      for (int shift = bi; shift < bits; shift += kDigitBits) smem_pass(k, n, ipt, shift, s, s_key);
+      if (bits == bi) {
+#pragma unroll
+        for (int j = 0; j < kItems; ++j)
+          if (holds(j, ipt, n)) s_key[entry_of(j, ipt)] = k[j];
+        __syncthreads();
+      }
+      unsigned long long runs[kRunWords];
+#pragma unroll
+      for (int w = 0; w < kRunWords; ++w) runs[w] = 0ull;
+      bool too_long = false;
+#pragma unroll
+      for (int j = 0; j < kItems; ++j) {
+        const int e = j * kThreads + threadIdx.x;
+        if (j >= ipt || e >= n) continue;
+        const unsigned long long d = s_key[e] >> bi;
+        if (e > 0 && (s_key[e - 1] >> bi) == d) continue;
+        int len = 1;
+        while (len <= kTieRun && e + len < n && (s_key[e + len] >> bi) == d) ++len;
+        if (len > kTieRun) too_long = true;
+        else runs[j / 12] |= (unsigned long long)len << (5 * (j % 12));
+      }
+      if (__syncthreads_or(too_long)) {
+#pragma unroll
+        for (int j = 0; j < kItems; ++j) k[j] = holds(j, ipt, n) ? s_key[entry_of(j, ipt)] : 0ull;
+        for (int shift = 0; shift < bits; shift += kDigitBits) smem_pass(k, n, ipt, shift, s, s_key);
+      } else {
+#pragma unroll
+        for (int j = 0; j < kItems; ++j) {
+          const int e = j * kThreads + threadIdx.x, len = (int)(runs[j / 12] >> (5 * (j % 12))) & 31;
+          for (int a = e + 1; a < e + len; ++a) {
+            const unsigned long long v = s_key[a];
+            int b = a;
+            for (; b > e && s_key[b - 1] > v; --b) s_key[b] = s_key[b - 1];
+            s_key[b] = v;
+          }
+        }
+        __syncthreads();
+      }
+      const unsigned long long imask = (1ull << bi) - 1ull;
+      for (int e = threadIdx.x; e < n; e += kThreads) out[range.x + e] = (int)(imin + (unsigned)(s_key[e] & imask));
+      __syncthreads();
+      return;
+    }
+
+    {
+      unsigned kmin = 0xffffffffu, kmax = 0u, imin = 0xffffffffu, imax = 0u;
+      for (int i = threadIdx.x; i < n; i += kThreads) {
+        const int g = bucket[range.x + i];
+        const unsigned d = depth_keys[g];
+        kmin = min(kmin, d); kmax = max(kmax, d);
+        imin = min(imin, (unsigned)g); imax = max(imax, (unsigned)g);
+      }
+      minmax_to_smem(kmin, kmax, imin, imax, s);
+    }
+    __syncthreads();
+    const unsigned kmin = s.red[0], imin = s.red[2];
+    const int bi = bits_of(s.red[3] - imin), bits = bits_of(s.red[1] - kmin) + bi;
+    const unsigned long long imask = (1ull << bi) - 1ull;
+    auto key_of = [&](int g) {
+      return ((unsigned long long)(depth_keys[g] - kmin) << bi) | (unsigned long long)((unsigned)g - imin);
+    };
+    int* src = bucket + range.x;
+    int* dstp = out + range.x;
+    for (int shift = 0; shift < bits; shift += kDigitBits) {
+      unsigned* s_cnt = reinterpret_cast<unsigned*>(s_key);
+      for (int d = threadIdx.x; d < kDigits; d += kThreads) s_cnt[d] = 0u;
+      __syncthreads();
+      for (int i = threadIdx.x; i < n; i += kThreads)
+        atomicAdd(&s_cnt[(unsigned)(key_of(src[i]) >> shift) & (kDigits - 1)], 1u);
+      __syncthreads();
+      {
+        int c[kDpt], sum = 0;
+#pragma unroll
+        for (int i = 0; i < kDpt; ++i) {
+          const int d = (int)threadIdx.x * kDpt + i;
+          c[i] = (d < kDigits) ? (int)s_cnt[d] : 0;
+          sum += c[i];
+        }
+        int total;
+        int b = block_exclusive_scan(sum, s.warp, total);
+#pragma unroll
+        for (int i = 0; i < kDpt; ++i) {
+          const int d = (int)threadIdx.x * kDpt + i;
+          if (d < kDigits) s.run[d] = b;
+          b += c[i];
+        }
+      }
+      __syncthreads();
+      for (int c0 = 0; c0 < n; c0 += kCap) {
+        const int m = min(kCap, n - c0);
+        unsigned long long k[kItems];
+#pragma unroll
+        for (int j = 0; j < kItems; ++j)
+          k[j] = holds(j, kItems, m) ? key_of(src[c0 + entry_of(j, kItems)]) : 0ull;
+        int dst[kItems];
+        radix_positions(k, m, kItems, shift, false, s, dst);
+#pragma unroll
+        for (int j = 0; j < kItems; ++j)
+          if (dst[j] >= 0) dstp[dst[j]] = (int)(imin + (unsigned)(k[j] & imask));
+        __syncthreads();
+      }
+      int* t = src; src = dstp; dstp = t;
+    }
+    if (src != out + range.x) {
+      for (int i = threadIdx.x; i < n; i += kThreads) out[range.x + i] = src[i];
+    }
+    __syncthreads();
+  }
+};
+
+}
diff --git a/goliath_b200/gsplat/fused.py b/goliath_b200/gsplat/fused.py
--- a/goliath_b200/gsplat/fused.py
+++ b/goliath_b200/gsplat/fused.py
@@ -63,11 +63,13 @@
     order = torch.empty(plan.order_len, device=dev, dtype=torch.int32)
     ws = _workspace(dev, L.gb_bin_tiles_workspace_bytes(G, T, cap))
     with torch.cuda.device(dev):
-        _lib.check((L.gb_bin_tiles_ranked if ranked else L.gb_bin_tiles_pack_ev)(
-            G, _lib.ptr(xys), _lib.ptr(depths), _lib.ptr(radii), _lib.ptr(conics), _lib.ptr(colors), _lib.ptr(opacity),
-            _lib.ptr(comp), H, W, 16, cap, _lib.ptr(bins), _lib.ptr(order), plan.sched, *map(_lib.ptr, outs),
-            _lib.ptr(n_out), _lib.ptr(_overflow_flag(dev)), _lib.ptr(ws), colors_ready, _lib.stream_ptr(dev)),
-            "bin_tiles_ranked" if ranked else "bin_tiles_pack")
+        args = (G, _lib.ptr(xys), _lib.ptr(depths), _lib.ptr(radii), _lib.ptr(conics), _lib.ptr(colors),
+                _lib.ptr(opacity), _lib.ptr(comp), H, W, 16, cap, _lib.ptr(bins), _lib.ptr(order))
+        tail = (_lib.ptr(n_out), _lib.ptr(_overflow_flag(dev)), _lib.ptr(ws), colors_ready, _lib.stream_ptr(dev))
+        if ranked:
+            _lib.check(L.gb_bin_tiles_buckets(*args, *map(_lib.ptr, outs), *tail), "bin_tiles_buckets")
+        else:
+            _lib.check(L.gb_bin_tiles_pack_ev(*args, plan.sched, *map(_lib.ptr, outs), *tail), "bin_tiles_pack")
     return bins, order
 
 
@@ -242,8 +244,9 @@
         if plan.ranked:
             gids = torch.empty(G, **i32)
             ranks = torch.empty(cap, **i32)
+            bucket = torch.empty(cap, **i32)
             records = torch.empty(G, 12, **f32)
-            outs = (ranks, records, gids)
+            outs = (ranks, bucket, records, gids)
         else:
             gids = torch.empty(cap, **i32)
             ranks = gids
@@ -257,10 +260,10 @@
             if plan.ranked:
                 hit_list = torch.empty(8 * cap, **i32)
                 hit_count = torch.empty(16 * tb[0] * tb[1] + 2, **i32)
-                _lib.check(L.gb_rasterize_ranked_fwd_lists(H, W, 4, _lib.ptr(bins), _lib.ptr(order), _lib.ptr(ranks),
-                                                           _lib.ptr(records), _lib.ptr(bg4), _lib.ptr(out4),
-                                                           _lib.ptr(final_Ts), _lib.ptr(final_idx), _lib.ptr(hit_list),
-                                                           _lib.ptr(hit_count), st), "rasterize_ranked_forward")
+                _lib.check(L.gb_rasterize_ranked_fwd_sort_lists(
+                    H, W, 4, _lib.ptr(bins), _lib.ptr(order), _lib.ptr(depths), _lib.ptr(bucket), _lib.ptr(ranks),
+                    _lib.ptr(records), _lib.ptr(bg4), _lib.ptr(out4), _lib.ptr(final_Ts), _lib.ptr(final_idx),
+                    _lib.ptr(hit_list), _lib.ptr(hit_count), st), "rasterize_ranked_forward")
             else:
                 _lib.check(plan.fwd(H, W, 4, _lib.ptr(bins), _lib.ptr(order), _lib.ptr(records), _lib.ptr(bg4),
                                     _lib.ptr(out4), _lib.ptr(final_Ts), _lib.ptr(final_idx), st),
diff --git a/include/goliath_b200.h b/include/goliath_b200.h
--- a/include/goliath_b200.h
+++ b/include/goliath_b200.h
@@ -139,6 +139,17 @@
                                   const float* v_output_alpha, float* v_xy, float* v_conic, float* v_colors,
                                   float* v_opacity, void* stream);
 
+int gb_bin_tiles_buckets(int G, const float* xys, const float* depths, const int32_t* radii, const float* conics,
+                         const float* colors3, const float* opacity, const float* compensation, int img_h, int img_w,
+                         int block_width, int64_t cap, int32_t* tile_bins, int32_t* tile_order, int32_t* ranks_keys,
+                         int32_t* bucket, float* rec_by_rank, int32_t* rank_to_gid, int32_t* n_out, int32_t* overflow,
+                         void* workspace, void* colors_ready, void* stream);
+int gb_rasterize_ranked_fwd_sort_lists(int img_h, int img_w, int channels, const int32_t* tile_bins,
+                                       const int32_t* tile_order, const float* depths, int32_t* bucket,
+                                       int32_t* ranks_keys, const float* rec_by_rank, const float* background,
+                                       float* out_img, float* final_Ts, int32_t* final_idx, int32_t* hit_list,
+                                       int32_t* hit_count, void* stream);
+
 int gb_tile_order(int num_tiles, const int32_t* tile_bins, int32_t* order, void* stream);
 
 int gb_get_blend_mode(void);
```
